# rhmes/point-cloud-compression

Measured on AMD Instinct MI355X. Metric: points/sec compress+decompress (ModelNet40-shaped 8192 K=256), higher is better.
Workload: dtype f32 (operands split into two scaled fp16 pieces of 22-23 bits together, three fp16-MFMA products per fp32 product, fp32 accumulate); 1 GPU; IPDAE K=256 d=16 L=7, 8192-pt CAD-like synthetic clouds (configs[1]); distinct_clouds_per_gpu=1024, points_per_cloud=8192, patches_per_cloud=64, octree_mode=reference, weights=seeded random, matmul=f16x2

## Files before the change

include/pccx.h:

```cpp
#ifndef PCCX_H
#define PCCX_H

#include <stddef.h>
#include <stdint.h>

#ifdef __cplusplus
extern "C" {
#endif

#define PCCX_API __attribute__((visibility("default")))

typedef enum {
    PCCX_OK = 0,
    PCCX_ERR_ARG = -1,
    PCCX_ERR_HIP = -2,
    PCCX_ERR_UNSUPPORTED = -3
} pccx_status;

PCCX_API const char *pccx_last_error(void);
PCCX_API int pccx_version(void);


PCCX_API int pccx_normalize(const float *pc, int B, int N, double margin, float *out, float *center,
                            float *longest, void *stream);

PCCX_API int pccx_denormalize(const float *pc, int B, int N, double margin, const float *center,
                              const float *longest, float *out, void *stream);

PCCX_API int pccx_fps(const float *xyz, int B, int N, int npoint, const int32_t *start_idx,
                      int64_t *idx_out, float *workspace, void *stream);

PCCX_API int pccx_morton_keys(const float *xyz, int64_t n, const float *lo_host, float extent, int64_t *keys,
                              void *stream);
PCCX_API int pccx_morton_keys_auto(const float *xyz, int64_t n, int64_t *keys, int32_t *bbox_workspace, void *stream);

PCCX_API size_t pccx_sort_keys_workspace_bytes(int64_t n);
PCCX_API int pccx_sort_keys_u64(int64_t *keys, int64_t n, int key_bits, int64_t *order, void *workspace, void *stream);
PCCX_API int pccx_gather_blocks(const float *pc, const int64_t *order, int64_t n, int block, int64_t first, int64_t stride,
                                int64_t count, float *blocks_out, void *stream);
PCCX_API int pccx_scatter_blocks(const float *rows_in, const int64_t *order, int64_t n, int block, int64_t first, int64_t stride,
                                 int64_t count, float *pc_out, void *stream);

PCCX_API int pccx_gather(const float *points, int B, int N, int C, const int64_t *idx, int M,
                         float *out, void *stream);

PCCX_API int pccx_knn(const float *q, int B, int M, const float *ref, int N, int K, float *dists,
                      int64_t *idx, float *nn, float patch_scale, void *stream);

PCCX_API int pccx_ball_query(const float *q, int B, int M, const float *ref, int N, int K,
                             float radius, float *dists, int64_t *idx, void *stream);
PCCX_API size_t pccx_ball_query_grid_workspace_ints(int B, int N);
PCCX_API int pccx_ball_query_grid(const float *q, int B, int M, const float *ref, int N, int K, float radius,
                                  int32_t *workspace, float *dists, int64_t *idx, void *stream);

PCCX_API int pccx_nn_dist(const float *X, int B, int P, const float *Y, int Q, float *d2, int32_t *nn,
                          void *stream);
PCCX_API int pccx_nn_dist_split_count(int B, int P, int Q);
PCCX_API int pccx_nn_dist_split(const float *X, int B, int P, const float *Y, int Q, int split, float *scratch_d, int32_t *scratch_nn,
                                float *d2, int32_t *nn, void *stream);

PCCX_API int pccx_grid_dims(int N, float ex, float ey, float ez, int32_t *dims, float *cell);
PCCX_API size_t pccx_grid_index_workspace_bytes(int B, int N);
PCCX_API size_t pccx_grid_query_workspace_bytes(int B, int M);
PCCX_API int pccx_grid_index_build(const float *Y, int B, int N, void *workspace, void *stream);
PCCX_API int pccx_grid_nn(const float *X, int B, int P, int Q, const void *index, void *query_workspace, float *d2, int32_t *nn,
                          void *stream);
PCCX_API int pccx_grid_knn(const float *q, int B, int M, int N, int K, const void *index, void *query_workspace, float *dists,
                           int64_t *idx, void *stream);

PCCX_API int pccx_chamfer_mean(const float *dxy, const float *dyx, int B, int P, int Q, float *out, void *stream);
PCCX_API int pccx_chamfer_grad(const float *X, int B, int P, const float *Y, int Q, const int32_t *nn_xy,
                               const int32_t *nn_yx, float grad_out, float *gX, float *gY, void *stream);
PCCX_API int pccx_chamfer_grad_dev(const float *X, int B, int P, const float *Y, int Q, const int32_t *nn_xy,
                                   const int32_t *nn_yx, const float *grad_out_dev, float *gX, float *gY, void *stream);
PCCX_API int pccx_chamfer_grad_dev_acc(const float *X, int B, int P, const float *Y, int Q, const int32_t *nn_xy,
                                       const int32_t *nn_yx, const float *grad_out_dev, float *gX, float *gY, int flags,
                                       void *stream);

PCCX_API int pccx_estimate_normals(const float *xyz, int B, int N, const int64_t *nbr, int K, float *normals,
                                   void *stream);
PCCX_API int pccx_point_plane_err(const float *X, int B, int P, const float *Y, const float *normals_Y, int Q,
                                  const int32_t *nn, float *err, void *stream);


PCCX_API int pccx_octree_bits_capacity(int S);

PCCX_API int pccx_octree_encode(const float *centres, int B, int S, int N, double min_bpp,
                                uint8_t *bits, int32_t *nbits, int32_t *depth, uint8_t *bytes,
                                int32_t *nbytes, void *stream);

PCCX_API int pccx_octree_decode(const uint8_t *bytes, int stride, const int32_t *nbytes, int B,
                                int mode, int S_out, float *out, int32_t *count, void *stream);


PCCX_API size_t pccx_ae_encoder_blob_floats(void);
PCCX_API int pccx_pack_ae_encoder(const float *sa_w0, const float *sa_b0, const float *sa_w1,
                                  const float *sa_b1, const float *sa_w2, const float *sa_b2,
                                  const float *pn_w0, const float *pn_b0, const float *pn_w1,
                                  const float *pn_b1, const float *pn_w2, const float *pn_b2,
                                  const float *pn_w3, const float *pn_b3, int d, float *blob_host);
PCCX_API size_t pccx_ae_decoder_blob_floats(int k);
PCCX_API int pccx_pack_ae_decoder(const float *ip_w0, const float *ip_b0, const float *ip_w1,
                                  const float *ip_b1, const float *ip_w2, const float *ip_b2,
                                  const float *m_w0, const float *m_b0, const float *m_w1,
                                  const float *m_b1, const float *m_w2, const float *m_b2,
                                  const float *m_w3, const float *m_b3, int k, int d, float *blob_host);
PCCX_API size_t pccx_prob_blob_floats(void);
PCCX_API int pccx_pack_prob(const float *p_w0, const float *p_b0, const float *p_w1, const float *p_b1,
                            const float *p_w2, const float *p_b2, const float *m_w0, const float *m_b0,
                            const float *m_w1, const float *m_b1, const float *m_w2, const float *m_b2,
                            int d, int L, float *blob_host);

PCCX_API int pccx_ae_encode(const float *patches, int P, int K, const float *enc_blob, int d, int L,
                            float *feat_ws, float *latent_raw, float *latent, float *latent_q,
                            void *stream);

PCCX_API int pccx_sa_forward(const float *patches, int P, int K, const float *enc_blob, float *feat,
                             void *stream);
PCCX_API int pccx_pn_forward(const float *patches, const float *feat, int P, int K,
                             const float *enc_blob, int d, int L, float *latent_raw, float *latent,
                             float *latent_q, void *stream);

PCCX_API size_t pccx_ae_decode_workspace_floats(int P);
PCCX_API int pccx_ae_decode(const float *latent_q, int P, int d, int k, const float *dec_blob,
                            float *workspace, float *patches_out, float scale, const float *centres,
                            const float *nrm_center, const float *nrm_longest, int S, double margin,
                            float *pc_out, void *stream);

PCCX_API size_t pccx_sa_b3_blob_floats(void);
PCCX_API int pccx_pack_sa_b3(const float *enc_blob_dev, float *sa_b3_blob_dev, void *stream);
PCCX_API int pccx_sa_forward_b3(const float *patches, int P, int K, const float *enc_blob, const float *sa_b3_blob,
                                float *feat, void *stream);
PCCX_API size_t pccx_pn_b3_blob_floats(void);
PCCX_API int pccx_pack_pn_b3(const float *enc_blob_dev, float *pn_b3_blob_dev, void *stream);
PCCX_API int pccx_pn_forward_b3(const float *patches, const float *feat, int P, int K, const float *enc_blob,
                                const float *pn_b3_blob, int d, int L, float *latent_raw, float *latent,
                                float *latent_q, void *stream);
PCCX_API int pccx_ae_encode_b3_fused_ok(int K);
PCCX_API int pccx_ae_encode_b3(const float *patches, int P, int K, const float *enc_blob, const float *sa_b3_blob,
                               const float *pn_b3_blob, int d, int L, float *latent_raw, float *latent,
                               float *latent_q, void *stream);
PCCX_API int pccx_patch_knn16_index_bytes(int K);
PCCX_API size_t pccx_patch_knn16_bytes(int P, int K);
PCCX_API int pccx_patch_knn16(const float *patches, int P, int K, void *nbr, void *stream);
PCCX_API size_t pccx_ae_encode_b3_workspace_bytes(int P, int K);
PCCX_API int pccx_ae_encode_b3_ws(const float *patches, int P, int K, const float *enc_blob, const float *sa_b3_blob,
                                  const float *pn_b3_blob, int d, int L, float *latent_raw, float *latent,
                                  float *latent_q, void *workspace, void *stream);
PCCX_API int pccx_ae_encode_b3_tables(const float *patches, int P, int K, const float *enc_blob, const float *sa_b3_blob,
                                      const float *pn_b3_blob, int d, int L, float *latent_raw, float *latent,
                                      float *latent_q, const void *tables, void *stream);
PCCX_API size_t pccx_dec_b3_blob_floats(int k);
PCCX_API int pccx_pack_ae_decoder_b3(const float *dec_blob_dev, int k, float *b3_blob_dev, void *stream);
PCCX_API size_t pccx_ae_decode_b3_workspace_floats(int P);
PCCX_API int pccx_ae_decode_b3(const float *latent_q, int P, int d, int k, const float *dec_blob,
                               const float *b3_blob, float *workspace, float *patches_out, float scale,
                               const float *centres, const float *nrm_center, const float *nrm_longest,
                               int S, double margin, float *pc_out, void *stream);

PCCX_API size_t pccx_ae_encoder_h2_blob_floats(void);
PCCX_API int pccx_pack_ae_encoder_h2(const float *sa_w0, const float *sa_b0, const float *sa_w1, const float *sa_b1,
                                     const float *sa_w2, const float *sa_b2, const float *pn_w0, const float *pn_b0,
                                     const float *pn_w1, const float *pn_b1, const float *pn_w2, const float *pn_b2,
                                     const float *pn_w3, const float *pn_b3, int d, float *h2_blob);
PCCX_API int pccx_ae_encode_h2_fused_ok(int K);
PCCX_API size_t pccx_ae_encode_h2_workspace_bytes(int P, int K);
PCCX_API int pccx_ae_encode_h2_ws(const float *patches, int P, int K, const float *enc_blob, const float *h2_blob, int d, int L,
                                  float *latent_raw, float *latent, float *latent_q, void *workspace, void *stream);
PCCX_API int pccx_ae_encode_h2_tables(const float *patches, int P, int K, const float *enc_blob, const float *h2_blob, int d, int L,
                                      float *latent_raw, float *latent, float *latent_q, const void *tables, void *stream);
PCCX_API size_t pccx_ae_decoder_h2_blob_floats(int k);
PCCX_API int pccx_pack_ae_decoder_h2(const float *ip_w0, const float *ip_b0, const float *ip_w1, const float *ip_b1,
                                     const float *ip_w2, const float *ip_b2, const float *m_w0, const float *m_b0,
                                     const float *m_w1, const float *m_b1, const float *m_w2, const float *m_b2,
                                     const float *m_w3, const float *m_b3, int k, int d, float *h2_blob);
PCCX_API size_t pccx_ae_decode_h2_workspace_floats(int P);
PCCX_API int pccx_ae_decode_h2(const float *latent_q, int P, int d, int k, const float *dec_blob, const float *h2_blob,
                               float *workspace, float *patches_out, float scale, const float *centres,
                               const float *nrm_center, const float *nrm_longest, int S, double margin, float *pc_out,
                               void *stream);

PCCX_API size_t pccx_patch_groups_workspace_ints(int B);
PCCX_API int pccx_patch_groups(const float *keys_a, int floats_a, const float *keys_b, int floats_b, int B, int S, int32_t *rep,
                               int32_t *uniq, int32_t *n_uniq, int32_t *workspace, void *stream);
PCCX_API int pccx_replicate_rows(const int32_t *rep, int64_t P, int row_floats, float *a0, float *a1, float *a2, void *stream);
PCCX_API int pccx_knn_list(const float *q, int B, int M, const float *ref, int N, int K, float *dists, int64_t *idx, float *nn,
                           float patch_scale, const int32_t *rep, void *stream);
PCCX_API int pccx_patch_knn16_list(const float *patches, int P, int K, void *nbr, const int32_t *uniq, const int32_t *n_uniq,
                                   void *stream);
PCCX_API int pccx_ae_encode_h2_tables_list(const float *patches, int P, int K, const float *enc_blob, const float *h2_blob, int d,
                                           int L, float *latent_raw, float *latent, float *latent_q, const void *tables,
                                           const int32_t *uniq, const int32_t *n_uniq, void *stream);
PCCX_API int pccx_ae_decode_h2_list(const float *latent_q, int P, int d, int k, const float *dec_blob, const float *h2_blob,
                                    float *workspace, float *patches_out, float scale, const float *centres,
                                    const float *nrm_center, const float *nrm_longest, int S, double margin, float *pc_out,
                                    const int32_t *uniq, const int32_t *n_uniq, void *stream);

PCCX_API int pccx_prob_forward(const float *centres, int B, int S, int d, int L, const float *prob_blob,
                               float *pmf, float *cdf, int32_t *cdf_int, void *stream);

PCCX_API int pccx_range_encode(const int32_t *cdf_int, const float *latent_q, int B, int nsym, int L,
                               uint8_t *out, int cap, int32_t *nbytes, void *stream);
PCCX_API int pccx_range_decode(const int32_t *cdf_int, const uint8_t *in, int stride,
                               const int32_t *nbytes, int B, int nsym, int L, float *latent_q,
                               void *stream);

PCCX_API int pccx_cdf_float_to_int(const float *cdf, int64_t nrows, int Lp, int32_t *cdf_int, void *stream);


PCCX_API size_t pccx_streams_packed_bytes(int B, int s_stride, int p_cap);
PCCX_API int pccx_write_streams_host(const void *packed_host, int B, int s_stride, int p_cap, const char *dir, const char *names,
                                     const int64_t *name_off, int threads);
PCCX_API int pccx_read_streams_host(void *packed_host, int B, int s_stride, int p_cap, const char *dir, const char *names,
                                    const int64_t *name_off, int threads);
PCCX_API int pccx_stream_sizes_host(int B, const char *dir, const char *names, const int64_t *name_off, int64_t *s_sizes,
                                    int64_t *p_sizes, int threads);


PCCX_API size_t pccx_packed_linear_floats(int N, int K);
PCCX_API int pccx_pack_linear(const float *W_host, int N, int K, float *wp_host);
PCCX_API int pccx_linear(const float *x, int M, int K, int ldx, const float *wp, const float *bias,
                         int N, int relu, float *out, int ldo, void *stream);

PCCX_API size_t pccx_packed_linear_b3_floats(int N, int K);
PCCX_API int pccx_pack_linear_b3(const float *wp_dev, int N, int K, float *wplanes_dev, void *stream);
PCCX_API int pccx_linear_b3(const float *x, int M, int K, int ldx, const float *wplanes, const float *bias,
                            int N, int relu, float *out, int ldo, void *stream);

PCCX_API size_t pccx_planes_floats(int64_t M, int K);
PCCX_API int pccx_group_planes(const float *f0, int C0, int ld0, const float *f1, int C1, int ld1, const int64_t *idx, int64_t M,
                               int64_t rows_per_batch, int64_t n_src, float *planes, void *stream);
PCCX_API int pccx_group_planes_centred(const float *feats, int C, int ldf, const float *offsets, const int64_t *idx, int64_t M,
                                       int64_t rows_per_batch, int64_t n_src, float *amax8, float *planes, void *stream);
PCCX_API int pccx_fold_planes(const float *f0, int C0, int ld0, int64_t mod0, const float *f1, int C1, int ld1, int64_t div1, int64_t M,
                              float *planes, void *stream);
PCCX_API int pccx_rows_affine_planes(const float *base, int C, int64_t div, const float *x, int ldx, int Ks, int64_t mod, const float *w,
                                     int relu, int64_t M, float *planes, void *stream);
PCCX_API size_t pccx_planes_gemm_weight_floats(int N, int K);
PCCX_API int pccx_pack_planes_gemm(const float *wplanes_dev, int N, int K, float *wstream_dev, void *stream);
PCCX_API int pccx_planes_gemm(const float *planes_in, int64_t M, int K, const float *wstream, const float *bias, int N, int relu,
                              int epilogue, int group, float *out, int ldo, void *stream);
PCCX_API int pccx_planes_gemm_gather(const float *src, int ldp, const int64_t *idx, int64_t rows_per_batch, int64_t n_src, int64_t M,
                                     int K, const float *wstream, const float *bias, int N, int relu, int epilogue, int group,
                                     float *out, int ldo, void *stream);
PCCX_API size_t pccx_planes_chain_wide_weight_floats(int K0);
PCCX_API int pccx_pack_planes_chain_wide(const float *wp3_l0, const float *wp3_l1, const float *wp3_l2, int K0, int N0, int N1, int N2,
                                         float *wstream_dev, void *stream);
PCCX_API int pccx_planes_chain_wide(const float *src, int ldp, const int64_t *idx, int64_t rows_per_batch, int64_t n_src, int64_t M,
                                    int K0, const float *wstream, const float *b0, int N0, const float *b1, int N1, const float *b2,
                                    int N2, float *out_planes, void *stream);
PCCX_API int pccx_planes_chain4(const float *planes_in, int64_t M, int K0, const float *wstream, const float *b0, int N0,
                                const float *b1, int N1, const float *b2, int N2, const float *b3, int N3, int group, float *out,
                                int ldo, void *stream);
PCCX_API int pccx_planes_chain4_gather(const float *src, int ldp, const int64_t *idx, int64_t rows_per_batch, int64_t n_src, int64_t M,
                                       int K0, const float *wstream, const float *b0, int N0, const float *b1, int N1,
                                       const float *b2, int N2, const float *b3, int N3, int group, float *out, int ldo, void *stream);

PCCX_API size_t pccx_planes_floats_h2(int64_t M, int K);
PCCX_API size_t pccx_packed_linear_h2_floats(int N, int K);
PCCX_API int pccx_pack_linear_h2(const float *wp_dev, int N, int K, float tau, float *wplanes_dev, void *stream);
PCCX_API size_t pccx_planes_gemm_weight_floats_h2(int N, int K);
PCCX_API int pccx_pack_planes_gemm_h2(const float *wplanes_dev, int N, int K, float *wstream_dev, void *stream);
PCCX_API int pccx_group_planes_h2(const float *f0, int C0, int ld0, const float *f1, int C1, int ld1, const int64_t *idx, int64_t M,
                                  int64_t rows_per_batch, int64_t n_src, float rho, const float *dyn, float *planes, void *stream);
PCCX_API int pccx_group_planes_centred_h2(const float *feats, int C, int ldf, const float *offsets, const int64_t *idx, int64_t M,
                                          int64_t rows_per_batch, int64_t n_src, float *amax8, float rho, const float *dyn, float *planes,
                                          void *stream);
PCCX_API int pccx_fold_planes_h2(const float *f0, int C0, int ld0, int64_t mod0, const float *f1, int C1, int ld1, int64_t div1, int64_t M,
                                 float rho, const float *dyn, float *planes, void *stream);
PCCX_API int pccx_rows_affine_planes_h2(const float *base, int C, int64_t div, const float *x, int ldx, int Ks, int64_t mod, const float *w,
                                        int relu, int64_t M, float rho, const float *dyn, float *planes, void *stream);
PCCX_API int pccx_planes_gemm_h2(const float *planes_in, int64_t M, int K, const float *wstream, const float *bias, int N, int relu,
                                 int epilogue, int group, float scale_out, const float *dyn, float *amax8, float *out, int ldo,
                                 void *stream);
PCCX_API int pccx_planes_gemm_h2_member_max(const float *planes_in, int64_t M, int K, const float *wstream, const float *bias, int N, int relu,
                                            int group, const unsigned char *member, float scale_out, const float *dyn, float *out, int ldo,
                                            void *stream);
PCCX_API int pccx_planes_gemm_h2_max_amax(const float *planes_in, int64_t M, int K, const float *wstream, const float *bias, int N, int relu,
                                          int group, float scale_out, const float *dyn, float *amax8, float *out, int ldo, void *stream);
PCCX_API int pccx_group_members(const int64_t *idx, int64_t n_idx, int64_t per_batch, int64_t n_src, unsigned char *member, void *stream);
PCCX_API int pccx_planes_gemm_gather_h2(const float *src, int ldp, const int64_t *idx, int64_t rows_per_batch, int64_t n_src, int64_t M,
                                        int K, const float *wstream, const float *bias, int N, int relu, int epilogue, int group,
                                        float rho_in, float scale_out, const float *dyn, float *amax8, float *out, int ldo,
                                        void *stream);
PCCX_API int pccx_planes_chain4_h2(const float *planes_in, int64_t M, int K0, const float *wstream, const float *b0, int N0,
                                   const float *b1, int N1, const float *b2, int N2, const float *b3, int N3, int group,
                                   const float *scales5_host, const float *dyn, float *amax8, float *out, int ldo, void *stream);
PCCX_API int pccx_planes_chain4_gather_h2(const float *src, int ldp, const int64_t *idx, int64_t rows_per_batch, int64_t n_src, int64_t M,
                                          int K0, const float *wstream, const float *b0, int N0, const float *b1, int N1,
                                          const float *b2, int N2, const float *b3, int N3, int group, const float *scales5_host,
                                          const float *dyn, float *amax8, float *out, int ldo, void *stream);
PCCX_API int pccx_absmax(const float *x, int64_t n, float *amax8, void *stream);
PCCX_API int pccx_dyn_scale(const float *m1_8, float a1, const float *m2_8, float a2, float add, int combine, float *dyn2, void *stream);

PCCX_API int pccx_softmax_cdf(const float *logits, int64_t rows, int L, float *pmf, float *cdf, int32_t *cdf_int, void *stream);
PCCX_API int pccx_reassemble(const float *patches, int64_t P, int k, float scale, const float *centres, const float *nrm_center,
                             const float *nrm_longest, int S, double margin, float *out, void *stream);
PCCX_API int pccx_rows_affine_small(const float *base, int C, int64_t div, const float *x, int ldx, int Ks, int64_t mod,
                                    const float *w, int relu, int64_t M, float *out, void *stream);
PCCX_API int pccx_gather_max(const float *y, int B, int N, int C, const int64_t *idx, int M, int ns, float *out, void *stream);
PCCX_API int pccx_gather_max_rows(const float *y, int B, int N, int C, const int64_t *idx, int M, int ns, const float *xyz, float *out, int ldo,
                                  void *stream);
PCCX_API int pccx_group_max(const float *x, int64_t G, int Kn, int C, float *out, void *stream);

PCCX_API int pccx_sigmoid_spread(const float *x, int64_t n, int L, int do_round, float *y, void *stream);
PCCX_API int pccx_round(const float *x, int64_t n, float *y, void *stream);

PCCX_API int pccx_quantize_st(const float *x, int64_t n, float qmin, float qmax, int levels, float *y_q,
                              float *y_deq, void *stream);

PCCX_API int pccx_pack_linear_device(const float *W, int N, int K, int transpose, float *wp, void *stream);
PCCX_API int pccx_linear_dw(const float *dZ, const float *X, int64_t M, int N, int K, int ldz, int ldx,
                            float *dW, int flags, void *stream);
PCCX_API int pccx_bn_train_stats(const float *Z, int64_t M, int C, float eps, float momentum, double *sums,
                                 float *mean, float *rstd, float *running_mean, float *running_var,
                                 void *stream);
PCCX_API int pccx_bn_relu_forward(const float *Z, int64_t M, int C, const float *mean, const float *rstd,
                                  const float *gamma, const float *beta, int relu, float *Y, void *stream);
PCCX_API int pccx_bn_relu_backward(const float *dY, const float *Y, const float *Z, int64_t M, int C,
                                   const float *mean, const float *rstd, const float *gamma, double *sums,
                                   float *dZ, float *g_gamma, float *g_beta, void *stream);
PCCX_API int pccx_linear_skinny(const float *x, int M, int K, int ldx, const float *W, const float *bias, int N, int flags,
                                float *out, int ldo, void *stream);
PCCX_API int pccx_linear_skinny_dx(const float *dZ, int M, int N, int ldz, const float *W, int K, int flags, float *dX, int ldd,
                                   void *stream);
PCCX_API int pccx_col_sum(const float *dY, int64_t M, int C, double *sums, float *g_bias, void *stream);
PCCX_API int pccx_bn_relu_train_forward(const float *Z, int64_t M, int C, float eps, float momentum, double *sums, const float *gamma,
                                        const float *beta, int relu, float *mean, float *rstd, float *running_mean,
                                        float *running_var, float *Y, int flags, void *stream);
PCCX_API int pccx_bn_relu_train_backward(const float *dY, const float *Y, const float *Z, int64_t M, int C, const float *mean,
                                         const float *rstd, const float *gamma, double *sums, float *dZ, float *g_gamma,
                                         float *g_beta, int flags, void *stream);
PCCX_API int pccx_col_sum_w(const float *dY, int64_t M, int C, double *sums, float *g_bias, int flags, void *stream);
PCCX_API size_t pccx_train_sums_doubles(int C);
PCCX_API int pccx_linear_moments(const float *x, int M, int K, int ldx, const float *wp, int N, int flags, float *out, int ldo,
                                 double *sums, void *stream);
PCCX_API int pccx_linear_bnback(const float *x, int M, int K, int ldx, const float *wp, int N, int flags, float *out, int ldo,
                                const float *Y, const float *Z, const float *mean, const float *rstd, double *sums, void *stream);
PCCX_API int pccx_zero_bytes(void *p, size_t bytes, void *stream);
PCCX_API int pccx_copy_bytes(const void *src, void *dst, size_t bytes, void *stream);
PCCX_API int pccx_add_i64_table(const int64_t *table_dev, int n, int64_t delta, void *stream);
PCCX_API int pccx_relu_backward(const float *dY, const float *Y, int64_t n, float *dZ, void *stream);
PCCX_API int pccx_group_max_arg(const float *x, int64_t G, int Kn, int C, float *out, int32_t *arg,
                                void *stream);
PCCX_API int pccx_group_max_backward(const float *dOut, const int32_t *arg, int64_t G, int Kn, int C,
                                     float *dX, void *stream);
PCCX_API int pccx_gather_backward(const float *dG, int ldg, const int64_t *idx, int B, int Mrows, int N,
                                  int C, float *dF, void *stream);
PCCX_API int pccx_gather_backward_acc(const float *dG, int ldg, const int64_t *idx, int B, int Mrows, int N, int C, float *dF,
                                      int flags, void *stream);
PCCX_API int pccx_smooth_l1(const float *a, const float *b, int64_t n, float grad_scale, double *value,
                            float *grad, void *stream);
PCCX_API int pccx_quantize_st_backward(const float *x, const float *d_ydeq, int64_t n, float qmin, float qmax,
                                       int levels, float *dx, void *stream);
PCCX_API int pccx_rate_from_logits(const float *logits, const float *y_q, int B, int bins, int ld_yq,
                                   float *out, void *stream);
PCCX_API int pccx_sumsq_accumulate(const float *g, int64_t n, double *acc, void *stream);
PCCX_API int pccx_adam_step(float *param, const float *grad, float *exp_avg, float *exp_avg_sq, int64_t n,
                            const double *gnorm_sq, float max_norm, float lr, float beta1, float beta2,
                            float eps, int step, void *stream);
PCCX_API int pccx_sumsq_multi(const int64_t *table_dev, int ntensors, int64_t total_blocks, double *acc, void *stream);
PCCX_API int pccx_adam_multi(const int64_t *table_dev, int ntensors, int64_t total_blocks, const double *gnorm_sq,
                             float max_norm, const float *hyper_dev, float lr, int step, float beta1, float beta2,
                             float eps, void *stream);
PCCX_API int pccx_adam_advance_dev(float *hyper, double beta1, double beta2, void *stream);
PCCX_API int pccx_adam_step_dev(float *param, const float *grad, float *exp_avg, float *exp_avg_sq, int64_t n,
                                const double *gnorm_sq, float max_norm, const float *hyper, float beta1, float beta2,
                                float eps, void *stream);

PCCX_API size_t pccx_linear_dw_det_workspace_floats(int64_t M, int N, int K);
PCCX_API int pccx_linear_dw_det(const float *dZ, const float *X, int64_t M, int N, int K, int ldz, int ldx, float *dW, int flags,
                                float *workspace, void *stream);
PCCX_API size_t pccx_linear_skinny_dx_det_workspace_floats(int M, int N, int K);
PCCX_API int pccx_linear_skinny_dx_det(const float *dZ, int M, int N, int ldz, const float *W, int K, int flags, float *dX, int ldd,
                                       float *workspace, void *stream);
PCCX_API size_t pccx_col_reduce_det_doubles(int64_t M, int C);
PCCX_API int pccx_col_reduce_det(int mode, const float *A, const float *Y, const float *Z, const float *mean, const float *rstd,
                                 int64_t M, int C, double *partials, double *sums, float *f32_out, void *stream);
PCCX_API size_t pccx_smooth_l1_det_doubles(int64_t n);
PCCX_API int pccx_smooth_l1_det(const float *a, const float *b, int64_t n, float grad_scale, double *partials, double *value,
                                float *grad, void *stream);
PCCX_API size_t pccx_sumsq_multi_det_doubles(int64_t total_blocks);
PCCX_API int pccx_sumsq_multi_det(const int64_t *table_dev, int ntensors, int64_t total_blocks, double *partials, double *acc,
                                  void *stream);
PCCX_API size_t pccx_scatter_add_ordered_workspace_ints(int B, int Mrows, int N);
PCCX_API int pccx_scatter_add_ordered(const float *vals, int ldv, const void *idx, int idx_is_i32, int B, int Mrows, int N, int C,
                                      float *out, int32_t *workspace, void *stream);
PCCX_API size_t pccx_chamfer_grad_det_workspace_floats(int B, int P, int Q);
PCCX_API size_t pccx_chamfer_grad_det_workspace_ints(int B, int P, int Q);
PCCX_API int pccx_chamfer_grad_det(const float *X, int B, int P, const float *Y, int Q, const int32_t *nn_xy, const int32_t *nn_yx,
                                   const float *grad_out_dev, float *gX, float *gY, float *ws_floats, int32_t *ws_ints, void *stream);

#ifdef __cplusplus
}
#endif
#endif
```

point-cloud-compression_amd/csrc/decoder.hip:

```cpp
#include <math.h>
#include <stdlib.h>

#include "blobs.h"
#include "common.h"
#include "mfma_chain.h"
#include "plane_ring.h"

__global__ __launch_bounds__(256, 2) void dec_head_kernel(const float *__restrict__ latent_q, int P, int d, int ntiles,
                                                          const float *__restrict__ blob, f32x4 *__restrict__ h2p,
                                                          const int *__restrict__ uniq, const int *__restrict__ n_uniq)
{
    const int tid = threadIdx.x, lane = tid & 63, w = tid >> 6;
    const int g = lane >> 4, n = lane & 15;
    const int tile = blockIdx.x * 4 + w;
    if (uniq) P = *n_uniq;
    if (tile >= (P + 15) / 16) return;
    const int patch = tile * 16 + n;
    const size_t src = patch < P ? (uniq ? (size_t)uniq[patch] : (size_t)patch) : 0;
    f32x4 in[1][1];
#pragma unroll
    for (int r = 0; r < 4; ++r) in[0][0][r] = (patch < P && 4 * g + r < d) ? latent_q[src * d + 4 * g + r] : 0.f;
    f32x4 a1[1][16];
#pragma unroll
    for (int mt = 0; mt < 16; ++mt) a1[0][mt] = *(const f32x4 *)(blob + DEC_H_B1 + 16 * mt + 4 * g);
    dense_acc<1, 16, 1, 16>((const f32x4 *)(blob + DEC_H_W1), lane, in, a1);
#pragma unroll
    for (int mt = 0; mt < 16; ++mt) a1[0][mt] = relu4(a1[0][mt]);
    const f32x4 *w2 = (const f32x4 *)(blob + DEC_H_W2);
#pragma unroll 1
    for (int mc = 0; mc < 16; ++mc) {
        const f32x4 *w2c = opaque_uniform(w2) + (size_t)mc * 4 * 64;
        f32x4 a2[1][4];
#pragma unroll
        for (int m = 0; m < 4; ++m) a2[0][m] = *(const f32x4 *)(blob + DEC_H_B2 + 16 * (4 * mc + m) + 4 * g);
        dense_acc<16, 4, 1, 64>(w2c, lane, a1, a2);
#pragma unroll
        for (int m = 0; m < 4; ++m) h2p[((size_t)(4 * mc + m) * ntiles + tile) * 64 + lane] = relu4(a2[0][m]);
    }
}

int pccx_dec_head_launch(const float *latent_q, int P, int d, int ntiles, const float *dec_blob, float *h2p, const int32_t *uniq,
                         const int32_t *n_uniq, hipStream_t st)
{
    hipLaunchKernelGGL(dec_head_kernel, dim3((ntiles + 3) / 4), dim3(256), 0, st, latent_q, P, d, ntiles, dec_blob, (f32x4 *)h2p, uniq, n_uniq);
    PCCX_CHECK_LAUNCH();
    return PCCX_OK;
}

__device__ __forceinline__ unsigned b3_rne(float x)
{
    unsigned u = __float_as_uint(x);
    u += 0x7FFFu + ((u >> 16) & 1u);
    return u >> 16;
}
__device__ __forceinline__ void b3_split(float x, unsigned &h, unsigned &m, unsigned &l)
{
    h = b3_rne(x);
    const float r1 = __fsub_rn(x, __uint_as_float(h << 16));
    m = b3_rne(r1);
    l = b3_rne(__fsub_rn(r1, __uint_as_float(m << 16)));
}

__global__ __launch_bounds__(256) void b3_split_kernel(const f32x4 *__restrict__ src, uint4 *__restrict__ dst, int n_outer, int KT16, int W,
                                                       size_t src_outer, size_t dst_outer, int src_w)
{
    const int lane = threadIdx.x & 63, T = (KT16 + 1) / 2;
    const size_t item = (size_t)blockIdx.x * 4 + (threadIdx.x >> 6);
    if (item >= (size_t)n_outer * T * W) return;
    const int j = (int)(item % W), t = (int)((item / W) % T);
    const size_t o = item / ((size_t)W * T);
    const f32x4 v0 = src[o * src_outer + ((size_t)(2 * t) * src_w + j) * 64 + lane];
    const f32x4 zero = {0.f, 0.f, 0.f, 0.f};
    const f32x4 v1 = 2 * t + 1 < KT16 ? src[o * src_outer + ((size_t)(2 * t + 1) * src_w + j) * 64 + lane] : zero;
    unsigned h[8], m[8], l[8];
#pragma unroll
    for (int r = 0; r < 4; ++r) { b3_split(v0[r], h[r], m[r], l[r]); b3_split(v1[r], h[4 + r], m[4 + r], l[4 + r]); }
    uint4 *d = dst + o * dst_outer + ((size_t)t * W + j) * 3 * 64 + lane;
    d[0] = make_uint4(h[0] | (h[1] << 16), h[2] | (h[3] << 16), h[4] | (h[5] << 16), h[6] | (h[7] << 16));
    d[64] = make_uint4(m[0] | (m[1] << 16), m[2] | (m[3] << 16), m[4] | (m[5] << 16), m[6] | (m[7] << 16));
    d[128] = make_uint4(l[0] | (l[1] << 16), l[2] | (l[3] << 16), l[4] | (l[5] << 16), l[6] | (l[7] << 16));
}

template <int NT>
__device__ __forceinline__ void dec_store_points(const f32x4 (&m3)[NT][1], int tile0, int ntiles, int g, int n, int P, int k, int p,
                                                 float *__restrict__ patches_out, float inv_scale_div, const float *__restrict__ centres,
                                                 const float *__restrict__ nrm_center, const float *__restrict__ nrm_longest, int S,
                                                 float one_minus_margin, float *__restrict__ pc_out)
{
    if (g != 0) return;
#pragma unroll
    for (int nt = 0; nt < NT; ++nt) {
        const int patch = (tile0 + nt) * 16 + n;
        if (tile0 + nt < ntiles && patch < P) {
            float v[3] = {m3[nt][0][0], m3[nt][0][1], m3[nt][0][2]};
            if (patches_out) {
                float *o = patches_out + ((size_t)patch * k + p) * 3;
                o[0] = v[0]; o[1] = v[1]; o[2] = v[2];
            }
            if (pc_out) {
                const int b = patch / S;
                const float lg = nrm_longest[b];
                float *o = pc_out + ((size_t)patch * k + p) * 3;
#pragma unroll
                for (int a = 0; a < 3; ++a) {
                    float t = __fdiv_rn(v[a], inv_scale_div);
                    t = __fadd_rn(t, centres[(size_t)patch * 3 + a]);
                    t = __fsub_rn(t, 0.5f);
                    t = __fdiv_rn(__fmul_rn(t, lg), one_minus_margin);
                    o[a] = __fadd_rn(t, nrm_center[3 * b + a]);
                }
            }
        }
    }
}

__global__ __launch_bounds__(256, 2) void dec_main_kernel(const f32x4 *__restrict__ h2p, const float *__restrict__ latent_q,
                                                          int P, int d, int k, int ntiles, const float *__restrict__ blob,
                                                          float *__restrict__ patches_out, float inv_scale_div,
                                                          const float *__restrict__ centres, const float *__restrict__ nrm_center,
                                                          const float *__restrict__ nrm_longest, int S, float one_minus_margin,
                                                          float *__restrict__ pc_out)
{
    const int tid = threadIdx.x, lane = tid & 63, w = tid >> 6;
    const int g = lane >> 4, n = lane & 15;
    const int nblk = (ntiles + 7) / 8;
    const int grp = blockIdx.x / (DEC_GROUP * k), rem = blockIdx.x % (DEC_GROUP * k);
    const int p = rem / DEC_GROUP, blk = grp * DEC_GROUP + rem % DEC_GROUP;
    if (blk >= nblk) return;
    const int tile0 = blk * 8 + 2 * w;
    __shared__ __attribute__((aligned(16))) f32x4 swt[2 * DEC_WS_CHUNK * 64];
    const int wu = __builtin_amdgcn_readfirstlane(w);
    const WStreamT<DEC_WS_CHUNK, 2> ws{blob + DEC_G_W(k) + (size_t)p * DEC_STREAM_CHUNKS * DEC_WS_CHUNK * 256, swt, DEC_STREAM_CHUNKS, lane, wu, false};
    ws.prologue();

    f32x4 acc[2][8];
#pragma unroll
    for (int mt = 0; mt < 8; ++mt) {
        const f32x4 b = *(const f32x4 *)(blob + DEC_G_B + p * 128 + 16 * mt + 4 * g);
        acc[0][mt] = b; acc[1][mt] = b;
    }
    const int t0 = tile0 < ntiles ? tile0 : ntiles - 1, t1 = tile0 + 1 < ntiles ? tile0 + 1 : ntiles - 1;
    {
        f32x4 b_cur[2], b_nxt[2];
        b_cur[0] = h2p[((size_t)0 * ntiles + t0) * 64 + lane];
        b_cur[1] = h2p[((size_t)0 * ntiles + t1) * 64 + lane];
#pragma unroll 1
        for (int c = 0; c < 64 / (DEC_WS_CHUNK / 8); ++c) {
            ws.boundary(c);
            const f32x4 *buf = swt + (c & 1) * DEC_WS_CHUNK * 64 + lane;
#pragma unroll
            for (int h = 0; h < DEC_WS_CHUNK / 8; ++h) {
                const int kt = (DEC_WS_CHUNK / 8) * c + h;
                const int kn = kt + 1 < 64 ? kt + 1 : 63;
                b_nxt[0] = h2p[((size_t)kn * ntiles + t0) * 64 + lane];
                b_nxt[1] = h2p[((size_t)kn * ntiles + t1) * 64 + lane];
                f32x4 a[8];
#pragma unroll
                for (int mt = 0; mt < 8; ++mt) a[mt] = buf[(h * 8 + mt) * 64];
                __builtin_amdgcn_sched_barrier(0);
#pragma unroll
                for (int r = 0; r < 4; ++r)
#pragma unroll
                    for (int mt = 0; mt < 8; ++mt) {
                        acc[0][mt] = mfma16(a[mt][r], b_cur[0][r], acc[0][mt]);
                        acc[1][mt] = mfma16(a[mt][r], b_cur[1][r], acc[1][mt]);
                    }
                __builtin_amdgcn_sched_barrier(0);
                b_cur[0] = b_nxt[0]; b_cur[1] = b_nxt[1];
            }
        }
    }
    f32x4 m3[2][1];
    {
        f32x4 in[2][9];
#pragma unroll
        for (int nt = 0; nt < 2; ++nt) {
#pragma unroll
            for (int mt = 0; mt < 8; ++mt) in[nt][mt] = relu4(acc[nt][mt]);
            const int patch = (tile0 + nt) * 16 + n;
#pragma unroll
            for (int r = 0; r < 4; ++r)
                in[nt][8][r] = (patch < P && 4 * g + r < d) ? latent_q[(size_t)patch * d + 4 * g + r] : 0.f;
        }
        f32x4 m0[2][8];
#pragma unroll
        for (int nt = 0; nt < 2; ++nt)
#pragma unroll
            for (int mt = 0; mt < 8; ++mt) m0[nt][mt] = *(const f32x4 *)(blob + DEC_M_B0 + 16 * mt + 4 * g);
        int f = DEC_STREAM_GEMM_FRAGS;
        dense_acc_stream<9, 8, 2>(ws, f, in, m0);
#pragma unroll
        for (int nt = 0; nt < 2; ++nt)
#pragma unroll
            for (int mt = 0; mt < 8; ++mt) m0[nt][mt] = relu4(m0[nt][mt]);
        f32x4 m1[2][4];
#pragma unroll
        for (int nt = 0; nt < 2; ++nt)
#pragma unroll
            for (int mt = 0; mt < 4; ++mt) m1[nt][mt] = *(const f32x4 *)(blob + DEC_M_B1 + 16 * mt + 4 * g);
        dense_acc_stream<8, 4, 2>(ws, f, m0, m1);
#pragma unroll
        for (int nt = 0; nt < 2; ++nt)
#pragma unroll
            for (int mt = 0; mt < 4; ++mt) m1[nt][mt] = relu4(m1[nt][mt]);
        f32x4 m2[2][2];
#pragma unroll
        for (int nt = 0; nt < 2; ++nt)
#pragma unroll
            for (int mt = 0; mt < 2; ++mt) m2[nt][mt] = *(const f32x4 *)(blob + DEC_M_B2 + 16 * mt + 4 * g);
        dense_acc_stream<4, 2, 2>(ws, f, m1, m2);
#pragma unroll
        for (int nt = 0; nt < 2; ++nt)
#pragma unroll
            for (int mt = 0; mt < 2; ++mt) m2[nt][mt] = relu4(m2[nt][mt]);
#pragma unroll
        for (int nt = 0; nt < 2; ++nt) m3[nt][0] = *(const f32x4 *)(blob + DEC_M_B3 + 4 * g);
        dense_acc_stream<2, 1, 2>(ws, f, m2, m3);
    }
    ws.drain();
    dec_store_points<2>(m3, tile0, ntiles, g, n, P, k, p, patches_out, inv_scale_div, centres, nrm_center, nrm_longest, S, one_minus_margin, pc_out);
}

template <int NT>
__global__ __launch_bounds__(256, NT == 2 ? 2 : 1) void dec_main_kernel_b3(const uint4 *__restrict__ h3, const float *__restrict__ latent_q,
                                                          int P, int d, int k, int ntiles, const float *__restrict__ blob,
                                                          const float *__restrict__ blob3,
                                                          float *__restrict__ patches_out, float inv_scale_div,
                                                          const float *__restrict__ centres, const float *__restrict__ nrm_center,
                                                          const float *__restrict__ nrm_longest, int S, float one_minus_margin,
                                                          float *__restrict__ pc_out)
{
    const int tid = threadIdx.x, lane = tid & 63, w = tid >> 6;
    const int g = lane >> 4, n = lane & 15;
    constexpr int GRP = DEC_GROUP * 2 / NT;
    const int nblk = (ntiles + 4 * NT - 1) / (4 * NT);
    const int grp = blockIdx.x / (GRP * k), rem = blockIdx.x % (GRP * k);
    const int p = rem / GRP, blk = grp * GRP + rem % GRP;
    if (blk >= nblk) return;
    const int tile0 = blk * 4 * NT + NT * w;
    __shared__ __attribute__((aligned(16))) f32x4 swt[4 * DEC_B3_CHUNK * 64];
    const int wu = __builtin_amdgcn_readfirstlane(w);
    const WStreamT<DEC_B3_CHUNK, 4> ws{blob3 + (size_t)p * DEC_B3_STREAM_CHUNKS * DEC_B3_CHUNK * 256, swt, DEC_B3_STREAM_CHUNKS, lane, wu, false};
    ws.prologue();

    f32x4 acc[NT][8];
#pragma unroll
    for (int mt = 0; mt < 8; ++mt) {
        const f32x4 b = *(const f32x4 *)(blob + DEC_G_B + p * 128 + 16 * mt + 4 * g);
#pragma unroll
        for (int nt = 0; nt < NT; ++nt) acc[nt][mt] = b;
    }
    int tq[NT];
#pragma unroll
    for (int nt = 0; nt < NT; ++nt) tq[nt] = tile0 + nt < ntiles ? tile0 + nt : ntiles - 1;
    pg_ring_gemm<3, NT, 3, 4, 2, true, 32, false>(
        ws, 32, [&](int nt, int pl, int t) { return h3 + (((size_t)t * ntiles + tq[nt]) * 3 + pl) * 64 + lane; }, 1.f, acc);
    f32x4 m3[NT][1];
    {
        int f = DEC_B3_GEMM_FRAGS;
        bf16x8 i0[NT][5][3];
        const f32x4 zero = {0.f, 0.f, 0.f, 0.f};
#pragma unroll
        for (int nt = 0; nt < NT; ++nt) {
#pragma unroll
            for (int t = 0; t < 4; ++t) b3_split8(relu4(acc[nt][2 * t]), relu4(acc[nt][2 * t + 1]), i0[nt][t]);
            const int patch = (tile0 + nt) * 16 + n;
            f32x4 lat;
#pragma unroll
            for (int r = 0; r < 4; ++r) lat[r] = (patch < P && 4 * g + r < d) ? latent_q[(size_t)patch * d + 4 * g + r] : 0.f;
            b3_split8(lat, zero, i0[nt][4]);
        }
        f32x4 m0[NT][8];
#pragma unroll
        for (int nt = 0; nt < NT; ++nt)
#pragma unroll
            for (int mt = 0; mt < 8; ++mt) m0[nt][mt] = *(const f32x4 *)(blob + DEC_M_B0 + 16 * mt + 4 * g);
        dense_b3_stream<5, 8, NT>(ws, f, i0, m0);
        bf16x8 i1[NT][4][3];
#pragma unroll
        for (int nt = 0; nt < NT; ++nt)
#pragma unroll
            for (int t = 0; t < 4; ++t) b3_split8(relu4(m0[nt][2 * t]), relu4(m0[nt][2 * t + 1]), i1[nt][t]);
        f32x4 m1[NT][4];
#pragma unroll
        for (int nt = 0; nt < NT; ++nt)
#pragma unroll
            for (int mt = 0; mt < 4; ++mt) m1[nt][mt] = *(const f32x4 *)(blob + DEC_M_B1 + 16 * mt + 4 * g);
        dense_b3_stream<4, 4, NT>(ws, f, i1, m1);
        bf16x8 i2[NT][2][3];
#pragma unroll
        for (int nt = 0; nt < NT; ++nt)
#pragma unroll
            for (int t = 0; t < 2; ++t) b3_split8(relu4(m1[nt][2 * t]), relu4(m1[nt][2 * t + 1]), i2[nt][t]);
        f32x4 m2[NT][2];
#pragma unroll
        for (int nt = 0; nt < NT; ++nt)
#pragma unroll
            for (int mt = 0; mt < 2; ++mt) m2[nt][mt] = *(const f32x4 *)(blob + DEC_M_B2 + 16 * mt + 4 * g);
        dense_b3_stream<2, 2, NT>(ws, f, i2, m2);
        bf16x8 i3[NT][1][3];
#pragma unroll
        for (int nt = 0; nt < NT; ++nt) b3_split8(relu4(m2[nt][0]), relu4(m2[nt][1]), i3[nt][0]);
#pragma unroll
        for (int nt = 0; nt < NT; ++nt) m3[nt][0] = *(const f32x4 *)(blob + DEC_M_B3 + 4 * g);
        dense_b3_stream<1, 1, NT>(ws, f, i3, m3);
    }
    ws.drain();
    dec_store_points<NT>(m3, tile0, ntiles, g, n, P, k, p, patches_out, inv_scale_div, centres, nrm_center, nrm_longest, S, one_minus_margin, pc_out);
}

static unsigned dec_grid(int ntiles, int k, int NT = 2)
{
    const int grp = DEC_GROUP * 2 / NT;
    const int nblk = (ntiles + 4 * NT - 1) / (4 * NT), groups = (nblk + grp - 1) / grp;
    return (unsigned)groups * grp * (unsigned)k;
}

extern "C" size_t pccx_ae_decode_workspace_floats(int P)
{
    const size_t ntiles = ((size_t)(P > 0 ? P : 0) + 15) / 16;
    return (size_t)64 * ntiles * 64 * 4;
}

extern "C" int pccx_ae_decode(const float *latent_q, int P, int d, int k, const float *dec_blob, float *workspace,
                              float *patches_out, float scale, const float *centres, const float *nrm_center,
                              const float *nrm_longest, int S, double margin, float *pc_out, void *stream)
{
    if (P == 0) return PCCX_OK;
    PCCX_CHECK_ARG(latent_q && dec_blob && workspace, "pccx_ae_decode: null pointer");
    PCCX_CHECK_ARG(patches_out || pc_out, "pccx_ae_decode: need patches_out and/or pc_out");
    PCCX_CHECK_ARG(P >= 0 && d >= 1 && d <= 16 && k >= 1 && k <= 65535, "pccx_ae_decode: unsupported P=%d d=%d k=%d", P, d, k);
    PCCX_CHECK_ARG(!pc_out || (centres && nrm_center && nrm_longest && S >= 1 && scale != 0.f),
                   "pccx_ae_decode: pc_out needs centres, center, longest, S >= 1 and scale != 0");
    if (P == 0) return PCCX_OK;
    hipStream_t st = (hipStream_t)stream;
    const int ntiles = (P + 15) / 16;
    hipLaunchKernelGGL(dec_head_kernel, dim3((ntiles + 3) / 4), dim3(256), 0, st, latent_q, P, d, ntiles, dec_blob,
                       (f32x4 *)workspace, (const int *)nullptr, (const int *)nullptr);
    PCCX_CHECK_LAUNCH();
    hipLaunchKernelGGL(dec_main_kernel, dim3(dec_grid(ntiles, k)), dim3(256), 0, st, (const f32x4 *)workspace, latent_q, P, d,
                       k, ntiles, dec_blob, patches_out, scale, centres, nrm_center, nrm_longest, S > 0 ? S : 1, (float)(1.0 - margin), pc_out);
    PCCX_CHECK_LAUNCH();
    return PCCX_OK;
}

extern "C" size_t pccx_dec_b3_blob_floats(int k) { return DEC_B3_BLOB_FLOATS(k > 0 ? k : 0); }

extern "C" int pccx_pack_ae_decoder_b3(const float *dec_blob_dev, int k, float *b3_blob_dev, void *stream)
{
    PCCX_CHECK_ARG(dec_blob_dev && b3_blob_dev && k >= 1, "pccx_pack_ae_decoder_b3: bad argument");
    hipStream_t st = (hipStream_t)stream;
    PCCX_CHECK_HIP(hipMemsetAsync(b3_blob_dev, 0, sizeof(float) * DEC_B3_BLOB_FLOATS(k), st));
    const size_t so = (size_t)DEC_STREAM_CHUNKS * DEC_WS_CHUNK * 64, dst_o = (size_t)DEC_B3_STREAM_CHUNKS * DEC_B3_CHUNK * 64;
    const f32x4 *src = (const f32x4 *)(dec_blob_dev + DEC_G_W(k));
    const int KT16[5] = {64, 9, 8, 4, 2}, MTL[5] = {8, 8, 4, 2, 1};
    size_t s_off = 0, d_off = 0;
    for (int l = 0; l < 5; ++l) {
        const int T = (KT16[l] + 1) / 2;
        const size_t items = (size_t)k * T * MTL[l];
        hipLaunchKernelGGL(b3_split_kernel, dim3((unsigned)((items + 3) / 4)), dim3(256), 0, st, src + s_off * 64,
                           (uint4 *)b3_blob_dev + d_off * 64, k, KT16[l], MTL[l], so, dst_o, MTL[l]);
        PCCX_CHECK_LAUNCH();
        s_off += (size_t)KT16[l] * MTL[l];
        d_off += (size_t)T * MTL[l] * 3;
    }
    return PCCX_OK;
}

extern "C" size_t pccx_sa_b3_blob_floats(void) { return (size_t)(1 * 4 * 3 + 2 * 8 * 3) * 256; }

extern "C" int pccx_pack_sa_b3(const float *enc_blob_dev, float *sa_b3_blob_dev, void *stream)
{
    PCCX_CHECK_ARG(enc_blob_dev && sa_b3_blob_dev, "pccx_pack_sa_b3: null pointer");
    hipStream_t st = (hipStream_t)stream;
    hipLaunchKernelGGL(b3_split_kernel, dim3((1 * 4 + 3) / 4), dim3(256), 0, st, (const f32x4 *)(enc_blob_dev + ENC_SA_W1),
                       (uint4 *)sa_b3_blob_dev, 1, 2, 4, (size_t)0, (size_t)0, 4);
    PCCX_CHECK_LAUNCH();
    hipLaunchKernelGGL(b3_split_kernel, dim3((2 * 8 + 3) / 4), dim3(256), 0, st, (const f32x4 *)(enc_blob_dev + ENC_SA_W2),
                       (uint4 *)sa_b3_blob_dev + 12 * 64, 1, 4, 8, (size_t)0, (size_t)0, 8);
    PCCX_CHECK_LAUNCH();
    return PCCX_OK;
}

extern "C" size_t pccx_pn_b3_blob_floats(void) { return PN_B3_BLOB_FLOATS; }

extern "C" int pccx_pack_pn_b3(const float *enc_blob_dev, float *pn_b3_blob_dev, void *stream)
{
    PCCX_CHECK_ARG(enc_blob_dev && pn_b3_blob_dev, "pccx_pack_pn_b3: null pointer");
    hipStream_t st = (hipStream_t)stream;
    PCCX_CHECK_HIP(hipMemsetAsync(pn_b3_blob_dev, 0, sizeof(float) * PN_B3_BLOB_FLOATS, st));
    struct Seg { size_t src; int kt16, w, src_w; };
    const Seg segs[6] = {{ENC_PN_W0, 9, 8, 8},
                         {ENC_PN_W1, 8, 16, 16},
                         {ENC_PN_W2, 16, 16, 32},
                         {ENC_PN_W3, 16, 1, 1},
                         {ENC_PN_W2 + (size_t)16 * 256, 16, 16, 32},
                         {ENC_PN_W3 + (size_t)16 * 256, 16, 1, 1}};
    size_t d_off = 0;
    for (int l = 0; l < 6; ++l) {
        const int T = (segs[l].kt16 + 1) / 2;
        const size_t items = (size_t)T * segs[l].w;
        hipLaunchKernelGGL(b3_split_kernel, dim3((unsigned)((items + 3) / 4)), dim3(256), 0, st, (const f32x4 *)(enc_blob_dev + segs[l].src),
                           (uint4 *)pn_b3_blob_dev + d_off * 64, 1, segs[l].kt16, segs[l].w, (size_t)0, (size_t)0, segs[l].src_w);
        PCCX_CHECK_LAUNCH();
        d_off += (size_t)T * segs[l].w * 3;
    }
    return PCCX_OK;
}

extern "C" size_t pccx_ae_decode_b3_workspace_floats(int P)
{
    const size_t ntiles = ((size_t)(P > 0 ? P : 0) + 15) / 16;
    return (size_t)(64 + 96) * ntiles * 64 * 4;
}

extern "C" int pccx_ae_decode_b3(const float *latent_q, int P, int d, int k, const float *dec_blob, const float *b3_blob,
                                 float *workspace, float *patches_out, float scale, const float *centres, const float *nrm_center,
                                 const float *nrm_longest, int S, double margin, float *pc_out, void *stream)
{
    if (P == 0) return PCCX_OK;
    PCCX_CHECK_ARG(latent_q && dec_blob && b3_blob && workspace, "pccx_ae_decode_b3: null pointer");
    PCCX_CHECK_ARG(patches_out || pc_out, "pccx_ae_decode_b3: need patches_out and/or pc_out");
    PCCX_CHECK_ARG(P >= 0 && d >= 1 && d <= 16 && k >= 1 && k <= 65535, "pccx_ae_decode_b3: unsupported P=%d d=%d k=%d", P, d, k);
    PCCX_CHECK_ARG(!pc_out || (centres && nrm_center && nrm_longest && S >= 1 && scale != 0.f),
                   "pccx_ae_decode_b3: pc_out needs centres, center, longest, S >= 1 and scale != 0");
    hipStream_t st = (hipStream_t)stream;
    const int ntiles = (P + 15) / 16;
    f32x4 *h2p = (f32x4 *)workspace;
    uint4 *h3 = (uint4 *)(workspace + (size_t)64 * ntiles * 64 * 4);
    hipLaunchKernelGGL(dec_head_kernel, dim3((ntiles + 3) / 4), dim3(256), 0, st, latent_q, P, d, ntiles, dec_blob, h2p, (const int *)nullptr, (const int *)nullptr);
    PCCX_CHECK_LAUNCH();
    const size_t items = (size_t)32 * ntiles;
    hipLaunchKernelGGL(b3_split_kernel, dim3((unsigned)((items + 3) / 4)), dim3(256), 0, st, (const f32x4 *)h2p, h3, 1, 64, ntiles,
                       (size_t)0, (size_t)0, ntiles);
    PCCX_CHECK_LAUNCH();
    const char *e = getenv("PCCX_DEC_NT");
    if (e && atoi(e) == 4)
        hipLaunchKernelGGL((dec_main_kernel_b3<4>), dim3(dec_grid(ntiles, k, 4)), dim3(256), 0, st, (const uint4 *)h3, latent_q, P, d, k,
                           ntiles, dec_blob, b3_blob, patches_out, scale, centres, nrm_center, nrm_longest, S > 0 ? S : 1,
                           (float)(1.0 - margin), pc_out);
    else
        hipLaunchKernelGGL((dec_main_kernel_b3<2>), dim3(dec_grid(ntiles, k)), dim3(256), 0, st, (const uint4 *)h3, latent_q, P, d, k,
                           ntiles, dec_blob, b3_blob, patches_out, scale, centres, nrm_center, nrm_longest, S > 0 ? S : 1,
                           (float)(1.0 - margin), pc_out);
    PCCX_CHECK_LAUNCH();
    return PCCX_OK;
}
```

point-cloud-compression_amd/csrc/decoder_h2.hip:

```cpp
#include <math.h>
#include <stdlib.h>

#include "blobs.h"
#include "common.h"
#include "mfma_chain.h"
#include "plane_ring.h"

int pccx_dec_head_launch(const float *latent_q, int P, int d, int ntiles, const float *dec_blob, float *h2p, const int32_t *uniq,
                         const int32_t *n_uniq, hipStream_t st);

__global__ __launch_bounds__(256) void dec_h2_prep_kernel(const f32x4 *__restrict__ h2p, const float *__restrict__ latent_q, int P, int d,
                                                          int ntiles, float sig_h, uint4 *__restrict__ h3, float *__restrict__ pscale,
                                                          const int *__restrict__ uniq, const int *__restrict__ n_uniq)
{
    const int lane = threadIdx.x & 63, g = lane >> 4, n = lane & 15;
    const int tile = blockIdx.x * 4 + (threadIdx.x >> 6);
    if (uniq) P = *n_uniq;
    if (tile >= (P + 15) / 16) return;
    float m = 0.f;
    for (int kt = 0; kt < 64; ++kt) {
        const f32x4 v = h2p[((size_t)kt * ntiles + tile) * 64 + lane];
        m = fmaxf(fmaxf(m, fmaxf(v[0], v[1])), fmaxf(v[2], v[3]));
    }
    const int patch = tile * 16 + n;
    const size_t src = patch < P ? (uniq ? (size_t)uniq[patch] : (size_t)patch) : 0;
#pragma unroll
    for (int r = 0; r < 4; ++r)
        if (patch < P && 4 * g + r < d) m = fmaxf(m, fabsf(latent_q[src * d + 4 * g + r]));
    m = fmaxf(m, __shfl_xor(m, 16));
    m = fmaxf(m, __shfl_xor(m, 32));
    const int rexp = (int)(__float_as_uint(m) >> 23) - 127;
    const float s = rexp >= 0 ? __uint_as_float((unsigned)(126 - rexp) << 23) : 1.0f;
    if (g == 0) pscale[patch] = s;
    const float sc = s * sig_h;
    for (int t = 0; t < 32; ++t) {
        const f32x4 v0 = h2p[((size_t)(2 * t) * ntiles + tile) * 64 + lane], v1 = h2p[((size_t)(2 * t + 1) * ntiles + tile) * 64 + lane];
        f16x8 pl[2];
        h2_split8(v0, v1, sc, pl);
        uint4 *o = h3 + (((size_t)t * ntiles + tile) * 2) * 64 + lane;
        o[0] = __builtin_bit_cast(uint4, pl[0]);
        o[64] = __builtin_bit_cast(uint4, pl[1]);
    }
}

template <int NT>
__global__ __launch_bounds__(256, 2) void dec_main_h2_kernel(const uint4 *__restrict__ h3, const float *__restrict__ pscale,
                                                             const float *__restrict__ latent_q, int P, int d, int k, int ntiles,
                                                             const float *__restrict__ hb, float *__restrict__ patches_out,
                                                             float inv_scale_div, const float *__restrict__ centres,
                                                             const float *__restrict__ nrm_center, const float *__restrict__ nrm_longest, int S,
                                                             float one_minus_margin, float *__restrict__ pc_out,
                                                             const int *__restrict__ uniq, const int *__restrict__ n_uniq)
{
    static_assert(NT == 2 || NT == 4, "two or four patch tiles per wave");
    constexpr int NP = NT / 2;
    constexpr int SETS = NT == 2 ? 3 : 2;
    const int tid = threadIdx.x, lane = tid & 63, w = tid >> 6;
    const int g = lane >> 4, n = lane & 15;
    constexpr int GRP = DEC_GROUP * 2 / NT;
    const int ntl = ((uniq ? *n_uniq : P) + 15) / 16;
    const int nblk = (ntl + 4 * NT - 1) / (4 * NT);
    const int grp = blockIdx.x / (GRP * k), rem = blockIdx.x % (GRP * k);
    const int p = rem / GRP, blk = grp * GRP + rem % GRP;
    if (blk >= nblk) return;
    const int tile0 = blk * 4 * NT + NT * w;
    constexpr int CH = DEC_H2_CHUNK, NB = 4;
    __shared__ __attribute__((aligned(16))) f32x4 swt[NB * CH * 64];
    const int wu = __builtin_amdgcn_readfirstlane(w);
    const WStreamT<CH, NB> ws{hb + DEC_H2_G_W(k) + (size_t)p * DEC_H2_STREAM_CHUNKS * DEC_H2_CHUNK * 256, swt, DEC_H2_STREAM_CHUNKS, lane, wu, false};
    ws.prologue();

    int tq[NT];
    float sn[NT];
#pragma unroll
    for (int nt = 0; nt < NT; ++nt) {
        tq[nt] = tile0 + nt < ntl ? tile0 + nt : ntl - 1;
        sn[nt] = pscale[tq[nt] * 16 + n];
    }
    f32x4 acc[NT][8];
#pragma unroll
    for (int mt = 0; mt < 8; ++mt) {
        const f32x4 b = *(const f32x4 *)(hb + DEC_H2_G_B + (size_t)p * 128 + 16 * mt + 4 * g);
#pragma unroll
        for (int nt = 0; nt < NT; ++nt) acc[nt][mt] = b * sn[nt];
    }
    pg_ring_gemm<2, NT, SETS, 4, 2, true, 32, false>(
        ws, 32, [&](int nt, int pl, int t) { return h3 + (((size_t)t * ntiles + tq[nt]) * 2 + pl) * 64 + lane; }, 1.f, acc);
    int lane_t = __builtin_amdgcn_mbcnt_hi(~0u, __builtin_amdgcn_mbcnt_lo(~0u, 0u));
    asm volatile("" : "+v"(lane_t));
    const int g_t = lane_t >> 4, n_t = lane_t & 15;
    const int tile0_t = blk * 4 * NT + NT * wu;
    const int *nu_t = n_uniq;
    asm volatile("" : "+s"(nu_t));
    const int P_t = uniq ? __builtin_amdgcn_readfirstlane(*nu_t) : P, ntl_t = (P_t + 15) / 16;
    const float *meta = hb + DEC_H2_META;
    asm volatile("" : "+s"(meta));
    auto uni = [](float v) { return __uint_as_float(__builtin_amdgcn_readfirstlane(__float_as_uint(v))); };
    const float rho0 = uni(meta[H2D_RHO0]), sig_q = uni(meta[H2D_SIG_Q]), rho1 = uni(meta[H2D_RHO1]);
    const float rho2 = uni(meta[H2D_RHO2]), rho3 = uni(meta[H2D_RHO3]), inv_out = uni(meta[H2D_INV_OUT]);
    float sn_t[NT];
#pragma unroll
    for (int nt = 0; nt < NT; ++nt) {
        const int tt = tile0_t + nt < ntl_t ? tile0_t + nt : ntl_t - 1;
        sn_t[nt] = pscale[tt * 16 + n_t];
    }
    const WStreamT<CH, NB> ws_t{ws.g, swt, DEC_H2_STREAM_CHUNKS, lane_t, wu, false};
    const unsigned goff = 16u * (unsigned)g_t;
    auto bias4 = [&](int at) { return *(const f32x4 *)((const char *)(hb + at) + goff); };
    int f = DEC_H2_GEMM_FRAGS;
#pragma unroll
    for (int pr = 0; pr < NP; ++pr) {
        f32x4 m3[2][1];
        {
            f16x8 i0[2][5][2];
            const f32x4 zero = {0.f, 0.f, 0.f, 0.f};
#pragma unroll
            for (int nt = 0; nt < 2; ++nt) {
#pragma unroll
                for (int t = 0; t < 4; ++t) h2_split8(relu4(acc[2 * pr + nt][2 * t]), relu4(acc[2 * pr + nt][2 * t + 1]), rho0, i0[nt][t]);
                const int patch = (tile0_t + 2 * pr + nt) * 16 + n_t;
                const int src = patch < P_t ? (uniq ? uniq[patch] : patch) : 0;
                f32x4 lat;
#pragma unroll
                for (int r = 0; r < 4; ++r) lat[r] = (patch < P_t && 4 * g_t + r < d) ? latent_q[(size_t)src * d + 4 * g_t + r] : 0.f;
                h2_split8(lat, zero, sn_t[2 * pr + nt] * sig_q, i0[nt][4]);
            }
            f32x4 m0[2][8];
#pragma unroll
            for (int nt = 0; nt < 2; ++nt)
#pragma unroll
                for (int mt = 0; mt < 8; ++mt) m0[nt][mt] = bias4(DEC_H2_M_B0 + 16 * mt) * sn_t[2 * pr + nt];
            dense_h2_stream<5, 8, 2>(ws_t, f, i0, m0);
            f16x8 i1[2][4][2];
#pragma unroll
            for (int nt = 0; nt < 2; ++nt)
#pragma unroll
                for (int t = 0; t < 4; ++t) h2_split8(relu4(m0[nt][2 * t]), relu4(m0[nt][2 * t + 1]), rho1, i1[nt][t]);
            f32x4 m1[2][4];
#pragma unroll
            for (int nt = 0; nt < 2; ++nt)
#pragma unroll
                for (int mt = 0; mt < 4; ++mt) m1[nt][mt] = bias4(DEC_H2_M_B1 + 16 * mt) * sn_t[2 * pr + nt];
            dense_h2_stream<4, 4, 2>(ws_t, f, i1, m1);
            f16x8 i2[2][2][2];
#pragma unroll
            for (int nt = 0; nt < 2; ++nt)
#pragma unroll
                for (int t = 0; t < 2; ++t) h2_split8(relu4(m1[nt][2 * t]), relu4(m1[nt][2 * t + 1]), rho2, i2[nt][t]);
            f32x4 m2[2][2];
#pragma unroll
            for (int nt = 0; nt < 2; ++nt)
#pragma unroll
                for (int mt = 0; mt < 2; ++mt) m2[nt][mt] = bias4(DEC_H2_M_B2 + 16 * mt) * sn_t[2 * pr + nt];
            dense_h2_stream<2, 2, 2>(ws_t, f, i2, m2);
            f16x8 i3[2][1][2];
#pragma unroll
            for (int nt = 0; nt < 2; ++nt) h2_split8(relu4(m2[nt][0]), relu4(m2[nt][1]), rho3, i3[nt][0]);
#pragma unroll
            for (int nt = 0; nt < 2; ++nt) m3[nt][0] = bias4(DEC_H2_M_B3) * sn_t[2 * pr + nt];
            dense_h2_stream<1, 1, 2>(ws_t, f, i3, m3);
        }
        if (g_t == 0) {
#pragma unroll
            for (int nt = 0; nt < 2; ++nt) {
                const int tile = tile0_t + 2 * pr + nt, slot = tile * 16 + n_t;
                if (tile < ntl_t && slot < P_t) {
                    const int patch = uniq ? uniq[slot] : slot;
                    const float un = __fmul_rn(inv_out, __fdiv_rn(1.0f, sn_t[2 * pr + nt]));
                    float v[3] = {__fmul_rn(m3[nt][0][0], un), __fmul_rn(m3[nt][0][1], un), __fmul_rn(m3[nt][0][2], un)};
                    if (patches_out) {
                        float *o = patches_out + ((size_t)patch * k + p) * 3;
                        o[0] = v[0]; o[1] = v[1]; o[2] = v[2];
                    }
                    if (pc_out) {
                        const int b = patch / S;
                        const float lg = nrm_longest[b];
                        float *o = pc_out + ((size_t)patch * k + p) * 3;
#pragma unroll
                        for (int a = 0; a < 3; ++a) {
                            float t = __fdiv_rn(v[a], inv_scale_div);
                            t = __fadd_rn(t, centres[(size_t)patch * 3 + a]);
                            t = __fsub_rn(t, 0.5f);
                            t = __fdiv_rn(__fmul_rn(t, lg), one_minus_margin);
                            o[a] = __fadd_rn(t, nrm_center[3 * b + a]);
                        }
                    }
                }
            }
        }
    }
    ws.drain();
}

static unsigned dec_h2_grid(int ntiles, int k, int NT)
{
    const int grp = DEC_GROUP * 2 / NT;
    const int nblk = (ntiles + 4 * NT - 1) / (4 * NT), groups = (nblk + grp - 1) / grp;
    return (unsigned)groups * grp * (unsigned)k;
}

extern "C" size_t pccx_ae_decode_h2_workspace_floats(int P)
{
    const size_t ntiles = ((size_t)(P > 0 ? P : 0) + 15) / 16;
    return (size_t)(64 + 64) * ntiles * 64 * 4 + ntiles * 16;
}

extern "C" int pccx_ae_decode_h2_list(const float *latent_q, int P, int d, int k, const float *dec_blob, const float *h2_blob, float *workspace,
                                      float *patches_out, float scale, const float *centres, const float *nrm_center, const float *nrm_longest,
                                      int S, double margin, float *pc_out, const int32_t *uniq, const int32_t *n_uniq, void *stream)
{
    if (P == 0) return PCCX_OK;
    PCCX_CHECK_ARG(latent_q && dec_blob && h2_blob && workspace, "pccx_ae_decode_h2: null pointer");
    PCCX_CHECK_ARG(patches_out || pc_out, "pccx_ae_decode_h2: need patches_out and/or pc_out");
    PCCX_CHECK_ARG(!uniq == !n_uniq, "pccx_ae_decode_h2_list: uniq and n_uniq come together");
    PCCX_CHECK_ARG(P >= 0 && d >= 1 && d <= 16 && k >= 1 && k <= 65535, "pccx_ae_decode_h2: unsupported P=%d d=%d k=%d", P, d, k);
    PCCX_CHECK_ARG(!pc_out || (centres && nrm_center && nrm_longest && S >= 1 && scale != 0.f),
                   "pccx_ae_decode_h2: pc_out needs centres, center, longest, S >= 1 and scale != 0");
    hipStream_t st = (hipStream_t)stream;
    const int ntiles = (P + 15) / 16;
    float *h2p = workspace;
    uint4 *h3 = (uint4 *)(workspace + (size_t)64 * ntiles * 64 * 4);
    float *pscale = workspace + (size_t)128 * ntiles * 64 * 4;
    const int rc = pccx_dec_head_launch(latent_q, P, d, ntiles, dec_blob, h2p, uniq, n_uniq, st);
    if (rc != PCCX_OK) return rc;
    hipLaunchKernelGGL(dec_h2_prep_kernel, dim3((ntiles + 3) / 4), dim3(256), 0, st, (const f32x4 *)h2p, latent_q, P, d, ntiles, 32768.0f, h3, pscale, uniq, n_uniq);
    PCCX_CHECK_LAUNCH();
    const char *e = getenv("PCCX_DEC_H2_NT");
    if (e && atoi(e) == 2)
        hipLaunchKernelGGL((dec_main_h2_kernel<2>), dim3(dec_h2_grid(ntiles, k, 2)), dim3(256), 0, st, (const uint4 *)h3, (const float *)pscale, latent_q, P,
                           d, k, ntiles, h2_blob, patches_out, scale, centres, nrm_center, nrm_longest, S > 0 ? S : 1, (float)(1.0 - margin), pc_out, uniq, n_uniq);
    else
        hipLaunchKernelGGL((dec_main_h2_kernel<4>), dim3(dec_h2_grid(ntiles, k, 4)), dim3(256), 0, st, (const uint4 *)h3, (const float *)pscale, latent_q, P,
                           d, k, ntiles, h2_blob, patches_out, scale, centres, nrm_center, nrm_longest, S > 0 ? S : 1, (float)(1.0 - margin), pc_out, uniq, n_uniq);
    PCCX_CHECK_LAUNCH();
    return PCCX_OK;
}

extern "C" int pccx_ae_decode_h2(const float *latent_q, int P, int d, int k, const float *dec_blob, const float *h2_blob, float *workspace,
                                 float *patches_out, float scale, const float *centres, const float *nrm_center, const float *nrm_longest,
                                 int S, double margin, float *pc_out, void *stream)
{
    return pccx_ae_decode_h2_list(latent_q, P, d, k, dec_blob, h2_blob, workspace, patches_out, scale, centres, nrm_center, nrm_longest, S, margin,
                                  pc_out, nullptr, nullptr, stream);
}
```

point-cloud-compression_amd/csrc/knn.hip:

```cpp
#include <math.h>

#include "common.h"

__device__ __forceinline__ int block_scan_find(int h, int remaining, int *s_wsum, int *s_found, int tid)
{
    const int lane = tid & 63, w = tid >> 6;
    int incl = h;
#pragma unroll
    for (int o = 1; o < 64; o <<= 1) {
        int t = __shfl_up(incl, o);
        if (lane >= o) incl += t;
    }
    if (lane == 63) s_wsum[w] = incl;
    __syncthreads();
    int base = 0;
    for (int k = 0; k < w; ++k) base += s_wsum[k];
    incl += base;
    const int excl = incl - h;
    if (excl < remaining && remaining <= incl) {
        s_found[0] = tid;
        s_found[1] = remaining - excl;
        s_found[2] = h;
    }
    __syncthreads();
    return 0;
}

__global__ __launch_bounds__(256) void knn_kernel(const float *__restrict__ q, int M, const float *__restrict__ ref,
                                                  int N, int K, int Kp, float *__restrict__ dists,
                                                  int64_t *__restrict__ idx, float *__restrict__ nn, float patch_scale,
                                                  const int *__restrict__ rep)
{
    extern __shared__ unsigned char smem_raw[];
    unsigned long long *sel = (unsigned long long *)smem_raw;
    unsigned *keys = (unsigned *)(sel + Kp);
    int *hist = (int *)(keys + N);
    int *s_wsum = hist + 256;
    int *s_found = s_wsum + 4;
    int *s_cnt = s_found + 3;

    const int tid = threadIdx.x;
    const int m = blockIdx.x, b = blockIdx.y;
    if (rep && rep[b * M + m] != b * M + m) return;
    const float *rp = ref + (size_t)b * N * 3;
    const float qx = q[((size_t)b * M + m) * 3], qy = q[((size_t)b * M + m) * 3 + 1], qz = q[((size_t)b * M + m) * 3 + 2];

    for (int i = tid; i < N; i += 256)
        keys[i] = __float_as_uint(pccx_sqdist(qx, qy, qz, rp[3 * i], rp[3 * i + 1], rp[3 * i + 2]));
    if (tid == 0) *s_cnt = 0;

    unsigned prefix = 0;
    int remaining = K, ties = 0;
    for (int p = 3; p >= 0; --p) {
        hist[tid] = 0;
        __syncthreads();
        const int sh = 8 * p;
        for (int i = tid; i < N; i += 256) {
            unsigned k = keys[i];
            bool match = (p == 3) || ((k >> (sh + 8)) == (prefix >> (sh + 8)));
            if (match) atomicAdd(&hist[(k >> sh) & 255u], 1);
        }
        __syncthreads();
        block_scan_find(hist[tid], remaining, s_wsum, s_found, tid);
        prefix |= (unsigned)s_found[0] << sh;
        remaining = s_found[1];
        ties = s_found[2];
        __syncthreads();
    }
    int idx_thresh = 0x7fffffff;
    if (ties != remaining) {
        unsigned ipre = 0;
        for (int p = 1; p >= 0; --p) {
            hist[tid] = 0;
            __syncthreads();
            const int sh = 8 * p;
            for (int i = tid; i < N; i += 256) {
                bool match = keys[i] == prefix && (p == 1 || ((unsigned)i >> 8) == (ipre >> 8));
                if (match) atomicAdd(&hist[((unsigned)i >> sh) & 255u], 1);
            }
            __syncthreads();
            block_scan_find(hist[tid], remaining, s_wsum, s_found, tid);
            ipre |= (unsigned)s_found[0] << sh;
            remaining = s_found[1];
            __syncthreads();
        }
        idx_thresh = (int)ipre;
    }

    for (int i = tid; i < N; i += 256) {
        unsigned k = keys[i];
        if (k < prefix || (k == prefix && i <= idx_thresh)) {
            int pos = atomicAdd(s_cnt, 1);
            if (pos < Kp) sel[pos] = ((unsigned long long)k << 32) | (unsigned)i;
        }
    }
    for (int i = K + tid; i < Kp; i += 256) sel[i] = ~0ull;
    __syncthreads();

    for (int size = 2; size <= Kp; size <<= 1) {
        for (int stride = size >> 1; stride > 0; stride >>= 1) {
            for (int t = tid; t < (Kp >> 1); t += 256) {
                int lo = 2 * t - (t & (stride - 1));
                int hi = lo + stride;
                bool up = ((lo & size) == 0);
                unsigned long long a = sel[lo], c = sel[hi];
                if ((a > c) == up) { sel[lo] = c; sel[hi] = a; }
            }
            __syncthreads();
        }
    }

    const size_t ob = ((size_t)b * M + m) * K;
    for (int k = tid; k < K; k += 256) {
        unsigned long long e = sel[k];
        int i = (int)(e & 0xffffffffu);
        if (dists) dists[ob + k] = __uint_as_float((unsigned)(e >> 32));
        if (idx) idx[ob + k] = i;
        if (nn) {
            float x = rp[3 * i], y = rp[3 * i + 1], z = rp[3 * i + 2];
            if (patch_scale != 0.f) {
                x = __fmul_rn(__fsub_rn(x, qx), patch_scale);
                y = __fmul_rn(__fsub_rn(y, qy), patch_scale);
                z = __fmul_rn(__fsub_rn(z, qz), patch_scale);
            }
            nn[(ob + k) * 3] = x; nn[(ob + k) * 3 + 1] = y; nn[(ob + k) * 3 + 2] = z;
        }
    }
}

#define KNN_PPT 32
#define KNN_BINS 2048
#define KNN_CAPB 256

template <int X>
__device__ __forceinline__ unsigned knn_xor_lane(unsigned v)
{
    if (X == 1) return (unsigned)__builtin_amdgcn_mov_dpp((int)v, 0xB1, 0xF, 0xF, true);
    if (X == 2) return (unsigned)__builtin_amdgcn_mov_dpp((int)v, 0x4E, 0xF, 0xF, true);
    if (X == 3) return (unsigned)__builtin_amdgcn_mov_dpp((int)v, 0x1B, 0xF, 0xF, true);
    if (X == 7) return (unsigned)__builtin_amdgcn_mov_dpp((int)v, 0x141, 0xF, 0xF, true);
    if (X == 15) return (unsigned)__builtin_amdgcn_mov_dpp((int)v, 0x140, 0xF, 0xF, true);
    if (X < 32) return (unsigned)__builtin_amdgcn_ds_swizzle((int)v, (X << 10) | 0x1F);
    return (unsigned)__shfl_xor((int)v, X);
}

__device__ __forceinline__ unsigned long long knn_exchange(unsigned long long v, int x)
{
    unsigned lo = (unsigned)v, hi = (unsigned)(v >> 32);
    switch (x) {
    case 1: lo = knn_xor_lane<1>(lo); hi = knn_xor_lane<1>(hi); break;
    case 2: lo = knn_xor_lane<2>(lo); hi = knn_xor_lane<2>(hi); break;
    case 3: lo = knn_xor_lane<3>(lo); hi = knn_xor_lane<3>(hi); break;
    case 4: lo = knn_xor_lane<4>(lo); hi = knn_xor_lane<4>(hi); break;
    case 7: lo = knn_xor_lane<7>(lo); hi = knn_xor_lane<7>(hi); break;
    case 8: lo = knn_xor_lane<8>(lo); hi = knn_xor_lane<8>(hi); break;
    case 15: lo = knn_xor_lane<15>(lo); hi = knn_xor_lane<15>(hi); break;
    case 16: lo = knn_xor_lane<16>(lo); hi = knn_xor_lane<16>(hi); break;
    case 31: lo = knn_xor_lane<31>(lo); hi = knn_xor_lane<31>(hi); break;
    default: lo = __shfl_xor(lo, x); hi = __shfl_xor(hi, x); break;
    }
    return ((unsigned long long)hi << 32) | lo;
}

template <int PSH, int SH, int WIDTH>
__device__ __forceinline__ void knn_level(const unsigned (&key)[KNN_PPT], int *hist, int *s_wsum, int *s_found, int tid,
                                          unsigned &P, int &r, int &cnt)
{
    const int lane = tid & 63, w = tid >> 6;
#pragma unroll
    for (int t = 0; t < KNN_BINS / 256; ++t) hist[t * 256 + tid] = 0;
    __syncthreads();
#pragma unroll
    for (int t = 0; t < KNN_PPT; ++t)
        if ((key[t] >> PSH) == P) atomicAdd(&hist[(key[t] >> SH) & ((1u << WIDTH) - 1u)], 1);
    __syncthreads();
    int own[KNN_BINS / 256], s = 0;
#pragma unroll
    for (int t = 0; t < KNN_BINS / 256; ++t) { own[t] = hist[tid * (KNN_BINS / 256) + t]; s += own[t]; }
    int incl = s;
#pragma unroll
    for (int o = 1; o < 64; o <<= 1) {
        const int up = __shfl_up(incl, o);
        if (lane >= o) incl += up;
    }
    if (lane == 63) s_wsum[w] = incl;
    __syncthreads();
    for (int k = 0; k < w; ++k) incl += s_wsum[k];
    int excl = incl - s;
    if (excl < r && r <= incl) {
#pragma unroll
        for (int t = 0; t < KNN_BINS / 256; ++t) {
            if (excl < r && r <= excl + own[t]) { s_found[0] = tid * (KNN_BINS / 256) + t; s_found[1] = excl; s_found[2] = own[t]; }
            excl += own[t];
        }
    }
    __syncthreads();
    P = (P << WIDTH) | (unsigned)s_found[0];
    r -= s_found[1];
    cnt = s_found[2];
}

__global__ __launch_bounds__(256, 4) void knn_fast_kernel(const float *__restrict__ q, int M, const float *__restrict__ ref,
                                                       int N, int K, float *__restrict__ dists, int64_t *__restrict__ idx,
                                                       float *__restrict__ nn, float patch_scale, const int *__restrict__ rep)
{
    __shared__ int hist[KNN_BINS];
    __shared__ unsigned long long selA[256], selB[KNN_CAPB];
    __shared__ int s_wsum[4], s_found[3], s_cnt[2];
    const int tid = threadIdx.x, lane = tid & 63, w = tid >> 6;
    const int m = blockIdx.x, b = blockIdx.y;
    if (rep && rep[b * M + m] != b * M + m) return;
    const float *rp = ref + (size_t)b * N * 3;
    const size_t qo = ((size_t)b * M + m) * 3;
    const float qx = q[qo], qy = q[qo + 1], qz = q[qo + 2];
    const size_t ob = ((size_t)b * M + m) * K;

    unsigned key[KNN_PPT];
#pragma unroll
    for (int t = 0; t < KNN_PPT; ++t) {
        const int i = t * 256 + tid;
        key[t] = i < N ? __float_as_uint(pccx_sqdist(qx, qy, qz, rp[3 * i], rp[3 * i + 1], rp[3 * i + 2])) : 0x7FFFFFFFu;
    }
    if (tid < 2) s_cnt[tid] = 0;

    unsigned P = 0;
    int sh = 20, r = K, cnt_b = 0;
    knn_level<31, 20, 11>(key, hist, s_wsum, s_found, tid, P, r, cnt_b);
    if (cnt_b > KNN_CAPB) {
        sh = 9;
        knn_level<20, 9, 11>(key, hist, s_wsum, s_found, tid, P, r, cnt_b);
        if (cnt_b > KNN_CAPB) {
            sh = 0;
            knn_level<9, 0, 9>(key, hist, s_wsum, s_found, tid, P, r, cnt_b);
        }
    }
    const int nA = K - r;

    const bool use_b = cnt_b <= KNN_CAPB;
    int cnt = 0;
#pragma unroll
    for (int t = 0; t < KNN_PPT; ++t) {
        const unsigned pre = key[t] >> sh;
        cnt += (pre < P ? 1 : 0) + (pre == P ? 0x10000 : 0);
    }
    int incl = cnt;
#pragma unroll
    for (int o = 1; o < 64; o <<= 1) {
        const int up = __shfl_up(incl, o);
        if (lane >= o) incl += up;
    }
    int base = 0;
    if (lane == 63) base = atomicAdd(&s_cnt[0], incl);
    base = __shfl(base, 63) + incl - cnt;
    int posA = base & 0xFFFF, posB = base >> 16;
#pragma unroll
    for (int t = 0; t < KNN_PPT; ++t) {
        const unsigned pre = key[t] >> sh;
        const unsigned long long e = ((unsigned long long)key[t] << 32) | (unsigned)(t * 256 + tid);
        if (pre < P) selA[posA++] = e;
        else if (pre == P && use_b) selB[posB++] = e;
    }
    __syncthreads();
    if (cnt_b <= KNN_CAPB) {
        if (tid < cnt_b) {
            const unsigned long long e = selB[tid];
            int rank = 0;
            for (int j = 0; j < cnt_b; ++j) rank += selB[j] < e ? 1 : 0;
            if (rank < r) selA[nA + rank] = e;
        }
    } else {
        int base = 0;
#pragma unroll 1
        for (int t = 0; t < KNN_PPT && base < r; ++t) {
            const bool tie = key[t] == P;
            const unsigned long long bal = __ballot(tie);
            if (lane == 0) s_wsum[w] = __popcll(bal);
            __syncthreads();
            int off = base, row = 0;
            for (int k = 0; k < 4; ++k) { off += k < w ? s_wsum[k] : 0; row += s_wsum[k]; }
            const int rank = off + __popcll(bal & ((1ull << lane) - 1ull));
            if (tie && rank < r) selA[nA + rank] = ((unsigned long long)key[t] << 32) | (unsigned)(t * 256 + tid);
            base += row;
            __syncthreads();
        }
    }
    __syncthreads();

    unsigned long long v = tid < K ? selA[tid] : ~0ull;
    __syncthreads();
#pragma unroll
    for (int size = 2; size <= 256; size <<= 1) {
#pragma unroll
        for (int step = 0, stride = size >> 1; stride > 0; ++step, stride >>= 1) {
            const int x = step == 0 ? size - 1 : stride;
            unsigned long long o;
            if (x >= 64) {
                selA[tid] = v;
                __syncthreads();
                o = selA[tid ^ x];
                __syncthreads();
            } else
                o = knn_exchange(v, x);
            const bool lower = (tid & (step == 0 ? size >> 1 : stride)) == 0;
            const bool o_less = o < v;
            v = (o_less == lower) ? o : v;
        }
    }

    if (tid < K) {
        const int i = (int)(v & 0xffffffffu);
        if (dists) dists[ob + tid] = __uint_as_float((unsigned)(v >> 32));
        if (idx) idx[ob + tid] = i;
        if (nn) {
            float x = rp[3 * i], y = rp[3 * i + 1], z = rp[3 * i + 2];
            if (patch_scale != 0.f) {
                x = __fmul_rn(__fsub_rn(x, qx), patch_scale);
                y = __fmul_rn(__fsub_rn(y, qy), patch_scale);
                z = __fmul_rn(__fsub_rn(z, qz), patch_scale);
            }
            nn[(ob + tid) * 3] = x; nn[(ob + tid) * 3 + 1] = y; nn[(ob + tid) * 3 + 2] = z;
        }
    }
}

extern "C" int pccx_knn_list(const float *q, int B, int M, const float *ref, int N, int K, float *dists, int64_t *idx,
                             float *nn, float patch_scale, const int32_t *rep, void *stream)
{
    if (B == 0 || M == 0) return PCCX_OK;
    PCCX_CHECK_ARG(q && ref && (dists || idx || nn), "pccx_knn: null pointer (q, ref and at least one of dists / idx / nn are needed)");
    PCCX_CHECK_ARG(B >= 0 && M >= 0 && N >= 1, "pccx_knn: bad shape B=%d M=%d N=%d", B, M, N);
    PCCX_CHECK_ARG(K >= 1 && K <= N && K <= 1024, "pccx_knn: need 1 <= K <= min(N,1024), got K=%d N=%d", K, N);
    PCCX_CHECK_ARG(N <= 32768, "pccx_knn: N=%d > 32768 unsupported", N);
    PCCX_CHECK_ARG(B <= 65535, "pccx_knn: B=%d > 65535 unsupported", B);
    int Kp = 2;
    while (Kp < K) Kp <<= 1;
    size_t shmem = (size_t)Kp * 8 + (size_t)N * 4 + (256 + 4 + 3 + 1) * 4;
    PCCX_CHECK_HIP(hipFuncSetAttribute(reinterpret_cast<const void *>(&knn_kernel),
                                       hipFuncAttributeMaxDynamicSharedMemorySize, 160 * 1024));
    if (N <= 256 * KNN_PPT && K <= 256)
        hipLaunchKernelGGL(knn_fast_kernel, dim3(M, B), dim3(256), 0, (hipStream_t)stream, q, M, ref, N, K, dists, idx, nn,
                           patch_scale, rep);
    else
        hipLaunchKernelGGL(knn_kernel, dim3(M, B), dim3(256), shmem, (hipStream_t)stream, q, M, ref, N, K, Kp, dists, idx, nn,
                           patch_scale, rep);
    PCCX_CHECK_LAUNCH();
    return PCCX_OK;
}

extern "C" int pccx_knn(const float *q, int B, int M, const float *ref, int N, int K, float *dists, int64_t *idx,
                        float *nn, float patch_scale, void *stream)
{
    return pccx_knn_list(q, B, M, ref, N, K, dists, idx, nn, patch_scale, nullptr, stream);
}

__global__ __launch_bounds__(256) void ball_query_kernel(const float *__restrict__ q, int M, const float *__restrict__ ref,
                                                         int N, int K, float r2, float *__restrict__ dists,
                                                         int64_t *__restrict__ idx)
{
    const int lane = threadIdx.x & 63, w = threadIdx.x >> 6;
    const int m = blockIdx.x * 4 + w, b = blockIdx.y;
    if (m >= M) return;
    const float *rp = ref + (size_t)b * N * 3;
    const size_t qo = ((size_t)b * M + m) * 3;
    const float qx = q[qo], qy = q[qo + 1], qz = q[qo + 2];
    const size_t ob = ((size_t)b * M + m) * K;
    int count = 0;
    for (int base = 0; base < N && count < K; base += 64) {
        int i = base + lane;
        float d = 0.f;
        bool in = false;
        if (i < N) {
            d = pccx_sqdist(qx, qy, qz, rp[3 * i], rp[3 * i + 1], rp[3 * i + 2]);
            in = d < r2;
        }
        unsigned long long mask = __ballot(in);
        int pos = count + pccx_ballot_rank(mask);
        if (in && pos < K) { dists[ob + pos] = d; idx[ob + pos] = i; }
        count += __popcll(mask);
    }
    if (count > K) count = K;
    for (int k = count + lane; k < K; k += 64) { dists[ob + k] = 0.f; idx[ob + k] = -1; }
}

extern "C" int pccx_ball_query(const float *q, int B, int M, const float *ref, int N, int K, float radius, float *dists,
                               int64_t *idx, void *stream)
{
    if (B == 0 || M == 0) return PCCX_OK;
    PCCX_CHECK_ARG(q && ref && dists && idx, "pccx_ball_query: null pointer");
    PCCX_CHECK_ARG(B >= 0 && M >= 0 && N >= 1 && K >= 1, "pccx_ball_query: bad shape");
    PCCX_CHECK_ARG(B <= 65535, "pccx_ball_query: B=%d > 65535 unsupported", B);
    hipLaunchKernelGGL(ball_query_kernel, dim3((M + 3) / 4, B), dim3(256), 0, (hipStream_t)stream, q, M, ref, N, K,
                       radius * radius, dists, idx);
    PCCX_CHECK_LAUNCH();
    return PCCX_OK;
}

#define BQ_GMAX 16
#define BQ_NMAX 32768

extern "C" size_t pccx_ball_query_grid_workspace_ints(int B, int N) { return (size_t)(B > 0 ? B : 0) * (size_t)(8 + BQ_GMAX * BQ_GMAX * BQ_GMAX + 1 + (N > 0 ? N : 0)); }

__device__ __forceinline__ int bq_cell(float v, float lo, float inv, int G)
{
    int c = (int)floorf((v - lo) * inv);
    return c < 0 ? 0 : (c > G - 1 ? G - 1 : c);
}

__global__ __launch_bounds__(256) void bq_grid_build_kernel(const float *__restrict__ ref, int N, float radius, int32_t *__restrict__ ws,
                                                            size_t ws_stride)
{
    __shared__ float red[6][256];
    __shared__ int hist[BQ_GMAX * BQ_GMAX * BQ_GMAX + 1];
    __shared__ int scan_tmp[256];
    const int b = blockIdx.x, tid = threadIdx.x;
    const float *rp = ref + (size_t)b * N * 3;
    int32_t *w = ws + (size_t)b * ws_stride;
    float lo[3] = {INFINITY, INFINITY, INFINITY}, hi[3] = {-INFINITY, -INFINITY, -INFINITY};
    for (int i = tid; i < N; i += 256)
#pragma unroll
        for (int a = 0; a < 3; ++a) { const float v = rp[3 * i + a]; lo[a] = fminf(lo[a], v); hi[a] = fmaxf(hi[a], v); }
#pragma unroll
    for (int a = 0; a < 3; ++a) { red[a][tid] = lo[a]; red[3 + a][tid] = hi[a]; }
    __syncthreads();
    for (int o = 128; o; o >>= 1) {
        if (tid < o)
#pragma unroll
            for (int a = 0; a < 3; ++a) {
                red[a][tid] = fminf(red[a][tid], red[a][tid + o]);
                red[3 + a][tid] = fmaxf(red[3 + a][tid], red[3 + a][tid + o]);
            }
        __syncthreads();
    }
    const float ext = fmaxf(fmaxf(red[3][0] - red[0][0], red[4][0] - red[1][0]), red[5][0] - red[2][0]);
    int G = (int)floorf(ext / (radius * 1.0001f));
    G = G < 1 ? 1 : (G > BQ_GMAX ? BQ_GMAX : G);
    const float cell = ext > 0.f ? ext / (float)G : 1.f, inv = 1.f / cell;
    const float lx = red[0][0], ly = red[1][0], lz = red[2][0];
    const int cells = G * G * G;
    for (int c = tid; c <= cells; c += 256) hist[c] = 0;
    __syncthreads();
    for (int i = tid; i < N; i += 256) {
        const int c = (bq_cell(rp[3 * i], lx, inv, G) * G + bq_cell(rp[3 * i + 1], ly, inv, G)) * G + bq_cell(rp[3 * i + 2], lz, inv, G);
        atomicAdd(&hist[c], 1);
    }
    __syncthreads();
    const int per = (cells + 255) / 256;
    int local = 0;
    for (int k = 0; k < per; ++k) { const int c = tid * per + k; if (c < cells) local += hist[c]; }
    scan_tmp[tid] = local;
    __syncthreads();
    if (tid == 0) { int run = 0; for (int t = 0; t < 256; ++t) { const int v = scan_tmp[t]; scan_tmp[t] = run; run += v; } }
    __syncthreads();
    int run = scan_tmp[tid];
    for (int k = 0; k < per; ++k) { const int c = tid * per + k; if (c < cells) { const int v = hist[c]; hist[c] = run; run += v; } }
    if (tid == 0) hist[cells] = N;
    __syncthreads();
    for (int c = tid; c <= cells; c += 256) w[8 + c] = hist[c];
    if (tid == 0) { w[0] = __float_as_int(lx); w[1] = __float_as_int(ly); w[2] = __float_as_int(lz); w[3] = __float_as_int(inv); w[4] = G; }
    __syncthreads();
    int32_t *sorted = w + 8 + BQ_GMAX * BQ_GMAX * BQ_GMAX + 1;
    for (int i = tid; i < N; i += 256) {
        const int c = (bq_cell(rp[3 * i], lx, inv, G) * G + bq_cell(rp[3 * i + 1], ly, inv, G)) * G + bq_cell(rp[3 * i + 2], lz, inv, G);
        sorted[atomicAdd(&hist[c], 1)] = i;
    }
}

__global__ __launch_bounds__(256) void bq_grid_query_kernel(const float *__restrict__ q, int M, const float *__restrict__ ref, int N, int K,
                                                            float r2, const int32_t *__restrict__ ws, size_t ws_stride,
                                                            float *__restrict__ dists, int64_t *__restrict__ idx)
{
    extern __shared__ unsigned bq_bits[];
    const int lane = threadIdx.x & 63, wv = threadIdx.x >> 6;
    const int m = blockIdx.x * 4 + wv, b = blockIdx.y;
    if (m >= M) return;
    const int words = (N + 31) >> 5;
    unsigned *bits = bq_bits + (size_t)wv * words;
    for (int t = lane; t < words; t += 64) bits[t] = 0u;
    const int32_t *w = ws + (size_t)b * ws_stride;
    const float lx = __int_as_float(w[0]), ly = __int_as_float(w[1]), lz = __int_as_float(w[2]), inv = __int_as_float(w[3]);
    const int G = w[4];
    const int32_t *cstart = w + 8, *sorted = w + 8 + BQ_GMAX * BQ_GMAX * BQ_GMAX + 1;
    const float *rp = ref + (size_t)b * N * 3;
    const size_t qo = ((size_t)b * M + m) * 3;
    const float qx = q[qo], qy = q[qo + 1], qz = q[qo + 2];
    const int cx = bq_cell(qx, lx, inv, G), cy = bq_cell(qy, ly, inv, G), cz = bq_cell(qz, lz, inv, G);
    for (int dx = -1; dx <= 1; ++dx)
        for (int dy = -1; dy <= 1; ++dy) {
            const int ix = cx + dx, iy = cy + dy;
            if (ix < 0 || ix >= G || iy < 0 || iy >= G) continue;
            const int z0 = cz > 0 ? cz - 1 : 0, z1 = cz < G - 1 ? cz + 1 : G - 1;
            const int col = (ix * G + iy) * G;
            const int p0 = cstart[col + z0], p1 = cstart[col + z1 + 1];
            for (int p = p0 + lane; p < p1; p += 64) {
                const int i = sorted[p];
                if (pccx_sqdist(qx, qy, qz, rp[3 * i], rp[3 * i + 1], rp[3 * i + 2]) < r2) atomicOr(&bits[i >> 5], 1u << (i & 31));
            }
        }
    const size_t ob = ((size_t)b * M + m) * K;
    int count = 0;
    for (int base = 0; base < words && count < K; base += 64) {
        const int t = base + lane;
        unsigned wbits = t < words ? bits[t] : 0u;
        const int pc = __popc(wbits);
        int incl = pc;
#pragma unroll
        for (int o = 1; o < 64; o <<= 1) {
            const int v = __shfl_up(incl, o);
            if (lane >= o) incl += v;
        }
        int pos = count + incl - pc;
        while (wbits && pos < K) {
            const int bit = __ffs(wbits) - 1;
            wbits &= wbits - 1;
            const int i = 32 * t + bit;
            dists[ob + pos] = pccx_sqdist(qx, qy, qz, rp[3 * i], rp[3 * i + 1], rp[3 * i + 2]);
            idx[ob + pos] = i;
            ++pos;
        }
        count += __shfl(incl, 63);
    }
    if (count > K) count = K;
    for (int k = count + lane; k < K; k += 64) { dists[ob + k] = 0.f; idx[ob + k] = -1; }
}

extern "C" int pccx_ball_query_grid(const float *q, int B, int M, const float *ref, int N, int K, float radius, int32_t *workspace,
                                    float *dists, int64_t *idx, void *stream)
{
    if (B == 0 || M == 0) return PCCX_OK;
    PCCX_CHECK_ARG(q && ref && dists && idx && workspace, "pccx_ball_query_grid: null pointer");
    PCCX_CHECK_ARG(B >= 0 && M >= 0 && N >= 1 && N <= BQ_NMAX && K >= 1 && radius > 0.f, "pccx_ball_query_grid: bad shape (N <= %d)", BQ_NMAX);
    PCCX_CHECK_ARG(B <= 65535, "pccx_ball_query_grid: B=%d > 65535 unsupported", B);
    const size_t stride = (size_t)8 + BQ_GMAX * BQ_GMAX * BQ_GMAX + 1 + (size_t)N;
    hipLaunchKernelGGL(bq_grid_build_kernel, dim3(B), dim3(256), 0, (hipStream_t)stream, ref, N, radius, workspace, stride);
    PCCX_CHECK_LAUNCH();
    const size_t lds = (size_t)4 * ((N + 31) / 32) * 4;
    hipLaunchKernelGGL(bq_grid_query_kernel, dim3((M + 3) / 4, B), dim3(256), lds, (hipStream_t)stream, q, M, ref, N, K, radius * radius,
                       workspace, stride, dists, idx);
    PCCX_CHECK_LAUNCH();
    return PCCX_OK;
}

#define NND_TILE 1024
typedef float f32x2 __attribute__((ext_vector_type(2)));

template <bool WANT_NN, int XPT>
__global__ __launch_bounds__(256) void nn_dist_kernel(const float *__restrict__ X, int P, const float *__restrict__ Y, int Q,
                                                      float *__restrict__ d2, int32_t *__restrict__ nn, int qchunk)
{
    __shared__ __attribute__((aligned(8))) float tyx[NND_TILE], tyy[NND_TILE], tyz[NND_TILE];
    const int b = blockIdx.y, tid = threadIdx.x;
    const float *xp = X + (size_t)b * P * 3;
    const float *yp = Y + (size_t)b * Q * 3;
    float x[XPT][3], best[XPT];
    int bi[XPT];
#pragma unroll
    for (int j = 0; j < XPT; ++j) {
        int i = blockIdx.x * (256 * XPT) + j * 256 + tid;
        int ii = i < P ? i : P - 1;
        x[j][0] = xp[3 * ii]; x[j][1] = xp[3 * ii + 1]; x[j][2] = xp[3 * ii + 2];
        best[j] = INFINITY; bi[j] = -1;
    }
    const int q_begin = blockIdx.z * qchunk, q_end = q_begin + qchunk < Q ? q_begin + qchunk : Q;
    const size_t slice = (size_t)blockIdx.z * gridDim.y * P;
    for (int base = q_begin; base < q_end; base += NND_TILE) {
        const int cnt = q_end - base < NND_TILE ? q_end - base : NND_TILE;
        const int cnt2 = (cnt + 1) & ~1;
        __syncthreads();
        for (int t = tid; t < cnt2; t += 256) {
            const size_t src = (size_t)(base + (t < cnt ? t : cnt - 1)) * 3;
            tyx[t] = yp[src]; tyy[t] = yp[src + 1]; tyz[t] = yp[src + 2];
        }
        __syncthreads();
        for (int t = 0; t < cnt2; t += 2) {
            const f32x2 yx = *(const f32x2 *)&tyx[t], yy = *(const f32x2 *)&tyy[t], yz = *(const f32x2 *)&tyz[t];
#pragma unroll
            for (int j = 0; j < XPT; ++j) {
                const f32x2 dx = x[j][0] - yx, dy = x[j][1] - yy, dz = x[j][2] - yz;
                f32x2 d = dx * dx;
                d = d + dy * dy;
                d = d + dz * dz;
                if (WANT_NN) {
                    if (d.x < best[j]) { best[j] = d.x; bi[j] = base + t; }
                    if (d.y < best[j]) { best[j] = d.y; bi[j] = base + t + 1; }
                } else
                    best[j] = fminf(fminf(best[j], d.x), d.y);
            }
        }
    }
#pragma unroll
    for (int j = 0; j < XPT; ++j) {
        int i = blockIdx.x * (256 * XPT) + j * 256 + tid;
        if (i < P) {
            d2[slice + (size_t)b * P + i] = best[j];
            if (WANT_NN) nn[slice + (size_t)b * P + i] = bi[j];
        }
    }
}

extern "C" int pccx_nn_dist(const float *X, int B, int P, const float *Y, int Q, float *d2, int32_t *nn, void *stream)
{
    if (B == 0) return PCCX_OK;
    PCCX_CHECK_ARG(X && Y && d2, "pccx_nn_dist: null pointer");
    PCCX_CHECK_ARG(B >= 0 && P >= 1 && Q >= 1, "pccx_nn_dist: bad shape");
    PCCX_CHECK_ARG(B <= 65535, "pccx_nn_dist: B=%d > 65535 unsupported", B);
    const bool small = (long long)B * ((P + 1023) / 1024) < 512;
    const int xpt = small ? 1 : 4;
    const int gx = (P + 256 * xpt - 1) / (256 * xpt);
    hipStream_t st = (hipStream_t)stream;
    if (nn) {
        if (small) hipLaunchKernelGGL((nn_dist_kernel<true, 1>), dim3(gx, B), dim3(256), 0, st, X, P, Y, Q, d2, nn, Q);
        else hipLaunchKernelGGL((nn_dist_kernel<true, 4>), dim3(gx, B), dim3(256), 0, st, X, P, Y, Q, d2, nn, Q);
    } else {
        if (small) hipLaunchKernelGGL((nn_dist_kernel<false, 1>), dim3(gx, B), dim3(256), 0, st, X, P, Y, Q, d2, nn, Q);
        else hipLaunchKernelGGL((nn_dist_kernel<false, 4>), dim3(gx, B), dim3(256), 0, st, X, P, Y, Q, d2, nn, Q);
    }
    PCCX_CHECK_LAUNCH();
    return PCCX_OK;
}

__global__ void nn_merge_kernel(const float *__restrict__ pd, const int32_t *__restrict__ pn, long n, int split, float *__restrict__ d2,
                                int32_t *__restrict__ nn)
{
    for (long i = (long)blockIdx.x * blockDim.x + threadIdx.x; i < n; i += (long)gridDim.x * blockDim.x) {
        float best = pd[i];
        int bi = pn ? pn[i] : -1;
        for (int z = 1; z < split; ++z) {
            const float v = pd[(size_t)z * n + i];
            if (v < best) { best = v; bi = pn ? pn[(size_t)z * n + i] : -1; }
        }
        d2[i] = best;
        if (nn) nn[i] = bi;
    }
}

extern "C" int pccx_nn_dist_split_count(int B, int P, int Q)
{
    const long long wgs = (long long)B * ((P + 255) / 256);
    if (wgs <= 0 || wgs >= 256 || Q < 2 * NND_TILE) return 1;
    int split = (int)((512 + wgs - 1) / wgs);
    const int max_split = Q / NND_TILE;
    if (split > max_split) split = max_split;
    if (split > 16) split = 16;
    return split < 1 ? 1 : split;
}

extern "C" int pccx_nn_dist_split(const float *X, int B, int P, const float *Y, int Q, int split, float *scratch_d, int32_t *scratch_nn,
                                  float *d2, int32_t *nn, void *stream)
{
    if (B == 0) return PCCX_OK;
    PCCX_CHECK_ARG(X && Y && d2 && scratch_d && (!nn || scratch_nn), "pccx_nn_dist_split: null pointer");
    PCCX_CHECK_ARG(B >= 0 && B <= 65535 && P >= 1 && Q >= 1 && split >= 1 && split <= 64, "pccx_nn_dist_split: bad shape (split=%d)", split);
    int qchunk = (Q + split - 1) / split;
    qchunk = (qchunk + NND_TILE - 1) / NND_TILE * NND_TILE;
    split = (Q + qchunk - 1) / qchunk;
    hipStream_t st = (hipStream_t)stream;
// ... 306 lines not shown
```

point-cloud-compression_amd/csrc/prob.hip:

```cpp
#include <math.h>

#include "blobs.h"
#include "common.h"
#include "mfma_chain.h"

__global__ __launch_bounds__(256, 2) void prob_forward_kernel(const float *__restrict__ centres, int S, int d, int L,
                                                              const float *__restrict__ blob, float *__restrict__ pmf,
                                                              float *__restrict__ cdf, int32_t *__restrict__ cdf_int)
{
    __shared__ __attribute__((aligned(16))) f32x4 swt[4 * PRB_WS_CHUNK * 64];
    __shared__ __attribute__((aligned(16))) float sfeat[256];
    __shared__ __attribute__((aligned(16))) float su[512];
    __shared__ float smax[4][256];
    __shared__ __attribute__((aligned(16))) float slog[4][16][128];
    const int tid = threadIdx.x, lane = tid & 63, w = tid >> 6;
    const int g = lane >> 4, n = lane & 15;
    const size_t b = blockIdx.x;
    const float *cp = centres + b * (size_t)S * 3;
    const int ntiles = S >> 4;
    const int wu = __builtin_amdgcn_readfirstlane(w);
    WStreamT<PRB_WS_CHUNK, 4, 4> ws{blob + PRB_STREAM, swt, PRB_STREAM_CHUNKS, lane, wu, true};
    ws.prologue();

    f32x4 run[16];
#pragma unroll
    for (int mt = 0; mt < 16; ++mt) run[mt][0] = run[mt][1] = run[mt][2] = run[mt][3] = -INFINITY;
    for (int tile = w; tile < ntiles; tile += 4) {
        const float *bl = opaque_uniform(blob);
        const int c = tile * 16 + n;
        f32x4 in[1][1];
        in[0][0][0] = g == 0 ? cp[3 * c] : 0.f;
        in[0][0][1] = g == 0 ? cp[3 * c + 1] : 0.f;
        in[0][0][2] = g == 0 ? cp[3 * c + 2] : 0.f;
        in[0][0][3] = 0.f;
        f32x4 a0[1][4];
#pragma unroll
        for (int mt = 0; mt < 4; ++mt) a0[0][mt] = *(const f32x4 *)(bl + PRB_P_B0 + 16 * mt + 4 * g);
        dense_acc<1, 4, 1, 4>((const f32x4 *)(bl + PRB_P_W0), lane, in, a0);
#pragma unroll
        for (int mt = 0; mt < 4; ++mt) a0[0][mt] = relu4(a0[0][mt]);
        f32x4 a1[1][8];
#pragma unroll
        for (int mt = 0; mt < 8; ++mt) a1[0][mt] = *(const f32x4 *)(bl + PRB_P_B1 + 16 * mt + 4 * g);
        dense_acc<4, 8, 1, 8>((const f32x4 *)(bl + PRB_P_W1), lane, a0, a1);
#pragma unroll
        for (int mt = 0; mt < 8; ++mt) a1[0][mt] = relu4(a1[0][mt]);
        f32x4 a2[1][16];
#pragma unroll
        for (int mt = 0; mt < 16; ++mt) a2[0][mt] = *(const f32x4 *)(bl + PRB_P_B2 + 16 * mt + 4 * g);
        dense_acc<8, 16, 1, 16>((const f32x4 *)(bl + PRB_P_W2), lane, a1, a2);
#pragma unroll
        for (int mt = 0; mt < 16; ++mt)
#pragma unroll
            for (int r = 0; r < 4; ++r) run[mt][r] = fmaxf(run[mt][r], fmaxf(row16_max(a2[0][mt][r]), 0.f));
    }
    if (n == 0)
#pragma unroll
        for (int mt = 0; mt < 16; ++mt)
#pragma unroll
            for (int r = 0; r < 4; ++r) smax[w][16 * mt + 4 * g + r] = run[mt][r];
    __syncthreads();
    sfeat[tid] = fmaxf(fmaxf(smax[0][tid], smax[1][tid]), fmaxf(smax[2][tid], smax[3][tid]));
    __syncthreads();

    {
        const float *bl = opaque_uniform(blob);
        f32x4 fin[1][16];
#pragma unroll
        for (int kt = 0; kt < 16; ++kt) fin[0][kt] = *(const f32x4 *)(sfeat + 16 * kt + 4 * g);
        f32x4 u[1][8];
#pragma unroll
        for (int m = 0; m < 8; ++m) u[0][m] = *(const f32x4 *)(bl + PRB_M_B0 + 16 * (8 * wu + m) + 4 * g);
        dense_acc<16, 8, 1, 32>((const f32x4 *)(bl + PRB_M_W0), lane, fin, u, 0, 8 * wu);
        if (n == 0)
#pragma unroll
            for (int m = 0; m < 8; ++m) *(f32x4 *)(su + 16 * (8 * wu + m) + 4 * g) = u[0][m];
    }
    __syncthreads();

    const int Lp = L + 1;
    for (int tile0 = 0; tile0 < ntiles; tile0 += 4) {
        const int tile = tile0 + w;
        {
            const float *bl = opaque_uniform(blob);
            ws.g = bl + PRB_STREAM;
            int lane2 = (int)__builtin_amdgcn_mbcnt_hi(~0u, __builtin_amdgcn_mbcnt_lo(~0u, 0u));
            asm volatile("" : "+v"(lane2));
            const int g = lane2 >> 4, n = lane2 & 15;
            ws.lane = lane2;
            const int c = (tile < ntiles ? tile : ntiles - 1) * 16 + n;
            int f = 0;
            f32x4 a0[1][32];
#pragma unroll
            for (int mt = 0; mt < 32; ++mt) a0[0][mt] = *(const f32x4 *)(su + 16 * mt + 4 * g);
            {
                f32x4 in[1][1];
                in[0][0][0] = g == 0 ? cp[3 * c] : 0.f;
                in[0][0][1] = g == 0 ? cp[3 * c + 1] : 0.f;
                in[0][0][2] = g == 0 ? cp[3 * c + 2] : 0.f;
                in[0][0][3] = 0.f;
                dense_acc_stream<1, 32, 1>(ws, f, in, a0);
            }
#pragma unroll
            for (int mt = 0; mt < 32; ++mt) a0[0][mt] = relu4(a0[0][mt]);
            f32x4 a2[1][8];
#pragma unroll
            for (int mt = 0; mt < 8; ++mt) a2[0][mt] = *(const f32x4 *)(bl + PRB_M_B2 + 16 * mt + 4 * g);
#pragma clang loop unroll(full)
            for (int mp = 0; mp < 16; ++mp) {
                f32x4 a1[1][2];
#pragma unroll
                for (int m = 0; m < 2; ++m) a1[0][m] = *(const f32x4 *)(bl + PRB_M_B1 + 16 * (2 * mp + m) + 4 * g);
                dense_acc_stream<32, 2, 1>(ws, f, a0, a1);
#pragma unroll
                for (int m = 0; m < 2; ++m) a1[0][m] = relu4(a1[0][m]);
                dense_acc_stream<2, 8, 1>(ws, f, a1, a2);
            }
            if (tile < ntiles)
#pragma unroll
                for (int mt = 0; mt < 8; ++mt) *(f32x4 *)(&slog[w][n][16 * mt + 4 * g]) = a2[0][mt];
        }
        __syncthreads();
        if (tile < ntiles) {
            for (int e = lane; e < 16 * d; e += 64) {
                const int cn = e / d, i = e % d;
                const float *lg = &slog[w][cn][i * L];
                float mx = -INFINITY;
                for (int l = 0; l < L; ++l) mx = fmaxf(mx, lg[l]);
                float sum = 0.f;
                for (int l = 0; l < L; ++l) sum += expf(lg[l] - mx);
                const size_t row = (b * S + (size_t)tile * 16 + cn) * d + i;
                float run_c = 0.f;
                if (cdf) cdf[row * Lp] = 0.f;
                if (cdf_int) cdf_int[row * Lp] = 0;
                for (int l = 0; l < L; ++l) {
                    const float pv = expf(lg[l] - mx) / sum;
                    if (pmf) pmf[row * L + l] = pv;
                    run_c = run_c + pv;
                    const float cv = fminf(run_c, 1.0f);
                    if (cdf) cdf[row * Lp + l + 1] = cv;
                    if (cdf_int) cdf_int[row * Lp + l + 1] = ((int)rintf(cv * (float)(65536 - (Lp - 1))) + (l + 1)) & 0xFFFF;
                }
            }
        }
        __syncthreads();
    }
    ws.drain();
}

extern "C" int pccx_prob_forward(const float *centres, int B, int S, int d, int L, const float *prob_blob, float *pmf,
                                 float *cdf, int32_t *cdf_int, void *stream)
{
    if (B == 0) return PCCX_OK;
    PCCX_CHECK_ARG(centres && prob_blob, "pccx_prob_forward: null pointer");
    PCCX_CHECK_ARG(pmf || cdf || cdf_int, "pccx_prob_forward: no output requested");
    PCCX_CHECK_ARG(B >= 0 && S >= 16 && S % 16 == 0, "pccx_prob_forward: need S %% 16 == 0 (S=%d)", S);
    PCCX_CHECK_ARG(d >= 1 && d <= 16 && L >= 1 && L <= 15 && d * L <= 128, "pccx_prob_forward: unsupported d=%d L=%d", d, L);
    hipLaunchKernelGGL(prob_forward_kernel, dim3(B), dim3(256), 0, (hipStream_t)stream, centres, S, d, L, prob_blob, pmf, cdf,
                       cdf_int);
    PCCX_CHECK_LAUNCH();
    return PCCX_OK;
}
```

point-cloud-compression_amd/pccx/codec.py:

```python
import dataclasses
import os

import numpy as np
import torch

from . import models, ops
from .ops import stage


def packed_layout(B, s_stride, p_cap):
    o_sn, o_pn, o_c = 0, 4 * B, 8 * B
    o_sb = o_c + 16 * B
    o_pb = o_sb + B * s_stride
    return o_sn, o_pn, o_c, o_sb, o_pb, o_pb + B * p_cap


@dataclasses.dataclass
class Compressed:
    s_bytes: torch.Tensor
    s_nbytes: torch.Tensor
    p_bytes: torch.Tensor
    p_nbytes: torch.Tensor
    c: torch.Tensor
    n_points: int
    extras: dict = None
    packed: torch.Tensor = None

    @classmethod
    def alloc(cls, B, s_stride, p_cap, n_points, device):
        return cls.from_packed(torch.empty(packed_layout(B, s_stride, p_cap)[-1], device=device, dtype=torch.uint8),
                               B, s_stride, p_cap, n_points)

    @classmethod
    def from_packed(cls, packed, B, s_stride, p_cap, n_points):
        o_sn, o_pn, o_c, o_sb, o_pb, end = packed_layout(B, s_stride, p_cap)
        if packed.numel() != end or packed.dtype != torch.uint8:
            raise ValueError(f"packed stream buffer: expected {end} bytes of uint8, got {packed.numel()} of {packed.dtype}")
        return cls(packed[o_sb:o_pb].view(B, s_stride), packed[o_sn:o_pn].view(torch.int32),
                   packed[o_pb:end].view(B, p_cap), packed[o_pn:o_c].view(torch.int32),
                   packed[o_c:o_sb].view(torch.float32).view(B, 4), n_points, None, packed)

    def bits(self):
        return 8 * (self.s_nbytes.long() + self.p_nbytes.long() + 16)

    def bpp(self):
        return self.bits().double() / self.n_points

    def to_host(self):
        if getattr(self, "_host", None) is None:
            B = self.s_bytes.shape[0]
            if self.packed is None:
                comp = Compressed.alloc(B, self.s_bytes.shape[1], self.p_bytes.shape[1], self.n_points, self.s_bytes.device)
                for dst, src in ((comp.s_bytes, self.s_bytes), (comp.s_nbytes, self.s_nbytes), (comp.p_bytes, self.p_bytes),
                                 (comp.p_nbytes, self.p_nbytes), (comp.c, self.c)):
                    dst.copy_(src)
                packed = comp.packed
            else:
                packed = self.packed
            self._host_packed = packed if not packed.is_cuda else packed.cpu()
            h = Compressed.from_packed(self._host_packed, B, self.s_bytes.shape[1], self.p_bytes.shape[1], self.n_points)
            sn, pn = h.s_nbytes.numpy(), h.p_nbytes.numpy()
            if (pn < 0).any() or (sn < 0).any():
                from ._lib import PccxError
                raise PccxError("range coder / octree output buffer too small for clouds %s (negative byte count): "
                                "raise `cap`" % np.nonzero((pn < 0) | (sn < 0))[0].tolist())
            self._host = (h.s_bytes.numpy(), sn, h.p_bytes.numpy(), pn, h.c.numpy())
        return self._host

    def files(self, b):
        sb, sn, pb, pn, c = self.to_host()
        return bytes(sb[b, :sn[b]]), bytes(pb[b, :pn[b]]), c[b].tobytes()

    def write_files(self, directory, names, threads=0):
        B = self.s_bytes.shape[0]
        if len(names) != B:
            raise ValueError(f"write_files: {len(names)} names for {B} clouds")
        self.to_host()
        host = self._host_packed
        write_streams(host, B, self.s_bytes.shape[1], self.p_bytes.shape[1], directory, names, threads)
        return int(self._host[1].sum()) + int(self._host[3].sum()) + 16 * B

    @classmethod
    def read_files(cls, directory, names, n_points=0, s_stride=None, p_cap=None, device=None, threads=0, out=None):
        B = len(names)
        if s_stride is None or p_cap is None:
            ss, ps = stream_sizes(directory, names, threads)
            if B and (ss.min() < 0 or ps.min() < 0):
                from ._lib import PccxError
                raise PccxError("missing .s.bin / .p.bin for: " + ", ".join(n for n, a, b_ in zip(names, ss, ps) if a < 0 or b_ < 0))
            s_stride = int(max(1, ss.max() if B else 1)) if s_stride is None else s_stride
            p_cap = int(max(1, ps.max() if B else 1)) if p_cap is None else p_cap
        need = packed_layout(B, s_stride, p_cap)[-1]
        host = out if out is not None else torch.empty(need, dtype=torch.uint8)
        if host.numel() != need or host.dtype != torch.uint8 or host.is_cuda:
            raise ValueError(f"read_files: `out` must be a host uint8 tensor of {need} bytes")
        read_streams(host, B, s_stride, p_cap, directory, names, threads)
        packed = host.to(device, non_blocking=True) if device is not None else host
        return cls.from_packed(packed, B, s_stride, p_cap, n_points)


def _name_table(names):
    blob, off, o = bytearray(), np.zeros(max(len(names), 1), dtype=np.int64), 0
    for i, n in enumerate(names):
        e = os.fsencode(n)
        if b"\0" in e or b"/" in e:
            raise ValueError(f"stream name {n!r}: a file name without directory part is expected")
        off[i] = o
        blob += e + b"\0"
        o += len(e) + 1
    return bytes(blob) or b"\0", off


def _host_u8(t, need, who):
    if not isinstance(t, torch.Tensor) or t.is_cuda or t.dtype != torch.uint8 or not t.is_contiguous() or t.numel() != need:
        raise ValueError(f"{who}: a contiguous host uint8 tensor of {need} bytes is expected (codec.packed_layout)")
    return t


def write_streams(packed_host, B, s_stride, p_cap, directory, names, threads=0):
    from . import _lib
    blob, off = _name_table(names)
    _host_u8(packed_host, packed_layout(B, s_stride, p_cap)[-1], "write_streams")
    _lib.call("pccx_write_streams_host", packed_host.data_ptr(), B, s_stride, p_cap, os.fsencode(directory), blob, off.ctypes.data, int(threads))


def read_streams(packed_host, B, s_stride, p_cap, directory, names, threads=0):
    from . import _lib
    blob, off = _name_table(names)
    _host_u8(packed_host, packed_layout(B, s_stride, p_cap)[-1], "read_streams")
    _lib.call("pccx_read_streams_host", packed_host.data_ptr(), B, s_stride, p_cap, os.fsencode(directory), blob, off.ctypes.data, int(threads))


def stream_sizes(directory, names, threads=0):
    from . import _lib
    blob, off = _name_table(names)
    ss, ps = np.zeros(max(len(names), 1), np.int64), np.zeros(max(len(names), 1), np.int64)
    _lib.call("pccx_stream_sizes_host", len(names), os.fsencode(directory), blob, off.ctypes.data, ss.ctypes.data, ps.ctypes.data, int(threads))
    return ss[:len(names)], ps[:len(names)]


class Codec:
    def __init__(self, ae, prob, K=256, ALPHA=2, N0=1024, octree_mode="reference", margin=0.01, matmul=None,
                 decoder_matmul=None, sa_matmul=None, pn_matmul=None, group_duplicates=True):
        from . import DEFAULT_MATMUL
        matmul = matmul or DEFAULT_MATMUL
        self.ae, self.prob = ae, prob
        self.decoder_matmul = decoder_matmul or matmul
        self.sa_matmul, self.pn_matmul = sa_matmul or matmul, pn_matmul or matmul
        for m in (self.decoder_matmul, self.sa_matmul, self.pn_matmul):
            models.check_matmul("matmul", m)
        self.K, self.ALPHA, self.N0 = K, ALPHA, N0
        self.k = K // ALPHA
        self.octree_mode = octree_mode
        self.group_duplicates = bool(group_duplicates)
        self.margin = margin
        if ae.K != K or ae.k != self.k:
            raise ValueError("AE was built for a different K / k")

    def compress(self, pc, start_idx, keep_extras=False):
        B, N, _ = pc.shape
        d, L = self.ae.d, self.ae.L
        with stage("normalize"):
            pcn, center, longest = ops.normalize(pc, self.margin)
        S = int(N * self.ALPHA // self.K)
        if self.octree_mode == "reference" and S != 64:
            raise ValueError(f"octree_mode='reference' reproduces octree_np.decode's hard-coded S=64 "
                             f"(octree_np.py:100; compress.py:102 asserts); got S={S}. Use octree_mode='full'.")
        with stage("fps"):
            fps_idx = ops.farthest_point_sample_batch(pcn, S, start_idx)
        with stage("gather"):
            sampled = ops.index_points(pcn, fps_idx)
        comp = Compressed.alloc(B, (ops.octree_bits_capacity(S) + 7) // 8, models.range_cap(S * d), N, pc.device)
        with stage("octree_encode"):
            oc = ops.octree_encode(sampled, N, ops.OCTREE_BPP_DICT[self.K],
                                   out_bytes=comp.s_bytes, out_nbytes=comp.s_nbytes)
        with stage("octree_decode"):
            rec, _ = ops.octree_decode(oc["bytes"], oc["nbytes"], self.octree_mode, S)
        scale = float((N / self.N0) ** (1 / 3))
        groups = ops.patch_groups(rec) if self.group_duplicates else None
        with stage("knn_patches"):
            nn = ops.knn_points(rec, pcn, self.K, patch_scale=scale,
                                return_dists=False, return_idx=keep_extras,
                                rep=None if keep_extras or groups is None else groups.rep)
        patches = nn.knn.view(B * S, self.K, 3)
        raw, latent, q = self.ae.encode(patches, sa_matmul=self.sa_matmul, pn_matmul=self.pn_matmul, groups=groups)
        with stage("prob"):
            cdf_int = self.prob.run(rec, ("cdf_int",))["cdf_int"]
        with stage("range_encode"):
            models.range_encode(cdf_int, q.view(B, S * d), L, out=comp.p_bytes, nb=comp.p_nbytes)
        comp.c[:, :3].copy_(center)
        comp.c[:, 3].copy_(longest)
        comp._cdf_int = cdf_int
        if keep_extras:
            comp.extras = dict(pcn=pcn, fps_idx=fps_idx, sampled=sampled, octree=oc, rec_sampled=rec, patches=patches,
                          latent_raw=raw, latent=latent, latent_q=q, cdf_int=cdf_int, knn_idx=nn.idx)
        return comp

    def decompress(self, comp, S=64, reuse_cdf=False):
        B = comp.s_bytes.shape[0]
        d, L = self.ae.d, self.ae.L
        with stage("octree_decode"):
            rec, cnt = ops.octree_decode(comp.s_bytes, comp.s_nbytes, self.octree_mode, S)
        cdf_int = getattr(comp, "_cdf_int", None) if reuse_cdf else None
        if cdf_int is None or cdf_int.shape[0] != B or cdf_int.shape[1] != S:
            with stage("prob"):
                cdf_int = self.prob.run(rec, ("cdf_int",))["cdf_int"]
        with stage("range_decode"):
            q = models.range_decode(cdf_int, comp.p_bytes, comp.p_nbytes, L)
        N = S * self.k
        scale = float((N / self.N0) ** (1 / 3))
        with stage("ae_decode"):
            return self.ae.decode(q.view(B * S, d), rec.view(B * S, 3), comp.c[:, :3].contiguous(),
                                  comp.c[:, 3].contiguous(), S=S, scale=scale, margin=self.margin,
                                  matmul=self.decoder_matmul, group=self.group_duplicates)


def d1_psnr(orig, recon, search=None, index=None):
    d2 = ops.nn_dist(recon, index if search == "grid" and index is not None else orig, search=search).double()
    mse = d2.mean(dim=1)
    rng = orig.amax(dim=1).double() - orig.amin(dim=1).double()
    diag2 = (rng * rng).sum(dim=1)
    return 10 * torch.log10(diag2 / mse)


def d2_psnr(orig, recon, knn=30, search=None, index=None):
    if search == "grid" and index is None:
        index = ops.GridIndex(orig)
    normals = ops.estimate_normals(orig, knn, search=search, index=index)
    mse = ops.point_plane_err(recon, orig, normals, search=search, index=index).double().mean(dim=1)
    rng = orig.amax(dim=1).double() - orig.amin(dim=1).double()
    return 10 * torch.log10((rng * rng).sum(dim=1) / mse)


def normalized_chamfer(orig, recon, search=None):
    lo = orig.amin(dim=(1, 2), keepdim=True)
    hi = orig.amax(dim=(1, 2), keepdim=True)
    a = ((orig - lo) / (hi - lo)).contiguous()
    b = ((recon - lo) / (hi - lo)).contiguous()
    return ops.nn_dist(b, a, search=search).double().mean(dim=1) + ops.nn_dist(a, b, search=search).double().mean(dim=1)
```

point-cloud-compression_amd/pccx/models.py:

```python
import torch
import torch.nn as nn

from . import _lib, MATMUL_MODES
from .ops import _stream, _f32c, stage


def check_matmul(name, value):
    if value not in MATMUL_MODES:
        raise ValueError(f"{name}={value!r}: expected 'f32', 'bf16x3' or 'f16x2'")


def _conv_stack(chans, relu):
    mods = nn.ModuleList()
    for i in range(len(chans) - 1):
        layers = [nn.Conv2d(chans[i], chans[i + 1], 1)]
        if relu[i]:
            layers.append(nn.ReLU())
        mods.append(nn.Sequential(*layers))
    return mods


def _pccx_default_matmul():
    from . import DEFAULT_MATMUL
    return DEFAULT_MATMUL
# ... 60 lines not shown
        B, Cc, N = x.shape
        if self._fused is not None and self.npoint == N and Cc == 3:
            return self._fused(x)
        from .families import group_max
        from . import ops
        pts = x.permute(0, 2, 1).contiguous()
        S = self.npoint
        new_xyz = pts if S == N else ops.index_points(pts, ops.farthest_point_sample_batch(pts, S, start_idx))
        nn_ = ops.knn_points(new_xyz, pts, self.K, patch_scale=1.0)
        rows = nn_.knn.reshape(B * S * self.K, Cc).contiguous()
        for layer in _lazy_layers(self, x.device, lambda dev: [_folded(self.conv0, True, dev), _folded(self.conv1, True, dev),
                                                               _folded(self.conv2, self.finalRelu, dev)]):
            rows = layer(rows)
        feat = group_max(rows.view(B * S, self.K, -1)).view(B, S, -1)
        return new_xyz.permute(0, 2, 1), feat.permute(0, 2, 1)


class PointNet(_ConvStack):
    def __init__(self, in_channel, mlps, relu, bn=False):
        super().__init__()
        if bn:
            raise _lib.PccxError("pccx.PointNet: bn=True is not on the codec path (AE.py:17 uses bn=False)")
        self.mlp_Modules = _conv_stack([in_channel] + list(mlps), relu)

    def forward(self, points):
        if self._fused is not None:
            r = self._fused(points)
            if r is not None:
                return r
        from .families import group_max
        rows, B, N = self._rows(points)
        return group_max(rows.view(B, N, -1))


class MLP(_ConvStack):
    def __init__(self, in_channel, mlps, relu, bn=False):
        super().__init__()
        if bn:
            raise _lib.PccxError("pccx.MLP: bn=True is not on the codec path (AE.py:27 uses bn=False)")
        self.mlp_Modules = _conv_stack([in_channel] + list(mlps), relu)

    def forward(self, points):
        rows, B, N = self._rows(points)
        return rows.view(B, N, -1).permute(0, 2, 1)


class LinearStack(nn.Sequential):

    _layers = None

    def load_state_dict(self, *a, **k):
        r = super().load_state_dict(*a, **k)
        self._layers = None
        return r

    def forward(self, x):
        x = _f32c(x, "inv_pool")
        lead = x.shape[:-1]
        rows = x.reshape(-1, x.shape[-1]).contiguous()
        for layer in _lazy_layers(self, x.device, lambda dev: _folded_sequence(list(self), dev)):
            rows = layer(rows)
        return rows.view(*lead, -1)


def _host(t):
    return t.detach().to("cpu", torch.float32).contiguous()


_WS = {}


def workspace(tag, numel, device):
    key = (tag, str(device), torch.cuda.current_stream().cuda_stream)
    t = _WS.get(key)
    if t is None or t.numel() < numel:
        _WS[key] = t = torch.empty(int(numel), device=device, dtype=torch.float32)
    return t[:numel]


def _pack(fn_name, size, tensors, ints):
    keep = [_host(t) for t in tensors]
    blob = torch.zeros(size, dtype=torch.float32)
    _lib.call(fn_name, *[t.data_ptr() for t in keep], *ints, blob.data_ptr())
    return blob


def _pack_on_device(fn_name, size, src, ints=()):
    blob = torch.empty(size, device=src.device, dtype=torch.float32)
    _lib.call(fn_name, src.data_ptr(), *ints, blob.data_ptr(), _stream())
    return blob


_DERIVED_BLOBS = {
    "sa_b3": lambda ae, lib, enc, dec: _pack_on_device("pccx_pack_sa_b3", lib.pccx_sa_b3_blob_floats(), enc),
    "pn_b3": lambda ae, lib, enc, dec: _pack_on_device("pccx_pack_pn_b3", lib.pccx_pn_b3_blob_floats(), enc),
    "dec_b3": lambda ae, lib, enc, dec: _pack_on_device("pccx_pack_ae_decoder_b3", lib.pccx_dec_b3_blob_floats(ae.k), dec, (ae.k,)),
    "enc_h2": lambda ae, lib, enc, dec: _pack("pccx_pack_ae_encoder_h2", lib.pccx_ae_encoder_h2_blob_floats(), ae._enc_tensors(),
                                              [ae.d]).to(enc.device),
    "dec_h2": lambda ae, lib, enc, dec: _pack("pccx_pack_ae_decoder_h2", lib.pccx_ae_decoder_h2_blob_floats(ae.k), ae._dec_tensors(),
                                              [ae.k, ae.d]).to(enc.device),
}
_FUSED_ENCODERS = {
    "f16x2": ("pccx_ae_encode_h2_tables_list", "pccx_ae_encode_h2_workspace_bytes", ("enc_h2",), True),
    "bf16x3": ("pccx_ae_encode_b3_tables", "pccx_ae_encode_b3_workspace_bytes", ("sa_b3", "pn_b3"), False),
}
_DECODERS = {
    "f32": ("pccx_ae_decode", "pccx_ae_decode_workspace_floats", "dec_h2", None),
    "bf16x3": ("pccx_ae_decode_b3", "pccx_ae_decode_b3_workspace_floats", "dec_h2_b3", "dec_b3"),
    "f16x2": ("pccx_ae_decode_h2_list", "pccx_ae_decode_h2_workspace_floats", "dec_h2_h2", "dec_h2"),
}


class AE(nn.Module):

    def __init__(self, K, k, d, L):
        super().__init__()
        if d < 1 or L < 1 or K % 16 != 0 or not 16 <= K <= 1024:
            raise _lib.PccxError(
                f"pccx.AE: --K must be a multiple of 16 in 16..1024 (got {K}; the reference's octree rate table pn_kit.py:17-23 has "
                f"64..1024 only) and --d, --L positive (got {d}, {L}); the reference's defaults are --K 256 --d 16 --L 7 "
                f"(compress.py:30-34)")
        self.fused_d = d <= 16
        self.sa = SetAbstraction(npoint=K, K=16, in_channel=0, mlp=[32, 64, 128])
        self.pn = PointNet(3 + 128, [128, 256, 512, d], [True, True, True, False])
        self.inv_pool = LinearStack(nn.Linear(d, 256), nn.ReLU(), nn.Linear(256, 1024), nn.ReLU(),
                                    nn.Linear(1024, k * 128), nn.ReLU())
        self.inv_mlp = MLP(d + 128, [128, 64, 32, 3], [True, True, True, False])
        self.K, self.k, self.d, self.L = K, k, d, L
        self._enc_blob = self._dec_blob = None
        self._derived_blobs = {}
        self.sa._own(self._sa_call)
        self.pn._own(self._pn_call)

    def quantize(self, x):
        from .ops import ste_round
        return ste_round(x)

    def _sa_call(self, x):
        P, _, K = x.shape
        if K % 16 != 0 or not 16 <= K <= 1024:
            raise _lib.PccxError(f"ae.sa: K={K} must be a multiple of 16 in 16..1024")
        patches = x.permute(0, 2, 1).contiguous()
        feat = torch.empty(P, 8, K, 16, device=x.device, dtype=torch.float32)
        self._launch_sa(patches, feat, _pccx_default_matmul())
        return x, feat.permute(0, 1, 3, 2).reshape(P, 128, K)

    def _pn_call(self, points):
        x = _f32c(points, "ae.pn")
        if not self.fused_d or x.dim() != 3 or x.shape[1] != 131 or x.shape[2] % 16 != 0 or not 16 <= x.shape[2] <= 1024:
            return None
        P, _, K = x.shape
        patches = x[:, :3].permute(0, 2, 1).contiguous()
        feat = x[:, 3:].reshape(P, 8, 16, K).permute(0, 1, 3, 2).contiguous()
        outs = [torch.empty(P, self.d, device=x.device, dtype=torch.float32) for _ in range(3)]
        self._launch_pn(patches, feat, outs, _pccx_default_matmul())
        return outs[0]

    def load_state_dict(self, *a, **k):
        r = super().load_state_dict(*a, **k)
        self._enc_blob = self._dec_blob = None
        self._derived_blobs.clear()
        return r

    def pack(self, device="cuda"):
        lib = _lib.load()
        tensors, d = self._enc_tensors(), self.d
        if not self.fused_d:
            tensors, d = tensors[:12] + [torch.zeros(16, 512), torch.zeros(16)], 16
        self._enc_blob = _pack("pccx_pack_ae_encoder", lib.pccx_ae_encoder_blob_floats(), tensors, [d]).to(device)
        self._dec_blob = _pack("pccx_pack_ae_decoder", lib.pccx_ae_decoder_blob_floats(self.k), self._dec_tensors(),
                               [self.k, self.d]).to(device) if self.fused_d else None
        self._derived_blobs.clear()
        return self

    def _enc_tensors(self):
        sd = self.state_dict()
        w = lambda key: sd[key].reshape(sd[key].shape[0], -1)
        return [w("sa.conv0.weight"), sd["sa.conv0.bias"], w("sa.conv1.weight"), sd["sa.conv1.bias"],
                w("sa.conv2.weight"), sd["sa.conv2.bias"],
                w("pn.mlp_Modules.0.0.weight"), sd["pn.mlp_Modules.0.0.bias"],
                w("pn.mlp_Modules.1.0.weight"), sd["pn.mlp_Modules.1.0.bias"],
                w("pn.mlp_Modules.2.0.weight"), sd["pn.mlp_Modules.2.0.bias"],
                w("pn.mlp_Modules.3.0.weight"), sd["pn.mlp_Modules.3.0.bias"]]

    def _dec_tensors(self):
        sd = self.state_dict()
        w = lambda key: sd[key].reshape(sd[key].shape[0], -1)
        return [sd["inv_pool.0.weight"], sd["inv_pool.0.bias"], sd["inv_pool.2.weight"], sd["inv_pool.2.bias"],
                sd["inv_pool.4.weight"], sd["inv_pool.4.bias"],
                w("inv_mlp.mlp_Modules.0.0.weight"), sd["inv_mlp.mlp_Modules.0.0.bias"],
                w("inv_mlp.mlp_Modules.1.0.weight"), sd["inv_mlp.mlp_Modules.1.0.bias"],
                w("inv_mlp.mlp_Modules.2.0.weight"), sd["inv_mlp.mlp_Modules.2.0.bias"],
                w("inv_mlp.mlp_Modules.3.0.weight"), sd["inv_mlp.mlp_Modules.3.0.bias"]]

    def _blobs(self, device):
        if self._enc_blob is None or self._enc_blob.device != torch.device(device):
            self.pack(device)
        return self._enc_blob, self._dec_blob

    def _derived(self, name, device):
        enc, dec = self._blobs(device)
        blob = self._derived_blobs.get(name)
        if blob is None or blob.device != enc.device:
            blob = self._derived_blobs[name] = _DERIVED_BLOBS[name](self, _lib.load(), enc, dec)
        return blob

    def _sa_b3_blob(self, device):
        return self._derived("sa_b3", device)

    def _pn_b3_blob(self, device):
        return self._derived("pn_b3", device)

    def _dec_b3_blob(self, device):
        return self._derived("dec_b3", device)

    def _enc_h2_blob(self, device):
        return self._derived("enc_h2", device)

    def _dec_h2_blob(self, device):
        return self._derived("dec_h2", device)

    def _launch_sa(self, x, feat, matmul):
        P, K, _ = x.shape
        enc, _ = self._blobs(x.device)
        check_matmul("sa_matmul", matmul)
        if matmul == "f32":
            _lib.call("pccx_sa_forward", x.data_ptr(), P, K, enc.data_ptr(), feat.data_ptr(), _stream())
        else:
            _lib.call("pccx_sa_forward_b3", x.data_ptr(), P, K, enc.data_ptr(), self._sa_b3_blob(x.device).data_ptr(),
                      feat.data_ptr(), _stream())

    def _launch_pn(self, x, feat, outs, matmul):
        P, K, _ = x.shape
        enc, _ = self._blobs(x.device)
        check_matmul("pn_matmul", matmul)
        if matmul == "f32":
            _lib.call("pccx_pn_forward", x.data_ptr(), feat.data_ptr(), P, K, enc.data_ptr(), self.d, self.L,
                      outs[0].data_ptr(), outs[1].data_ptr(), outs[2].data_ptr(), _stream())
        else:
            _lib.call("pccx_pn_forward_b3", x.data_ptr(), feat.data_ptr(), P, K, enc.data_ptr(), self._pn_b3_blob(x.device).data_ptr(),
                      self.d, self.L, outs[0].data_ptr(), outs[1].data_ptr(), outs[2].data_ptr(), _stream())

    def encode(self, patches, sa_matmul=None, pn_matmul=None, fused=True, groups=None):
        x = _f32c(patches, "AE.encode")
        outs = self._encode(x, sa_matmul, pn_matmul, fused, groups)
        if groups is not None:
            from .ops import replicate_rows
            replicate_rows(groups, *outs)
        return outs

    def _encode(self, x, sa_matmul, pn_matmul, fused, groups):
        P, K, _ = x.shape
        if groups is not None and groups.rep.numel() != P:
            raise _lib.PccxError(f"AE.encode: groups of {groups.rep.numel()} patches for {P} patches")
        if not self.fused_d:
            return self.encode_generic(x)
        outs = [torch.empty(P, self.d, device=x.device, dtype=torch.float32) for _ in range(3)]
        sa_matmul, pn_matmul = sa_matmul or _pccx_default_matmul(), pn_matmul or _pccx_default_matmul()
        lib = _lib.load()
        if fused and sa_matmul == pn_matmul == "f16x2" and lib.pccx_ae_encode_h2_fused_ok(K):
            mode = "f16x2"
        else:
            sa_matmul, pn_matmul = ("bf16x3" if m == "f16x2" else m for m in (sa_matmul, pn_matmul))
            mode = "bf16x3" if fused and sa_matmul == pn_matmul == "bf16x3" and lib.pccx_ae_encode_b3_fused_ok(K) else None
        if mode is not None:
            tables_fn, ws_bytes, blobs, takes_lists = _FUSED_ENCODERS[mode]
            enc, _ = self._blobs(x.device)
            ws = workspace("patch_knn16", (getattr(lib, ws_bytes)(P, K) + 3) // 4, x.device)
            lists = (groups.uniq.data_ptr(), groups.n_uniq.data_ptr()) if takes_lists and groups is not None else (None, None)
            with stage("patch_knn16"):
                _lib.call("pccx_patch_knn16_list", x.data_ptr(), P, K, ws.data_ptr(), *lists, _stream())
            with stage("sa_pn_forward"):
                _lib.call(tables_fn, x.data_ptr(), P, K, enc.data_ptr(), *[self._derived(b, x.device).data_ptr() for b in blobs],
                          self.d, self.L, outs[0].data_ptr(), outs[1].data_ptr(), outs[2].data_ptr(), ws.data_ptr(),
                          *(lists if takes_lists else ()), _stream())
            return tuple(outs)
        ws = workspace("sa_feat", P * K * 128, x.device)
        with stage("sa_forward"):
            self._launch_sa(x, ws, sa_matmul)
        with stage("pn_forward"):
            self._launch_pn(x, ws, outs, pn_matmul)
        return tuple(outs)

    def encode_generic(self, x, chunk=1024):
        from .families import sigmoid_spread, round_
        raws = []
        for i in range(0, x.shape[0], chunk):
            xt = x[i:i + chunk].permute(0, 2, 1).contiguous()
            _, feat = self.sa(xt)
            raws.append(self.pn(torch.cat((xt, feat), dim=1)))
        raw = torch.cat(raws) if raws else torch.empty(0, self.d, device=x.device)
        latent = sigmoid_spread(raw, self.L)
        return raw, latent, round_(latent)

    def decode_generic(self, q, chunk=1024):
        outs = []
        for i in range(0, q.shape[0], chunk):
            lq = q[i:i + chunk]
            lin = self.inv_pool(lq).view(lq.shape[0], -1, self.k)
            mlp_in = torch.cat((lin, lq.unsqueeze(-1).tile((1, 1, self.k))), dim=1)
            outs.append(self.inv_mlp(mlp_in).transpose(2, 1).contiguous())
        return torch.cat(outs) if outs else torch.empty(0, self.k, 3, device=q.device)

    def decode(self, latent_q, centres=None, center=None, longest=None, S=None, scale=None, margin=0.01, matmul=None, group=False):
        matmul = matmul or _pccx_default_matmul()
        q = _f32c(latent_q, "AE.decode")
        P = q.shape[0]
        reassemble = centres is not None
        if not (self.fused_d or reassemble):
            return self.decode_generic(q)
        if reassemble:
            B = P // S
            centres = _f32c(centres.reshape(P, 3), "AE.decode.centres")
            center = _f32c(center.reshape(B, 3), "AE.decode.center")
            longest = _f32c(longest.reshape(B), "AE.decode.longest")
            form = (float(scale), centres.data_ptr(), center.data_ptr(), longest.data_ptr(), int(S), float(margin))
            result = torch.empty(B, S * self.k, 3, device=q.device, dtype=torch.float32)
        else:
            form = (0.0, None, None, None, 1, float(margin))
            result = torch.empty(P, self.k, 3, device=q.device, dtype=torch.float32)
        if not self.fused_d:
            raw = self.decode_generic(q)
            _lib.call("pccx_reassemble", raw.data_ptr(), P, self.k, *form, result.data_ptr(), _stream())
            return result
        check_matmul("matmul", matmul)
        fn, ws_floats, ws_tag, blob = _DECODERS[matmul]
        _, dec = self._blobs(q.device)
        extra = (self._derived(blob, q.device).data_ptr(),) if blob else ()
        ws = workspace(ws_tag, getattr(_lib.load(), ws_floats)(P), q.device)
        groups, lists = None, ()
        if matmul == "f16x2":
            if group and reassemble:
                from .ops import patch_groups, replicate_rows
                groups = patch_groups(centres.view(B, S, 3), q.view(B, S, self.d))
            lists = (groups.uniq.data_ptr(), groups.n_uniq.data_ptr()) if groups is not None else (None, None)
        dest = (None, *form, result.data_ptr()) if reassemble else (result.data_ptr(), *form, None)
        _lib.call(fn, q.data_ptr(), P, self.d, self.k, dec.data_ptr(), *extra, ws.data_ptr(), *dest, *lists, _stream())
        if groups is not None:
            replicate_rows(groups, result)
        return result

    def forward(self, xyz):
        _, latent, q = self.encode(xyz)
        return self.decode(q), latent, q


class ConditionalProbabilityModel(nn.Module):

    _layers = None

    def __init__(self, L, d):
        super().__init__()
        self.L, self.d = L, d
        self.model_pn = PointNet(3, [64, 128, 256], [True, True, True])
        self.model_mlp = nn.Sequential(nn.Conv2d(3 + 256, 512, 1), nn.ReLU(), nn.Conv2d(512, 512, 1), nn.ReLU(),
                                       nn.Conv2d(512, d * L, 1))
        self._blob = None

    def load_state_dict(self, *a, **k):
        r = super().load_state_dict(*a, **k)
        self._blob = self._layers = self.model_pn._layers = None
        return r

    def fused_ok(self, S=16):
        return self.d <= 16 and self.L <= 15 and self.d * self.L <= 128 and S % 16 == 0 and S >= 16

    def pack(self, device="cuda"):
        if not self.fused_ok():
            self._blob = self._layers = None
            return self
        sd = self.state_dict()
        w = lambda key: sd[key].reshape(sd[key].shape[0], -1)
        blob = _pack("pccx_pack_prob", _lib.load().pccx_prob_blob_floats(),
                     [w("model_pn.mlp_Modules.0.0.weight"), sd["model_pn.mlp_Modules.0.0.bias"],
                      w("model_pn.mlp_Modules.1.0.weight"), sd["model_pn.mlp_Modules.1.0.bias"],
                      w("model_pn.mlp_Modules.2.0.weight"), sd["model_pn.mlp_Modules.2.0.bias"],
                      w("model_mlp.0.weight"), sd["model_mlp.0.bias"], w("model_mlp.2.weight"), sd["model_mlp.2.bias"],
                      w("model_mlp.4.weight"), sd["model_mlp.4.bias"]], [self.d, self.L])
        self._blob = blob.to(device)
        return self

    def run(self, sampled_xyz, want=("pmf",)):
        x = _f32c(sampled_xyz, "ConditionalProbabilityModel")
        B, S, _ = x.shape
        if not self.fused_ok(S):
            return self._run_generic(x, want)
        if self._blob is None or self._blob.device != x.device:
            self.pack(x.device)
        r, ptrs = self._outputs(want, B, S, x.device)
        _lib.call("pccx_prob_forward", x.data_ptr(), B, S, self.d, self.L, self._blob.data_ptr(), *ptrs, _stream())
        return r

    def _outputs(self, want, B, S, device):
        kinds = {"pmf": (self.L, torch.float32), "cdf": (self.L + 1, torch.float32), "cdf_int": (self.L + 1, torch.int32)}
        r = {name: torch.empty(B, S, self.d, n, device=device, dtype=dt) for name, (n, dt) in kinds.items() if name in want}
        return r, [r[name].data_ptr() if name in r else None for name in kinds]

    def _run_generic(self, x, want):
        B, S, _ = x.shape
        feature = self.model_pn(x.transpose(1, 2).contiguous())
        rows = torch.cat((x, feature[:, None, :].expand(B, S, feature.shape[1])), dim=2).reshape(B * S, -1)
        buf = torch.zeros(B * S, (rows.shape[1] + 3) // 4 * 4, device=x.device, dtype=torch.float32)
        buf[:, :rows.shape[1]] = rows
        rows = buf[:, :rows.shape[1]]
        for layer in _lazy_layers(self, x.device, lambda dev: _folded_sequence(list(self.model_mlp), dev)):
            rows = layer(rows)
        r, ptrs = self._outputs(want, B, S, x.device)
        _lib.call("pccx_softmax_cdf", rows.contiguous().data_ptr(), B * S * self.d, self.L, *ptrs, _stream())
        return r

    def forward(self, sampled_xyz):
        return self.run(sampled_xyz, ("pmf",))["pmf"]


def range_cap(nsym):
    return int(nsym) * 2 + 16


def range_encode(cdf_int, latent_q, L, cap=None, out=None, nb=None):
    B = cdf_int.shape[0]
    nsym = cdf_int[0].numel() // (L + 1)
    q = _f32c(latent_q.reshape(B, nsym), "range_encode")
    if out is None:
        out = torch.empty(B, cap or range_cap(nsym), device=q.device, dtype=torch.uint8)
    if nb is None:
        nb = torch.empty(B, device=q.device, dtype=torch.int32)
    cap = out.shape[1]
    if (out.shape[0] != B or out.dtype != torch.uint8 or not out.is_contiguous() or tuple(nb.shape) != (B,)
            or nb.dtype != torch.int32 or not nb.is_contiguous()):
        raise _lib.PccxError("range_encode: out must be dense (B,cap) u8 and nb dense (B,) i32")
    _lib.call("pccx_range_encode", cdf_int.contiguous().data_ptr(), q.data_ptr(), B, nsym, int(L), out.data_ptr(), cap,
              nb.data_ptr(), _stream())
    return out, nb


def range_decode(cdf_int, bytes_, nbytes, L):
    B = cdf_int.shape[0]
    nsym = cdf_int[0].numel() // (L + 1)
    bytes_ = bytes_.contiguous()
    q = torch.empty(B, nsym, device=bytes_.device, dtype=torch.float32)
    _lib.call("pccx_range_decode", cdf_int.contiguous().data_ptr(), bytes_.data_ptr(), bytes_.shape[1],
              nbytes.to(torch.int32).contiguous().data_ptr(), B, nsym, int(L), q.data_ptr(), _stream())
    return q
```

point-cloud-compression_amd/pccx/ops.py:

```python
import collections

import torch

from . import _lib

KNN = collections.namedtuple("KNN", ["dists", "idx", "knn"])
Groups = collections.namedtuple("Groups", ["rep", "uniq", "n_uniq"])
OCTREE_BPP_DICT = {1024: 0.07, 512: 0.125, 256: 0.25, 128: 0.5, 64: 1.0}


def _stream():
    return torch.cuda.current_stream().cuda_stream


class StageTimer:

    def __init__(self):
        self.records = []

    def totals_ms(self):
        torch.cuda.synchronize()
        out = {}
        for name, a, b in self.records:
            t, n = out.get(name, (0.0, 0))
            out[name] = (t + a.elapsed_time(b), n + 1)
        return out


_timer = None


def set_timer(t):
    global _timer
    _timer = t


class stage:
    def __init__(self, name):
        self.name = name

    def __enter__(self):
        if _timer is not None:
            self.a = torch.cuda.Event(enable_timing=True)
            self.a.record()

    def __exit__(self, *exc):
        if _timer is not None:
            b = torch.cuda.Event(enable_timing=True)
            b.record()
            _timer.records.append((self.name, self.a, b))
        return False


def _dev(t, name):
    if not isinstance(t, torch.Tensor) or not t.is_cuda:
        raise _lib.PccxError(f"{name}: expected a tensor on the GPU (pccx has no CPU fallback)")
    return t


def _f32c(t, name):
    _dev(t, name)
    if t.dtype != torch.float32:
        raise _lib.PccxError(f"{name}: expected float32, got {t.dtype}")
    return t.contiguous()


def normalize(pc, margin=0.01):
    pc = _f32c(pc, "normalize")
    B, N, _ = pc.shape
    out = torch.empty_like(pc)
    center = torch.empty(B, 3, device=pc.device, dtype=torch.float32)
    longest = torch.empty(B, device=pc.device, dtype=torch.float32)
    _lib.call("pccx_normalize", pc.data_ptr(), B, N, float(margin), out.data_ptr(), center.data_ptr(),
              longest.data_ptr(), _stream())
    return out, center, longest


def denormalize(pc, center, longest, margin=0.01):
    pc = _f32c(pc, "denormalize")
    B, N, _ = pc.shape
    center = _f32c(center.reshape(B, 3), "denormalize.center")
    longest = _f32c(longest.reshape(B), "denormalize.longest")
    out = torch.empty_like(pc)
    _lib.call("pccx_denormalize", pc.data_ptr(), B, N, float(margin), center.data_ptr(), longest.data_ptr(),
              out.data_ptr(), _stream())
    return out


def farthest_point_sample_batch(xyz, npoint, start_idx=None):
    xyz = _f32c(xyz, "farthest_point_sample_batch")
    B, N, _ = xyz.shape
    if start_idx is None:
        start_idx = torch.randint(0, N, (B,), dtype=torch.long)
    start = None if isinstance(start_idx, str) and start_idx == "zero" else torch.as_tensor(start_idx).to(device=xyz.device, dtype=torch.int32).contiguous()
    out = torch.empty(B, npoint, device=xyz.device, dtype=torch.int64)
    work = torch.empty(B * N, device=xyz.device, dtype=torch.float32) if N > 16384 else None
    _lib.call("pccx_fps", xyz.data_ptr(), B, N, int(npoint), start.data_ptr() if start is not None else None, out.data_ptr(),
              work.data_ptr() if work is not None else None, _stream())
    return out


def sample_farthest_points(xyz, K):
    idx = farthest_point_sample_batch(xyz, K, start_idx="zero")
    return index_points(xyz, idx), idx


def index_points(points, idx):
    points = _f32c(points, "index_points")
    B, N, Cc = points.shape
    idx = _dev(idx, "index_points.idx").to(torch.int64).contiguous()
    M = idx[0].numel()
    out = torch.empty(B, M, Cc, device=points.device, dtype=torch.float32)
    _lib.call("pccx_gather", points.data_ptr(), B, N, Cc, idx.data_ptr(), M, out.data_ptr(), _stream())
    return out.view(*idx.shape, Cc)


def knn_gather(x, idx):
    return index_points(x, idx)


def patch_groups(keys_a, keys_b=None):
    a = _f32c(keys_a, "patch_groups.keys_a")
    B, S, fa = a.shape
    b = _f32c(keys_b.reshape(B, S, -1), "patch_groups.keys_b") if keys_b is not None else None
    buf = torch.empty(2 * B * S + 1 + _lib.load().pccx_patch_groups_workspace_ints(B), device=a.device, dtype=torch.int32)
    g = Groups(buf[:B * S], buf[B * S:2 * B * S], buf[2 * B * S:2 * B * S + 1])
    with stage("patch_groups"):
        _lib.call("pccx_patch_groups", a.data_ptr(), fa, b.data_ptr() if b is not None else None, b.shape[2] if b is not None else 0, B, S,
                  g.rep.data_ptr(), g.uniq.data_ptr(), g.n_uniq.data_ptr(), buf[2 * B * S + 1:].data_ptr(), _stream())
    return g


def replicate_rows(groups, *arrays):
    P = groups.rep.numel()
    if not arrays or len(arrays) > 3 or any(t.dtype != torch.float32 or not t.is_contiguous() or t.numel() != arrays[0].numel() or t.numel() % max(P, 1)
                                            for t in arrays):
        raise _lib.PccxError("replicate_rows: one to three dense float32 arrays of P rows each, all of one row width, are expected")
    ptrs = [t.data_ptr() for t in arrays] + [None] * (3 - len(arrays))
    with stage("replicate"):
        _lib.call("pccx_replicate_rows", groups.rep.data_ptr(), P, arrays[0].numel() // max(P, 1), *ptrs, _stream())


def knn_points(p1, p2, K, return_nn=True, patch_scale=0.0, return_dists=True, return_idx=True, rep=None):
    p1, p2 = _f32c(p1, "knn_points.p1"), _f32c(p2, "knn_points.p2")
    B, M, _ = p1.shape
    N = p2.shape[1]
    dists = torch.empty(B, M, K, device=p1.device, dtype=torch.float32) if return_dists else None
    idx = torch.empty(B, M, K, device=p1.device, dtype=torch.int64) if return_idx else None
    nn = torch.empty(B, M, K, 3, device=p1.device, dtype=torch.float32) if return_nn else None
    ptr = lambda t: t.data_ptr() if t is not None else None
    if rep is not None and (rep.dtype != torch.int32 or rep.numel() != B * M or not rep.is_cuda or not rep.is_contiguous()):
        raise _lib.PccxError("knn_points: rep must be the dense int32 (B*M) table of patch_groups over the queries")
    _lib.call("pccx_knn_list", p1.data_ptr(), B, M, p2.data_ptr(), N, int(K), ptr(dists), ptr(idx), ptr(nn), float(patch_scale), ptr(rep), _stream())
    return KNN(dists, idx, nn)


def ball_query(p1, p2, K, radius, method="auto", extent=1.0):
    p1, p2 = _f32c(p1, "ball_query.p1"), _f32c(p2, "ball_query.p2")
    B, M, _ = p1.shape
    N = p2.shape[1]
    dists = torch.empty(B, M, K, device=p1.device, dtype=torch.float32)
    idx = torch.empty(B, M, K, device=p1.device, dtype=torch.int64)
    if method == "grid" or (method == "auto" and 4096 <= N <= 32768 and float(extent) >= 4.0 * float(radius)):
        ws = torch.empty(_lib.load().pccx_ball_query_grid_workspace_ints(B, N), device=p1.device, dtype=torch.int32)
        _lib.call("pccx_ball_query_grid", p1.data_ptr(), B, M, p2.data_ptr(), N, int(K), float(radius), ws.data_ptr(),
                  dists.data_ptr(), idx.data_ptr(), _stream())
    else:
        _lib.call("pccx_ball_query", p1.data_ptr(), B, M, p2.data_ptr(), N, int(K), float(radius),
                  dists.data_ptr(), idx.data_ptr(), _stream())
    return KNN(dists, idx, None)


def _search(search, who):
    if search is None or search == "brute":
        return False
    if search == "grid":
        return True
    raise ValueError(f"{who}: search must be None, 'brute' or 'grid', got {search!r}")


class GridIndex:

    def __init__(self, y):
        y = _f32c(y, "GridIndex.y")
        if y.dim() != 3 or y.shape[2] != 3:
            raise _lib.PccxError(f"GridIndex: expected (B,Q,3), got {tuple(y.shape)}")
        self.B, self.Q = int(y.shape[0]), int(y.shape[1])
        self.device = y.device
        self.ws = torch.empty(max(int(_lib.load().pccx_grid_index_workspace_bytes(self.B, self.Q)), 16), device=y.device, dtype=torch.uint8)
        with stage("grid_index"):
            _lib.call("pccx_grid_index_build", y.data_ptr(), self.B, self.Q, self.ws.data_ptr(), _stream())

    def _queries(self, x, who):
        x = _f32c(x, who)
        if x.dim() != 3 or x.shape[2] != 3 or x.shape[0] != self.B or x.device != self.device:
            raise _lib.PccxError(f"{who}: expected ({self.B},P,3) on {self.device}, got {tuple(x.shape)} on {x.device}")
        qws = torch.empty(max(int(_lib.load().pccx_grid_query_workspace_bytes(self.B, int(x.shape[1]))), 16), device=x.device, dtype=torch.uint8)
        return x, qws

    def nn(self, x, return_idx=False):
        x, qws = self._queries(x, "GridIndex.nn")
        P = int(x.shape[1])
        d2 = torch.empty(self.B, P, device=x.device, dtype=torch.float32)
        nn = torch.empty(self.B, P, device=x.device, dtype=torch.int32) if return_idx else None
        with stage("grid_nn"):
            _lib.call("pccx_grid_nn", x.data_ptr(), self.B, P, self.Q, self.ws.data_ptr(), qws.data_ptr(), d2.data_ptr(),
                      nn.data_ptr() if nn is not None else None, _stream())
        return (d2, nn) if return_idx else d2

    def knn(self, x, K):
        x, qws = self._queries(x, "GridIndex.knn")
        M = int(x.shape[1])
        dists = torch.empty(self.B, M, int(K), device=x.device, dtype=torch.float32)
        idx = torch.empty(self.B, M, int(K), device=x.device, dtype=torch.int64)
        with stage("grid_knn"):
            _lib.call("pccx_grid_knn", x.data_ptr(), self.B, M, self.Q, int(K), self.ws.data_ptr(), qws.data_ptr(), dists.data_ptr(),
                      idx.data_ptr(), _stream())
        return KNN(dists, idx, None)


def nn_dist(x, y, return_idx=False, search=None):
    if _search(search, "nn_dist"):
        return (y if isinstance(y, GridIndex) else GridIndex(y)).nn(x, return_idx)
    x, y = _f32c(x, "nn_dist.x"), _f32c(y, "nn_dist.y")
    B, P, _ = x.shape
    d2 = torch.empty(B, P, device=x.device, dtype=torch.float32)
    nn = torch.empty(B, P, device=x.device, dtype=torch.int32) if return_idx else None
    split = _lib.load().pccx_nn_dist_split_count(B, P, int(y.shape[1])) if B > 0 else 1
    if split > 1:
        sd = torch.empty(split, B, P, device=x.device, dtype=torch.float32)
        sn = torch.empty(split, B, P, device=x.device, dtype=torch.int32) if return_idx else None
        _lib.call("pccx_nn_dist_split", x.data_ptr(), B, P, y.data_ptr(), y.shape[1], split, sd.data_ptr(),
                  sn.data_ptr() if sn is not None else None, d2.data_ptr(), nn.data_ptr() if nn is not None else None, _stream())
        return (d2, nn) if return_idx else d2
    _lib.call("pccx_nn_dist", x.data_ptr(), B, P, y.data_ptr(), y.shape[1], d2.data_ptr(),
              nn.data_ptr() if nn is not None else None, _stream())
    return (d2, nn) if return_idx else d2


def estimate_normals(xyz, knn=30, search=None, index=None):
    grid = _search(search, "estimate_normals")
    xyz = _f32c(xyz, "estimate_normals")
    B, N, _ = xyz.shape
    if grid:
        idx = (index if index is not None else GridIndex(xyz)).knn(xyz, min(knn, N)).idx
    else:
        idx = knn_points(xyz, xyz, min(knn, N), return_nn=False).idx
    out = torch.empty(B, N, 3, device=xyz.device, dtype=torch.float32)
    _lib.call("pccx_estimate_normals", xyz.data_ptr(), B, N, idx.data_ptr(), idx.shape[2], out.data_ptr(), _stream())
    return out


def point_plane_err(x, y, normals_y, search=None, index=None):
    grid = _search(search, "point_plane_err")
    x, y, normals_y = _f32c(x, "point_plane_err.x"), _f32c(y, "point_plane_err.y"), _f32c(normals_y, "point_plane_err.n")
    B, P, _ = x.shape
    _, nn = (index if index is not None else GridIndex(y)).nn(x, return_idx=True) if grid else nn_dist(x, y, return_idx=True)
    err = torch.empty(B, P, device=x.device, dtype=torch.float32)
    _lib.call("pccx_point_plane_err", x.data_ptr(), B, P, y.data_ptr(), normals_y.data_ptr(), y.shape[1], nn.data_ptr(),
              err.data_ptr(), _stream())
    return err


zeros_hook = None
deterministic_hook = None


def chamfer_grad_det(x, y, nxy, nyx, gd):
    lib = _lib.load()
    B, P, Q = x.shape[0], x.shape[1], y.shape[1]
    gx, gy = torch.empty_like(x), torch.empty_like(y)
    wf = torch.empty(max(int(lib.pccx_chamfer_grad_det_workspace_floats(B, P, Q)), 1), device=x.device, dtype=torch.float32)
    wi = torch.empty(max(int(lib.pccx_chamfer_grad_det_workspace_ints(B, P, Q)), 1), device=x.device, dtype=torch.int32)
    _lib.call("pccx_chamfer_grad_det", x.data_ptr(), B, P, y.data_ptr(), Q, nxy.data_ptr(), nyx.data_ptr(), gd.data_ptr(), gx.data_ptr(),
              gy.data_ptr(), wf.data_ptr(), wi.data_ptr(), _stream())
    return gx, gy


class _ChamferFn(torch.autograd.Function):

    @staticmethod
    def forward(ctx, x, y):
        dxy, nxy = nn_dist(x, y, return_idx=True)
        dyx, nyx = nn_dist(y, x, return_idx=True)
        ctx.save_for_backward(x, y, nxy, nyx)
        ctx.det = bool(deterministic_hook()) if deterministic_hook is not None else False
        out = torch.empty((), device=x.device, dtype=torch.float32)
        _lib.call("pccx_chamfer_mean", dxy.data_ptr(), dyx.data_ptr(), x.shape[0], x.shape[1], y.shape[1], out.data_ptr(), _stream())
        return out

    @staticmethod
    def backward(ctx, g):
        x, y, nxy, nyx = ctx.saved_tensors
        gd = g.detach().to(torch.float32).reshape(1).contiguous()
        if ctx.det:
            return chamfer_grad_det(x, y, nxy, nyx, gd)
        if zeros_hook is not None:
            gx, gy = zeros_hook(tuple(x.shape), torch.float32, x.device)[0], zeros_hook(tuple(y.shape), torch.float32, y.device)[0]
            _lib.call("pccx_chamfer_grad_dev_acc", x.data_ptr(), x.shape[0], x.shape[1], y.data_ptr(), y.shape[1], nxy.data_ptr(),
                      nyx.data_ptr(), gd.data_ptr(), gx.data_ptr(), gy.data_ptr(), 4, _stream())
            return gx, gy
        gx, gy = torch.empty_like(x), torch.empty_like(y)
        _lib.call("pccx_chamfer_grad_dev", x.data_ptr(), x.shape[0], x.shape[1], y.data_ptr(), y.shape[1], nxy.data_ptr(),
                  nyx.data_ptr(), gd.data_ptr(), gx.data_ptr(), gy.data_ptr(), _stream())
        return gx, gy


class _STERound(torch.autograd.Function):

    @staticmethod
    def forward(ctx, x):
        xc = _f32c(x, "STEQuantize")
        y = torch.empty_like(xc)
        _lib.call("pccx_round", xc.data_ptr(), xc.numel(), y.data_ptr(), _stream())
        return y

    @staticmethod
    def backward(ctx, g):
        return g


def ste_round(x):
    if isinstance(x, torch.Tensor) and not x.is_cuda:
        return _STERound.apply(x.cuda()).to(x.device)
    return _STERound.apply(x)


def chamfer_distance(x, y, batch_reduction="mean"):
    if batch_reduction == "mean" and (x.requires_grad or y.requires_grad):
        return _ChamferFn.apply(_f32c(x, "chamfer.x"), _f32c(y, "chamfer.y")), None
    dxy, dyx = nn_dist(x, y), nn_dist(y, x)
    per = dxy.double().mean(dim=1) + dyx.double().mean(dim=1)
    if batch_reduction == "mean":
        per = per.mean()
    elif batch_reduction == "sum":
        per = per.sum()
    return per.float(), None


def octree_bits_capacity(S):
    return int(_lib.load().pccx_octree_bits_capacity(int(S)))


def octree_encode(centres, N, min_bpp, out_bytes=None, out_nbytes=None):
    centres = _f32c(centres, "octree_encode")
    B, S, _ = centres.shape
    cap = octree_bits_capacity(S)
    dev = centres.device
    if out_bytes is None:
        out_bytes = torch.empty(B, (cap + 7) // 8, device=dev, dtype=torch.uint8)
    if out_nbytes is None:
        out_nbytes = torch.empty(B, device=dev, dtype=torch.int32)
    if (tuple(out_bytes.shape) != (B, (cap + 7) // 8) or out_bytes.dtype != torch.uint8 or not out_bytes.is_contiguous()
            or tuple(out_nbytes.shape) != (B,) or out_nbytes.dtype != torch.int32 or not out_nbytes.is_contiguous()):
        raise _lib.PccxError("octree_encode: out_bytes must be dense (B, (cap+7)//8) u8 and out_nbytes dense (B,) i32")
    r = dict(bits=torch.empty(B, cap, device=dev, dtype=torch.uint8),
             nbits=torch.empty(B, device=dev, dtype=torch.int32),
             depth=torch.empty(B, device=dev, dtype=torch.int32),
             bytes=out_bytes, nbytes=out_nbytes)
    _lib.call("pccx_octree_encode", centres.data_ptr(), B, S, int(N), float(min_bpp), r["bits"].data_ptr(),
              r["nbits"].data_ptr(), r["depth"].data_ptr(), r["bytes"].data_ptr(), r["nbytes"].data_ptr(), _stream())
    return r


def octree_decode(bytes_, nbytes, mode="reference", S_out=64):
    _dev(bytes_, "octree_decode")
    bytes_ = bytes_.contiguous()
    B, stride = bytes_.shape
    nbytes = _dev(nbytes, "octree_decode.nbytes").to(torch.int32).contiguous()
    out = torch.empty(B, S_out, 3, device=bytes_.device, dtype=torch.float32)
    count = torch.empty(B, device=bytes_.device, dtype=torch.int32)
    _lib.call("pccx_octree_decode", bytes_.data_ptr(), stride, nbytes.data_ptr(), B,
              {"reference": 0, "full": 1}[mode], int(S_out), out.data_ptr(), count.data_ptr(), _stream())
    return out, count
```

Before: 1.024 billion points/s.

## Add unique-list paths for kNN, prob model and decoder head in reference mode

When patches are grouped in reference octree mode, the kNN kernel now walks a compact list of unique patches with a persistent grid instead of launching one block per query and early-exiting duplicates. A distinct-clouds variant of the probability model kernel and a per-tile split of the decoder head kernel (four waves each take a quarter of the output channels) are added and selected on that path. The aim is to drop wasted blocks and raise parallelism when most patches are unique, at the cost of more code paths and a fixed grid cap for the list kernel.

```diff
diff --git a/include/pccx.h b/include/pccx.h
--- a/include/pccx.h
+++ b/include/pccx.h
@@ -186,6 +186,9 @@
 PCCX_API int pccx_replicate_rows(const int32_t *rep, int64_t P, int row_floats, float *a0, float *a1, float *a2, void *stream);
 PCCX_API int pccx_knn_list(const float *q, int B, int M, const float *ref, int N, int K, float *dists, int64_t *idx, float *nn,
                            float patch_scale, const int32_t *rep, void *stream);
+PCCX_API int pccx_knn_uniq_ok(int N, int K);
+PCCX_API int pccx_knn_uniq(const float *q, int B, int M, const float *ref, int N, int K, float *dists, int64_t *idx, float *nn,
+                           float patch_scale, const int32_t *uniq, const int32_t *n_uniq, void *stream);
 PCCX_API int pccx_patch_knn16_list(const float *patches, int P, int K, void *nbr, const int32_t *uniq, const int32_t *n_uniq,
                                    void *stream);
 PCCX_API int pccx_ae_encode_h2_tables_list(const float *patches, int P, int K, const float *enc_blob, const float *h2_blob, int d,
@@ -195,9 +198,15 @@
                                     float *workspace, float *patches_out, float scale, const float *centres,
                                     const float *nrm_center, const float *nrm_longest, int S, double margin, float *pc_out,
                                     const int32_t *uniq, const int32_t *n_uniq, void *stream);
+PCCX_API int pccx_ae_decode_h2_short_list(const float *latent_q, int P, int d, int k, const float *dec_blob, const float *h2_blob,
+                                          float *workspace, float *patches_out, float scale, const float *centres,
+                                          const float *nrm_center, const float *nrm_longest, int S, double margin, float *pc_out,
+                                          const int32_t *uniq, const int32_t *n_uniq, void *stream);
 
 PCCX_API int pccx_prob_forward(const float *centres, int B, int S, int d, int L, const float *prob_blob,
                                float *pmf, float *cdf, int32_t *cdf_int, void *stream);
+PCCX_API int pccx_prob_forward_distinct(const float *centres, int B, int S, int d, int L, const float *prob_blob,
+                                        float *pmf, float *cdf, int32_t *cdf_int, void *stream);
 
 PCCX_API int pccx_range_encode(const int32_t *cdf_int, const float *latent_q, int B, int nsym, int L,
                                uint8_t *out, int cap, int32_t *nbytes, void *stream);
diff --git a/point-cloud-compression_amd/csrc/decoder.hip b/point-cloud-compression_amd/csrc/decoder.hip
--- a/point-cloud-compression_amd/csrc/decoder.hip
+++ b/point-cloud-compression_amd/csrc/decoder.hip
@@ -6,13 +6,14 @@
 #include "mfma_chain.h"
 #include "plane_ring.h"
 
+template <bool SPLIT>
 __global__ __launch_bounds__(256, 2) void dec_head_kernel(const float *__restrict__ latent_q, int P, int d, int ntiles,
                                                           const float *__restrict__ blob, f32x4 *__restrict__ h2p,
                                                           const int *__restrict__ uniq, const int *__restrict__ n_uniq)
 {
     const int tid = threadIdx.x, lane = tid & 63, w = tid >> 6;
     const int g = lane >> 4, n = lane & 15;
-    const int tile = blockIdx.x * 4 + w;
+    const int tile = SPLIT ? blockIdx.x : blockIdx.x * 4 + w;
     if (uniq) P = *n_uniq;
     if (tile >= (P + 15) / 16) return;
     const int patch = tile * 16 + n;
@@ -27,8 +28,9 @@
 #pragma unroll
     for (int mt = 0; mt < 16; ++mt) a1[0][mt] = relu4(a1[0][mt]);
     const f32x4 *w2 = (const f32x4 *)(blob + DEC_H_W2);
+    const int mc0 = SPLIT ? 4 * __builtin_amdgcn_readfirstlane(w) : 0;
 #pragma unroll 1
-    for (int mc = 0; mc < 16; ++mc) {
+    for (int mc = mc0; mc < mc0 + (SPLIT ? 4 : 16); ++mc) {
         const f32x4 *w2c = opaque_uniform(w2) + (size_t)mc * 4 * 64;
         f32x4 a2[1][4];
 #pragma unroll
@@ -40,9 +42,12 @@
 }
 
 int pccx_dec_head_launch(const float *latent_q, int P, int d, int ntiles, const float *dec_blob, float *h2p, const int32_t *uniq,
-                         const int32_t *n_uniq, hipStream_t st)
-{
-    hipLaunchKernelGGL(dec_head_kernel, dim3((ntiles + 3) / 4), dim3(256), 0, st, latent_q, P, d, ntiles, dec_blob, (f32x4 *)h2p, uniq, n_uniq);
+                         const int32_t *n_uniq, bool per_tile, hipStream_t st)
+{
+    if (uniq && per_tile)
+        hipLaunchKernelGGL(dec_head_kernel<true>, dim3(ntiles), dim3(256), 0, st, latent_q, P, d, ntiles, dec_blob, (f32x4 *)h2p, uniq, n_uniq);
+    else
+        hipLaunchKernelGGL(dec_head_kernel<false>, dim3((ntiles + 3) / 4), dim3(256), 0, st, latent_q, P, d, ntiles, dec_blob, (f32x4 *)h2p, uniq, n_uniq);
     PCCX_CHECK_LAUNCH();
     return PCCX_OK;
 }
@@ -335,7 +340,7 @@
     if (P == 0) return PCCX_OK;
     hipStream_t st = (hipStream_t)stream;
     const int ntiles = (P + 15) / 16;
-    hipLaunchKernelGGL(dec_head_kernel, dim3((ntiles + 3) / 4), dim3(256), 0, st, latent_q, P, d, ntiles, dec_blob,
+    hipLaunchKernelGGL(dec_head_kernel<false>, dim3((ntiles + 3) / 4), dim3(256), 0, st, latent_q, P, d, ntiles, dec_blob,
                        (f32x4 *)workspace, (const int *)nullptr, (const int *)nullptr);
     PCCX_CHECK_LAUNCH();
     hipLaunchKernelGGL(dec_main_kernel, dim3(dec_grid(ntiles, k)), dim3(256), 0, st, (const f32x4 *)workspace, latent_q, P, d,
@@ -428,7 +433,7 @@
     const int ntiles = (P + 15) / 16;
     f32x4 *h2p = (f32x4 *)workspace;
     uint4 *h3 = (uint4 *)(workspace + (size_t)64 * ntiles * 64 * 4);
-    hipLaunchKernelGGL(dec_head_kernel, dim3((ntiles + 3) / 4), dim3(256), 0, st, latent_q, P, d, ntiles, dec_blob, h2p, (const int *)nullptr, (const int *)nullptr);
+    hipLaunchKernelGGL(dec_head_kernel<false>, dim3((ntiles + 3) / 4), dim3(256), 0, st, latent_q, P, d, ntiles, dec_blob, h2p, (const int *)nullptr, (const int *)nullptr);
     PCCX_CHECK_LAUNCH();
     const size_t items = (size_t)32 * ntiles;
     hipLaunchKernelGGL(b3_split_kernel, dim3((unsigned)((items + 3) / 4)), dim3(256), 0, st, (const f32x4 *)h2p, h3, 1, 64, ntiles,
diff --git a/point-cloud-compression_amd/csrc/decoder_h2.hip b/point-cloud-compression_amd/csrc/decoder_h2.hip
--- a/point-cloud-compression_amd/csrc/decoder_h2.hip
+++ b/point-cloud-compression_amd/csrc/decoder_h2.hip
@@ -7,7 +7,7 @@
 #include "plane_ring.h"
 
 int pccx_dec_head_launch(const float *latent_q, int P, int d, int ntiles, const float *dec_blob, float *h2p, const int32_t *uniq,
-                         const int32_t *n_uniq, hipStream_t st);
+                         const int32_t *n_uniq, bool per_tile, hipStream_t st);
 
 __global__ __launch_bounds__(256) void dec_h2_prep_kernel(const f32x4 *__restrict__ h2p, const float *__restrict__ latent_q, int P, int d,
                                                           int ntiles, float sig_h, uint4 *__restrict__ h3, float *__restrict__ pscale,
@@ -205,9 +205,9 @@
     return (size_t)(64 + 64) * ntiles * 64 * 4 + ntiles * 16;
 }
 
-extern "C" int pccx_ae_decode_h2_list(const float *latent_q, int P, int d, int k, const float *dec_blob, const float *h2_blob, float *workspace,
-                                      float *patches_out, float scale, const float *centres, const float *nrm_center, const float *nrm_longest,
-                                      int S, double margin, float *pc_out, const int32_t *uniq, const int32_t *n_uniq, void *stream)
+static int dec_h2_list(const float *latent_q, int P, int d, int k, const float *dec_blob, const float *h2_blob, float *workspace,
+                       float *patches_out, float scale, const float *centres, const float *nrm_center, const float *nrm_longest,
+                       int S, double margin, float *pc_out, const int32_t *uniq, const int32_t *n_uniq, bool short_list, void *stream)
 {
     if (P == 0) return PCCX_OK;
     PCCX_CHECK_ARG(latent_q && dec_blob && h2_blob && workspace, "pccx_ae_decode_h2: null pointer");
@@ -221,7 +221,7 @@
     float *h2p = workspace;
     uint4 *h3 = (uint4 *)(workspace + (size_t)64 * ntiles * 64 * 4);
     float *pscale = workspace + (size_t)128 * ntiles * 64 * 4;
-    const int rc = pccx_dec_head_launch(latent_q, P, d, ntiles, dec_blob, h2p, uniq, n_uniq, st);
+    const int rc = pccx_dec_head_launch(latent_q, P, d, ntiles, dec_blob, h2p, uniq, n_uniq, short_list, st);
     if (rc != PCCX_OK) return rc;
     hipLaunchKernelGGL(dec_h2_prep_kernel, dim3((ntiles + 3) / 4), dim3(256), 0, st, (const f32x4 *)h2p, latent_q, P, d, ntiles, 32768.0f, h3, pscale, uniq, n_uniq);
     PCCX_CHECK_LAUNCH();
@@ -236,6 +236,22 @@
     return PCCX_OK;
 }
 
+extern "C" int pccx_ae_decode_h2_list(const float *latent_q, int P, int d, int k, const float *dec_blob, const float *h2_blob, float *workspace,
+                                      float *patches_out, float scale, const float *centres, const float *nrm_center, const float *nrm_longest,
+                                      int S, double margin, float *pc_out, const int32_t *uniq, const int32_t *n_uniq, void *stream)
+{
+    return dec_h2_list(latent_q, P, d, k, dec_blob, h2_blob, workspace, patches_out, scale, centres, nrm_center, nrm_longest, S, margin, pc_out, uniq,
+                       n_uniq, false, stream);
+}
+
+extern "C" int pccx_ae_decode_h2_short_list(const float *latent_q, int P, int d, int k, const float *dec_blob, const float *h2_blob, float *workspace,
+                                            float *patches_out, float scale, const float *centres, const float *nrm_center, const float *nrm_longest,
+                                            int S, double margin, float *pc_out, const int32_t *uniq, const int32_t *n_uniq, void *stream)
+{
+    return dec_h2_list(latent_q, P, d, k, dec_blob, h2_blob, workspace, patches_out, scale, centres, nrm_center, nrm_longest, S, margin, pc_out, uniq,
+                       n_uniq, true, stream);
+}
+
 extern "C" int pccx_ae_decode_h2(const float *latent_q, int P, int d, int k, const float *dec_blob, const float *h2_blob, float *workspace,
                                  float *patches_out, float scale, const float *centres, const float *nrm_center, const float *nrm_longest,
                                  int S, double margin, float *pc_out, void *stream)
diff --git a/point-cloud-compression_amd/csrc/knn.hip b/point-cloud-compression_amd/csrc/knn.hip
--- a/point-cloud-compression_amd/csrc/knn.hip
+++ b/point-cloud-compression_amd/csrc/knn.hip
@@ -131,6 +131,7 @@
 #define KNN_PPT 32
 #define KNN_BINS 2048
 #define KNN_CAPB 256
+#define KNN_LIST_GRID (256 * 8)
 
 template <int X>
 __device__ __forceinline__ unsigned knn_xor_lane(unsigned v)
@@ -200,16 +201,12 @@
     cnt = s_found[2];
 }
 
-__global__ __launch_bounds__(256, 4) void knn_fast_kernel(const float *__restrict__ q, int M, const float *__restrict__ ref,
-                                                       int N, int K, float *__restrict__ dists, int64_t *__restrict__ idx,
-                                                       float *__restrict__ nn, float patch_scale, const int *__restrict__ rep)
-{
-    __shared__ int hist[KNN_BINS];
-    __shared__ unsigned long long selA[256], selB[KNN_CAPB];
-    __shared__ int s_wsum[4], s_found[3], s_cnt[2];
-    const int tid = threadIdx.x, lane = tid & 63, w = tid >> 6;
-    const int m = blockIdx.x, b = blockIdx.y;
-    if (rep && rep[b * M + m] != b * M + m) return;
+__device__ __forceinline__ void knn_fast_query(const float *__restrict__ q, int M, const float *__restrict__ ref, int N, int K,
+                                               float *__restrict__ dists, int64_t *__restrict__ idx, float *__restrict__ nn, float patch_scale,
+                                               int m, int b, int tid, int *hist, unsigned long long *selA, unsigned long long *selB,
+                                               int *s_wsum, int *s_found, int *s_cnt)
+{
+    const int lane = tid & 63, w = tid >> 6;
     const float *rp = ref + (size_t)b * N * 3;
     const size_t qo = ((size_t)b * M + m) * 3;
     const float qx = q[qo], qy = q[qo + 1], qz = q[qo + 2];
@@ -323,8 +320,38 @@
     }
 }
 
-extern "C" int pccx_knn_list(const float *q, int B, int M, const float *ref, int N, int K, float *dists, int64_t *idx,
-                             float *nn, float patch_scale, const int32_t *rep, void *stream)
+__global__ __launch_bounds__(256, 4) void knn_fast_kernel(const float *__restrict__ q, int M, const float *__restrict__ ref,
+                                                       int N, int K, float *__restrict__ dists, int64_t *__restrict__ idx,
+                                                       float *__restrict__ nn, float patch_scale, const int *__restrict__ rep)
+{
+    __shared__ int hist[KNN_BINS];
+    __shared__ unsigned long long selA[256], selB[KNN_CAPB];
+    __shared__ int s_wsum[4], s_found[3], s_cnt[2];
+    const int m = blockIdx.x, b = blockIdx.y;
+    if (rep && rep[b * M + m] != b * M + m) return;
+    knn_fast_query(q, M, ref, N, K, dists, idx, nn, patch_scale, m, b, threadIdx.x, hist, selA, selB, s_wsum, s_found, s_cnt);
+}
+
+__global__ __launch_bounds__(256, 4) void knn_fast_list_kernel(const float *__restrict__ q, int M, const float *__restrict__ ref,
+                                                            int N, int K, float *__restrict__ dists, int64_t *__restrict__ idx,
+                                                            float *__restrict__ nn, float patch_scale, const int *__restrict__ uniq,
+                                                            const int *__restrict__ n_uniq)
+{
+    __shared__ int hist[KNN_BINS];
+    __shared__ unsigned long long selA[256], selB[KNN_CAPB];
+    __shared__ int s_wsum[4], s_found[3], s_cnt[2];
+    const int nlist = *n_uniq;
+    for (int slot = blockIdx.x; slot < nlist; slot += gridDim.x) {
+        int tid = threadIdx.x;
+        asm volatile("" : "+v"(tid));
+        const int p = uniq[slot];
+        knn_fast_query(q, M, ref, N, K, dists, idx, nn, patch_scale, p % M, p / M, tid, hist, selA, selB, s_wsum, s_found, s_cnt);
+        __syncthreads();
+    }
+}
+
+static int knn_launch(const float *q, int B, int M, const float *ref, int N, int K, float *dists, int64_t *idx, float *nn,
+                      float patch_scale, const int32_t *rep, const int32_t *uniq, const int32_t *n_uniq, void *stream)
 {
     if (B == 0 || M == 0) return PCCX_OK;
     PCCX_CHECK_ARG(q && ref && (dists || idx || nn), "pccx_knn: null pointer (q, ref and at least one of dists / idx / nn are needed)");
@@ -337,20 +364,41 @@
     size_t shmem = (size_t)Kp * 8 + (size_t)N * 4 + (256 + 4 + 3 + 1) * 4;
     PCCX_CHECK_HIP(hipFuncSetAttribute(reinterpret_cast<const void *>(&knn_kernel),
                                        hipFuncAttributeMaxDynamicSharedMemorySize, 160 * 1024));
-    if (N <= 256 * KNN_PPT && K <= 256)
-        hipLaunchKernelGGL(knn_fast_kernel, dim3(M, B), dim3(256), 0, (hipStream_t)stream, q, M, ref, N, K, dists, idx, nn,
-                           patch_scale, rep);
-    else
+    if (N <= 256 * KNN_PPT && K <= 256) {
+        const long long bm = (long long)B * M;
+        const dim3 grid = uniq ? dim3((unsigned)(bm < KNN_LIST_GRID ? bm : KNN_LIST_GRID)) : dim3(M, B);
+        if (uniq)
+            hipLaunchKernelGGL(knn_fast_list_kernel, grid, dim3(256), 0, (hipStream_t)stream, q, M, ref, N, K, dists, idx, nn, patch_scale, uniq, n_uniq);
+        else
+            hipLaunchKernelGGL(knn_fast_kernel, grid, dim3(256), 0, (hipStream_t)stream, q, M, ref, N, K, dists, idx, nn, patch_scale, rep);
+    } else
         hipLaunchKernelGGL(knn_kernel, dim3(M, B), dim3(256), shmem, (hipStream_t)stream, q, M, ref, N, K, Kp, dists, idx, nn,
                            patch_scale, rep);
     PCCX_CHECK_LAUNCH();
     return PCCX_OK;
 }
 
+extern "C" int pccx_knn_list(const float *q, int B, int M, const float *ref, int N, int K, float *dists, int64_t *idx,
+                             float *nn, float patch_scale, const int32_t *rep, void *stream)
+{
+    return knn_launch(q, B, M, ref, N, K, dists, idx, nn, patch_scale, rep, nullptr, nullptr, stream);
+}
+
+extern "C" int pccx_knn_uniq_ok(int N, int K) { return N >= 1 && N <= 256 * KNN_PPT && K >= 1 && K <= 256 && K <= N; }
+
+extern "C" int pccx_knn_uniq(const float *q, int B, int M, const float *ref, int N, int K, float *dists, int64_t *idx, float *nn,
+                             float patch_scale, const int32_t *uniq, const int32_t *n_uniq, void *stream)
+{
+    PCCX_CHECK_ARG(!uniq == !n_uniq, "pccx_knn_uniq: uniq and n_uniq come together");
+    PCCX_CHECK_ARG(!uniq || pccx_knn_uniq_ok(N, K), "pccx_knn_uniq: the list form needs N <= %d and K <= 256 (N=%d K=%d); use pccx_knn_list",
+                   256 * KNN_PPT, N, K);
+    return knn_launch(q, B, M, ref, N, K, dists, idx, nn, patch_scale, nullptr, uniq, n_uniq, stream);
+}
+
 extern "C" int pccx_knn(const float *q, int B, int M, const float *ref, int N, int K, float *dists, int64_t *idx,
                         float *nn, float patch_scale, void *stream)
 {
-    return pccx_knn_list(q, B, M, ref, N, K, dists, idx, nn, patch_scale, nullptr, stream);
+    return knn_launch(q, B, M, ref, N, K, dists, idx, nn, patch_scale, nullptr, nullptr, nullptr, stream);
 }
 
 __global__ __launch_bounds__(256) void ball_query_kernel(const float *__restrict__ q, int M, const float *__restrict__ ref,
diff --git a/point-cloud-compression_amd/csrc/prob.hip b/point-cloud-compression_amd/csrc/prob.hip
--- a/point-cloud-compression_amd/csrc/prob.hip
+++ b/point-cloud-compression_amd/csrc/prob.hip
@@ -148,6 +148,236 @@
     ws.drain();
 }
 
+__device__ __forceinline__ void prob_wave_sync()
+{
+    __builtin_amdgcn_fence(__ATOMIC_RELEASE, "wavefront");
+    __builtin_amdgcn_wave_barrier();
+    __builtin_amdgcn_fence(__ATOMIC_ACQUIRE, "wavefront");
+}
+
+template <int W>
+__device__ __forceinline__ void prob_store_pmf(const float *rows, const int *slots, int nslots, int t, int lane, size_t row0, int rl,
+                                               float *__restrict__ pmf)
+{
+    const int per = rl / W;
+    for (int it = lane; it < nslots * per; it += 64) {
+        const int c = it / per, j = (it % per) * W, sl = slots[c];
+        if ((sl >> 4) != t) continue;
+        const float *src = rows + (sl & 15) * 128 + j;
+        float *dst = pmf + (row0 + c) * (size_t)rl + j;
+        if constexpr (W == 4) *(f32x4 *)dst = *(const f32x4 *)src;
+        else *dst = *src;
+    }
+}
+
+template <int W>
+__device__ __forceinline__ void prob_store_cdf(const float *rows, const int *slots, int nslots, int t, int lane, size_t row0, int d, int L,
+                                               float *__restrict__ cdf, int32_t *__restrict__ cdf_int)
+{
+    const int Lp = L + 1, rl = d * Lp, per = rl / W;
+    for (int it = lane; it < nslots * per; it += 64) {
+        const int c = it / per, j = (it % per) * W, sl = slots[c];
+        if ((sl >> 4) != t) continue;
+        float cv[W];
+        int ci[W];
+#pragma unroll
+        for (int q = 0; q < W; ++q) {
+            const int i = (j + q) / Lp, l = (j + q) % Lp;
+            cv[q] = l ? rows[(sl & 15) * 128 + i * L + l - 1] : 0.f;
+            ci[q] = l ? ((int)rintf(cv[q] * (float)(65536 - (Lp - 1))) + l) & 0xFFFF : 0;
+        }
+        const size_t o = (row0 + c) * (size_t)rl + j;
+        if constexpr (W == 4) {
+            if (cdf) *(f32x4 *)(cdf + o) = f32x4{cv[0], cv[1], cv[2], cv[3]};
+            if (cdf_int) *(int4 *)(cdf_int + o) = make_int4(ci[0], ci[1], ci[2], ci[3]);
+        } else {
+            if (cdf) cdf[o] = cv[0];
+            if (cdf_int) cdf_int[o] = ci[0];
+        }
+    }
+}
+
+__global__ __launch_bounds__(256, 2) void prob_forward_distinct_kernel(const float *__restrict__ centres, int B, int S, int d, int L,
+                                                                       const float *__restrict__ blob, float *__restrict__ pmf,
+                                                                       float *__restrict__ cdf, int32_t *__restrict__ cdf_int)
+{
+    __shared__ __attribute__((aligned(16))) f32x4 swt[4 * PRB_WS_CHUNK * 64];
+    __shared__ __attribute__((aligned(16))) float sfeat[4][256];
+    __shared__ __attribute__((aligned(16))) float su[4][512];
+    __shared__ __attribute__((aligned(16))) float slog[4][16][128];
+    __shared__ int slot_of[4][64], cen_of[4][64], s_nt[4];
+    const int tid = threadIdx.x, lane = tid & 63, w = tid >> 6;
+    const int g = lane >> 4, n = lane & 15;
+    const int wu = __builtin_amdgcn_readfirstlane(w);
+    const int bw = blockIdx.x * 4 + wu;
+    const bool live = bw < B;
+    const size_t b = live ? bw : B - 1;
+    const float *cp = centres + b * (size_t)S * 3;
+    WStreamT<PRB_WS_CHUNK, 4, 4> ws{blob + PRB_STREAM, swt, PRB_STREAM_CHUNKS, lane, wu, true};
+    ws.prologue();
+
+    int nt;
+    {
+        const bool valid = lane < S;
+        const int cl = valid ? lane : S - 1;
+        const unsigned kx = __float_as_uint(cp[3 * cl]), ky = __float_as_uint(cp[3 * cl + 1]), kz = __float_as_uint(cp[3 * cl + 2]);
+        int rep = cl;
+        for (int j = S - 1; j >= 0; --j) {
+            const unsigned jx = __builtin_amdgcn_readlane(kx, j), jy = __builtin_amdgcn_readlane(ky, j), jz = __builtin_amdgcn_readlane(kz, j);
+            if (jx == kx && jy == ky && jz == kz) rep = j;
+        }
+        const unsigned long long reps = __ballot(valid && rep == lane);
+        const int rank = __popcll(reps & ((1ull << lane) - 1ull));
+        const int slot = __shfl(rank, rep);
+        {
+            unsigned long long m = reps;
+            const int nd = __popcll(reps);
+            for (int i = 0; i < (lane < nd ? lane : 0); ++i) m &= m - 1ull;
+            cen_of[w][lane] = lane < nd ? __ffsll((long long)m) - 1 : 0;
+        }
+        if (valid) slot_of[w][lane] = slot;
+        nt = __builtin_amdgcn_readfirstlane((__popcll(reps) + 15) >> 4);
+        if (lane == 0) s_nt[w] = nt;
+    }
+    __syncthreads();
+
+    {
+        f32x4 run[16];
+#pragma unroll
+        for (int mt = 0; mt < 16; ++mt) run[mt][0] = run[mt][1] = run[mt][2] = run[mt][3] = -INFINITY;
+        for (int tile = 0; tile < nt; ++tile) {
+            const float *bl = opaque_uniform(blob);
+            const int c = cen_of[w][tile * 16 + n];
+            f32x4 in[1][1];
+            in[0][0][0] = g == 0 ? cp[3 * c] : 0.f;
+            in[0][0][1] = g == 0 ? cp[3 * c + 1] : 0.f;
+            in[0][0][2] = g == 0 ? cp[3 * c + 2] : 0.f;
+            in[0][0][3] = 0.f;
+            f32x4 a0[1][4];
+#pragma unroll
+            for (int mt = 0; mt < 4; ++mt) a0[0][mt] = *(const f32x4 *)(bl + PRB_P_B0 + 16 * mt + 4 * g);
+            dense_acc<1, 4, 1, 4>((const f32x4 *)(bl + PRB_P_W0), lane, in, a0);
+#pragma unroll
+            for (int mt = 0; mt < 4; ++mt) a0[0][mt] = relu4(a0[0][mt]);
+            f32x4 a1[1][8];
+#pragma unroll
+            for (int mt = 0; mt < 8; ++mt) a1[0][mt] = *(const f32x4 *)(bl + PRB_P_B1 + 16 * mt + 4 * g);
+            dense_acc<4, 8, 1, 8>((const f32x4 *)(bl + PRB_P_W1), lane, a0, a1);
+#pragma unroll
+            for (int mt = 0; mt < 8; ++mt) a1[0][mt] = relu4(a1[0][mt]);
+            f32x4 a2[1][16];
+#pragma unroll
+            for (int mt = 0; mt < 16; ++mt) a2[0][mt] = *(const f32x4 *)(bl + PRB_P_B2 + 16 * mt + 4 * g);
+            dense_acc<8, 16, 1, 16>((const f32x4 *)(bl + PRB_P_W2), lane, a1, a2);
+#pragma unroll
+            for (int mt = 0; mt < 16; ++mt)
+#pragma unroll
+                for (int r = 0; r < 4; ++r) run[mt][r] = fmaxf(run[mt][r], fmaxf(row16_max(a2[0][mt][r]), 0.f));
+        }
+        if (n == 0)
+#pragma unroll
+            for (int mt = 0; mt < 16; ++mt) *(f32x4 *)(&sfeat[w][16 * mt + 4 * g]) = run[mt];
+    }
+    __syncthreads();
+    const int ntmax = max(max(s_nt[0], s_nt[1]), max(s_nt[2], s_nt[3]));
+
+    {
+        const float *bl = opaque_uniform(blob);
+        f32x4 fin[1][16];
+#pragma unroll
+        for (int kt = 0; kt < 16; ++kt) fin[0][kt] = *(const f32x4 *)(&sfeat[n & 3][16 * kt + 4 * g]);
+        f32x4 u[1][8];
+#pragma unroll
+        for (int m = 0; m < 8; ++m) u[0][m] = *(const f32x4 *)(bl + PRB_M_B0 + 16 * (8 * wu + m) + 4 * g);
+        dense_acc<16, 8, 1, 32>((const f32x4 *)(bl + PRB_M_W0), lane, fin, u, 0, 8 * wu);
+        if (n < 4)
+#pragma unroll
+            for (int m = 0; m < 8; ++m) *(f32x4 *)(&su[n][16 * (8 * wu + m) + 4 * g]) = u[0][m];
+    }
+    __syncthreads();
+
+    const int Lp = L + 1;
+    for (int t = 0; t < ntmax; ++t) {
+        const bool act = live && t < nt;
+        {
+            const float *bl = opaque_uniform(blob);
+            ws.g = bl + PRB_STREAM;
+            int lane2 = (int)__builtin_amdgcn_mbcnt_hi(~0u, __builtin_amdgcn_mbcnt_lo(~0u, 0u));
+            asm volatile("" : "+v"(lane2));
+            const int g = lane2 >> 4, n = lane2 & 15;
+            ws.lane = lane2;
+            const int c = cen_of[wu][(t < nt ? t : nt - 1) * 16 + n];
+            int f = 0;
+            f32x4 a0[1][32];
+#pragma unroll
+            for (int mt = 0; mt < 32; ++mt) a0[0][mt] = *(const f32x4 *)(&su[wu][16 * mt + 4 * g]);
+            {
+                f32x4 in[1][1];
+                in[0][0][0] = g == 0 ? cp[3 * c] : 0.f;
+                in[0][0][1] = g == 0 ? cp[3 * c + 1] : 0.f;
+                in[0][0][2] = g == 0 ? cp[3 * c + 2] : 0.f;
+                in[0][0][3] = 0.f;
+                dense_acc_stream<1, 32, 1>(ws, f, in, a0);
+            }
+#pragma unroll
+            for (int mt = 0; mt < 32; ++mt) a0[0][mt] = relu4(a0[0][mt]);
+            f32x4 a2[1][8];
+#pragma unroll
+            for (int mt = 0; mt < 8; ++mt) a2[0][mt] = *(const f32x4 *)(bl + PRB_M_B2 + 16 * mt + 4 * g);
+#pragma clang loop unroll(full)
+            for (int mp = 0; mp < 16; ++mp) {
+                f32x4 a1[1][2];
+#pragma unroll
+                for (int m = 0; m < 2; ++m) a1[0][m] = *(const f32x4 *)(bl + PRB_M_B1 + 16 * (2 * mp + m) + 4 * g);
+                dense_acc_stream<32, 2, 1>(ws, f, a0, a1);
+#pragma unroll
+                for (int m = 0; m < 2; ++m) a1[0][m] = relu4(a1[0][m]);
+                dense_acc_stream<2, 8, 1>(ws, f, a1, a2);
+            }
+            if (t < nt)
+#pragma unroll
+                for (int mt = 0; mt < 8; ++mt) *(f32x4 *)(&slog[wu][n][16 * mt + 4 * g]) = a2[0][mt];
+        }
+        prob_wave_sync();
+        const int nslots = S < 64 ? S : 64;
+        if (act)
+            for (int e = lane; e < 16 * d; e += 64) {
+                float *lg = &slog[wu][e / d][(e % d) * L];
+                float mx = -INFINITY;
+                for (int l = 0; l < L; ++l) mx = fmaxf(mx, lg[l]);
+                float sum = 0.f;
+                for (int l = 0; l < L; ++l) sum += expf(lg[l] - mx);
+                for (int l = 0; l < L; ++l) lg[l] = expf(lg[l] - mx) / sum;
+            }
+        prob_wave_sync();
+        if (act && pmf) {
+            if ((d * L) % 4 == 0 && ((uintptr_t)pmf & 15) == 0) prob_store_pmf<4>(&slog[wu][0][0], slot_of[wu], nslots, t, lane, b * S, d * L, pmf);
+            else prob_store_pmf<1>(&slog[wu][0][0], slot_of[wu], nslots, t, lane, b * S, d * L, pmf);
+        }
+        if (cdf || cdf_int) {
+            prob_wave_sync();
+            if (act)
+                for (int e = lane; e < 16 * d; e += 64) {
+                    float *lg = &slog[wu][e / d][(e % d) * L];
+                    float run_c = 0.f;
+                    for (int l = 0; l < L; ++l) {
+                        run_c = run_c + lg[l];
+                        lg[l] = fminf(run_c, 1.0f);
+                    }
+                }
+            prob_wave_sync();
+            if (act) {
+                if ((d * Lp) % 4 == 0 && (((uintptr_t)cdf | (uintptr_t)cdf_int) & 15) == 0)
+                    prob_store_cdf<4>(&slog[wu][0][0], slot_of[wu], nslots, t, lane, b * S, d, L, cdf, cdf_int);
+                else
+                    prob_store_cdf<1>(&slog[wu][0][0], slot_of[wu], nslots, t, lane, b * S, d, L, cdf, cdf_int);
+            }
+        }
+        prob_wave_sync();
+    }
+    ws.drain();
+}
+
 extern "C" int pccx_prob_forward(const float *centres, int B, int S, int d, int L, const float *prob_blob, float *pmf,
                                  float *cdf, int32_t *cdf_int, void *stream)
 {
@@ -161,3 +391,17 @@
     PCCX_CHECK_LAUNCH();
     return PCCX_OK;
 }
+
+extern "C" int pccx_prob_forward_distinct(const float *centres, int B, int S, int d, int L, const float *prob_blob, float *pmf,
+                                          float *cdf, int32_t *cdf_int, void *stream)
+{
+    if (B == 0) return PCCX_OK;
+    PCCX_CHECK_ARG(centres && prob_blob, "pccx_prob_forward_distinct: null pointer");
+    PCCX_CHECK_ARG(pmf || cdf || cdf_int, "pccx_prob_forward_distinct: no output requested");
+    PCCX_CHECK_ARG(B >= 0 && S >= 16 && S % 16 == 0 && S <= 64, "pccx_prob_forward_distinct: need S %% 16 == 0, S <= 64 (S=%d)", S);
+    PCCX_CHECK_ARG(d >= 1 && d <= 16 && L >= 1 && L <= 15 && d * L <= 128, "pccx_prob_forward_distinct: unsupported d=%d L=%d", d, L);
+    hipLaunchKernelGGL(prob_forward_distinct_kernel, dim3((B + 3) / 4), dim3(256), 0, (hipStream_t)stream, centres, B, S, d, L, prob_blob,
+                       pmf, cdf, cdf_int);
+    PCCX_CHECK_LAUNCH();
+    return PCCX_OK;
+}
diff --git a/point-cloud-compression_amd/pccx/codec.py b/point-cloud-compression_amd/pccx/codec.py
--- a/point-cloud-compression_amd/pccx/codec.py
+++ b/point-cloud-compression_amd/pccx/codec.py
@@ -156,6 +156,9 @@
         self.margin = margin
         if ae.K != K or ae.k != self.k:
             raise ValueError("AE was built for a different K / k")
+
+    def _distinct(self):
+        return self.octree_mode == "reference" and self.group_duplicates
 
     def compress(self, pc, start_idx, keep_extras=False):
         B, N, _ = pc.shape
@@ -181,11 +184,11 @@
         with stage("knn_patches"):
             nn = ops.knn_points(rec, pcn, self.K, patch_scale=scale,
                                 return_dists=False, return_idx=keep_extras,
-                                rep=None if keep_extras or groups is None else groups.rep)
+                                **({} if keep_extras or groups is None else {"groups": groups} if self._distinct() else {"rep": groups.rep}))
         patches = nn.knn.view(B * S, self.K, 3)
         raw, latent, q = self.ae.encode(patches, sa_matmul=self.sa_matmul, pn_matmul=self.pn_matmul, groups=groups)
         with stage("prob"):
-            cdf_int = self.prob.run(rec, ("cdf_int",))["cdf_int"]
+            cdf_int = self.prob.run(rec, ("cdf_int",), distinct=self._distinct())["cdf_int"]
         with stage("range_encode"):
             models.range_encode(cdf_int, q.view(B, S * d), L, out=comp.p_bytes, nb=comp.p_nbytes)
         comp.c[:, :3].copy_(center)
@@ -204,7 +207,7 @@
         cdf_int = getattr(comp, "_cdf_int", None) if reuse_cdf else None
         if cdf_int is None or cdf_int.shape[0] != B or cdf_int.shape[1] != S:
             with stage("prob"):
-                cdf_int = self.prob.run(rec, ("cdf_int",))["cdf_int"]
+                cdf_int = self.prob.run(rec, ("cdf_int",), distinct=self._distinct())["cdf_int"]
         with stage("range_decode"):
             q = models.range_decode(cdf_int, comp.p_bytes, comp.p_nbytes, L)
         N = S * self.k
@@ -212,7 +215,7 @@
         with stage("ae_decode"):
             return self.ae.decode(q.view(B * S, d), rec.view(B * S, 3), comp.c[:, :3].contiguous(),
                                   comp.c[:, 3].contiguous(), S=S, scale=scale, margin=self.margin,
-                                  matmul=self.decoder_matmul, group=self.group_duplicates)
+                                  matmul=self.decoder_matmul, group=self.group_duplicates, short_list=self._distinct())
 
 
 def d1_psnr(orig, recon, search=None, index=None):
diff --git a/point-cloud-compression_amd/pccx/models.py b/point-cloud-compression_amd/pccx/models.py
--- a/point-cloud-compression_amd/pccx/models.py
+++ b/point-cloud-compression_amd/pccx/models.py
@@ -386,7 +386,7 @@
             outs.append(self.inv_mlp(mlp_in).transpose(2, 1).contiguous())
         return torch.cat(outs) if outs else torch.empty(0, self.k, 3, device=q.device)
 
-    def decode(self, latent_q, centres=None, center=None, longest=None, S=None, scale=None, margin=0.01, matmul=None, group=False):
+    def decode(self, latent_q, centres=None, center=None, longest=None, S=None, scale=None, margin=0.01, matmul=None, group=False, short_list=False):
         matmul = matmul or _pccx_default_matmul()
         q = _f32c(latent_q, "AE.decode")
         P = q.shape[0]
@@ -419,6 +419,8 @@
                 groups = patch_groups(centres.view(B, S, 3), q.view(B, S, self.d))
             lists = (groups.uniq.data_ptr(), groups.n_uniq.data_ptr()) if groups is not None else (None, None)
         dest = (None, *form, result.data_ptr()) if reassemble else (result.data_ptr(), *form, None)
+        if groups is not None and short_list:
+            fn = "pccx_ae_decode_h2_short_list"
         _lib.call(fn, q.data_ptr(), P, self.d, self.k, dec.data_ptr(), *extra, ws.data_ptr(), *dest, *lists, _stream())
         if groups is not None:
             replicate_rows(groups, result)
@@ -464,7 +466,7 @@
         self._blob = blob.to(device)
         return self
 
-    def run(self, sampled_xyz, want=("pmf",)):
+    def run(self, sampled_xyz, want=("pmf",), distinct=False):
         x = _f32c(sampled_xyz, "ConditionalProbabilityModel")
         B, S, _ = x.shape
         if not self.fused_ok(S):
@@ -472,7 +474,8 @@
         if self._blob is None or self._blob.device != x.device:
             self.pack(x.device)
         r, ptrs = self._outputs(want, B, S, x.device)
-        _lib.call("pccx_prob_forward", x.data_ptr(), B, S, self.d, self.L, self._blob.data_ptr(), *ptrs, _stream())
+        fn = "pccx_prob_forward_distinct" if distinct and S <= 64 else "pccx_prob_forward"
+        _lib.call(fn, x.data_ptr(), B, S, self.d, self.L, self._blob.data_ptr(), *ptrs, _stream())
         return r
 
     def _outputs(self, want, B, S, device):
diff --git a/point-cloud-compression_amd/pccx/ops.py b/point-cloud-compression_amd/pccx/ops.py
--- a/point-cloud-compression_amd/pccx/ops.py
+++ b/point-cloud-compression_amd/pccx/ops.py
@@ -141,7 +141,7 @@
         _lib.call("pccx_replicate_rows", groups.rep.data_ptr(), P, arrays[0].numel() // max(P, 1), *ptrs, _stream())
 
 
-def knn_points(p1, p2, K, return_nn=True, patch_scale=0.0, return_dists=True, return_idx=True, rep=None):
+def knn_points(p1, p2, K, return_nn=True, patch_scale=0.0, return_dists=True, return_idx=True, rep=None, groups=None):
     p1, p2 = _f32c(p1, "knn_points.p1"), _f32c(p2, "knn_points.p2")
     B, M, _ = p1.shape
     N = p2.shape[1]
@@ -151,6 +151,14 @@
     ptr = lambda t: t.data_ptr() if t is not None else None
     if rep is not None and (rep.dtype != torch.int32 or rep.numel() != B * M or not rep.is_cuda or not rep.is_contiguous()):
         raise _lib.PccxError("knn_points: rep must be the dense int32 (B*M) table of patch_groups over the queries")
+    if groups is not None:
+        if rep is not None or groups.rep.numel() != B * M:
+            raise _lib.PccxError("knn_points: groups must be the patch_groups of the (B, M) queries, given without rep")
+        if _lib.load().pccx_knn_uniq_ok(N, int(K)):
+            _lib.call("pccx_knn_uniq", p1.data_ptr(), B, M, p2.data_ptr(), N, int(K), ptr(dists), ptr(idx), ptr(nn), float(patch_scale),
+                      groups.uniq.data_ptr(), groups.n_uniq.data_ptr(), _stream())
+            return KNN(dists, idx, nn)
+        rep = groups.rep
     _lib.call("pccx_knn_list", p1.data_ptr(), B, M, p2.data_ptr(), N, int(K), ptr(dists), ptr(idx), ptr(nn), float(patch_scale), ptr(rep), _stream())
     return KNN(dists, idx, nn)
 
```

New measurement: 1.092 billion points/s (median of 6 runs). 1.07x the previous value.
